# kaist-ina/BWA-MEME

Hardware: AMD Instinct MI355X
Metric: seeding_reads_per_sec (higher is better)
Workload: dtype u64; 1 GPU; learned-index seeding (rounds 1-3 + hit gather), 150 bp SE reads vs 3100 Mbp synthetic genome (fwd+rc suffix array of 6200000000 entries), index and reads resident in HBM; genome_bp=3100000000, sa_entries=6200000000, read_len=150, rmi_leaves_log2=28

## Files before the change

bwa-meme_amd/csrc/meme_common.h:

```cpp
#pragma once
#include <hip/hip_runtime.h>
#include <stdint.h>
#include <stdio.h>
#include <string>
#include <type_traits>
#include <utility>
#include <vector>

#include "meme_hip.h"

typedef uint64_t u64;
typedef int64_t i64;

struct __attribute__((aligned(16))) SaEnt {
    u64 key;
    u64 pos;
};

struct RmiRec {
    double icpt;
    double slope;
    u64 err;
};

struct Rmi32 {
    double icpt;
    double slope;
    u64 err;
    u64 pad;
};

struct DevIndex {
    i64 n = 0;
    const SaEnt* sa = nullptr;
    const u64* pac = nullptr;
    const Rmi32* l2 = nullptr;
    const Rmi32* l1 = nullptr;
    i64 n_l2 = 0, n_l1 = 0;
    int shift = 64;
    const uint8_t* plcp = nullptr;
};

template <bool HOST> struct Buf {
    void* p = nullptr;
    size_t cap = 0;
    Buf() = default;
    Buf(const Buf&) = delete; Buf& operator=(const Buf&) = delete;
    ~Buf() { if (p) (void)(HOST ? hipHostFree(p) : hipFree(p)); }
    template <class T> T* as() const { return (T*)p; }
};
typedef Buf<false> DevBuf;
typedef Buf<true> HostBuf;
static_assert(!std::is_copy_constructible<DevBuf>::value && !std::is_copy_assignable<DevBuf>::value && !std::is_copy_constructible<HostBuf>::value &&
              !std::is_copy_assignable<HostBuf>::value, "a workspace owns its memory: a copy would free it twice");
template <int N> struct Events {
    hipEvent_t e[N] = {};
    Events() = default;
    Events(const Events&) = delete; Events& operator=(const Events&) = delete;
    ~Events() { for (hipEvent_t x : e) if (x) (void)hipEventDestroy(x); }
    hipEvent_t& operator[](int i) { return e[i]; }
    hipError_t ensure() { for (hipEvent_t& x : e) if (!x) { const hipError_t r = hipEventCreate(&x); if (r != hipSuccess) return r; } return hipSuccess; }
};
struct Stream {
    hipStream_t s = nullptr;
    Stream() = default;
    Stream(const Stream&) = delete; Stream& operator=(const Stream&) = delete;
    ~Stream() { if (s) (void)hipStreamDestroy(s); }
    operator hipStream_t() const { return s; }
};

struct Carve {
    unsigned char* base;
    size_t bytes = 0;
    explicit Carve(void* b) : base((unsigned char*)b) {}
    template <class T> T* take(size_t count, size_t align = 1) { bytes = (bytes + align - 1) / align * align; T* q = base ? (T*)(base + bytes) : nullptr; bytes += count * sizeof(T); return q; }
    i64* col(i64 n) { return take<i64>((size_t)n + 1); }
};
struct ContigTab {
    i64* off; int* len; unsigned char* alt; size_t bytes;
    ContigTab(void* base, i64 n, bool with_alt) { Carve c(base); off = c.take<i64>(n); len = c.take<int>(n); alt = c.take<unsigned char>((with_alt ? n : 0) + 64); bytes = c.bytes; }
};
struct ChainCounts {
    i64 *chain_off, *seed_off, *nch, *nsd; int* tree; unsigned char* fb; unsigned long long* route; size_t bytes;
    ChainCounts(void* base, i64 n) { Carve c(base); chain_off = c.col(n); seed_off = c.col(n); nch = c.col(n); nsd = c.col(n); tree = c.take<int>(n); fb = c.take<unsigned char>(n + 64);
                                     route = c.take<unsigned long long>(8, 16); bytes = c.bytes; }
};
struct ChainLists {
    i64 *list[5], *work[5], *woff[5]; unsigned char* cls; size_t bytes;
    ChainLists(void* base, i64 n) { Carve c(base); for (int k = 0; k < 5; ++k) { list[k] = c.col(n); work[k] = c.col(n); woff[k] = c.col(n); } cls = c.take<unsigned char>(n + 64); bytes = c.bytes; }
};
enum { EXT_L = 0, EXT_R = 1, EXT_B = 2 };
struct ExtCounts {
    i64 *cnt[3], *off[3], *cntS, *offS; size_t bytes;
    ExtCounts(void* base, i64 n) { Carve c(base); for (i64*& q : cnt) q = c.col(n); for (i64*& q : off) q = c.col(n); cntS = c.col(n); offS = c.col(n); bytes = c.bytes; }
    bool adjacent(i64 n) const { return off[1] == off[0] + (n + 1) && off[2] == off[1] + (n + 1); }
};
struct CountScan {
    i64 *cnt, *off; size_t bytes;
    CountScan(void* base, i64 n) { Carve c(base); cnt = c.col(n); off = c.col(n); bytes = c.bytes; }
};
struct ExtRetry {
    meme_seqpair* half[2]; size_t bytes;
    ExtRetry(void* base, i64 nmax) { Carve c(base); for (meme_seqpair*& q : half) q = c.take<meme_seqpair>((size_t)nmax + 1); bytes = c.bytes; }
};
struct ExtRounds {
    int4* state; uint8_t* act; uint8_t* sel; size_t bytes;
    ExtRounds(void* base, i64 n, i64 seeds) { Carve c(base); state = c.take<int4>(n + 1); act = c.take<uint8_t>(n + 1); sel = c.take<uint8_t>(seeds + 64); bytes = c.bytes; }
};
struct GcigCols {
    i64 *zsz, *csz, *zoff, *coff, *ncig, *ooff, *msz, *moff, *psz, *poff, *isdp, *dpoff, *dplist, *is16, *o16, *is32, *o32, *is64, *o64, *bad; size_t bytes;
    GcigCols(void* base, i64 n) { Carve c(base); zsz = c.col(n); csz = c.col(n); zoff = c.col(n); coff = c.col(n); ncig = c.col(n); ooff = c.col(n); msz = c.col(n); moff = c.col(n);
        psz = c.col(n); poff = c.col(n); isdp = c.col(n); dpoff = c.col(n); dplist = c.col(n); is16 = c.col(n); o16 = c.col(n); is32 = c.col(n); o32 = c.col(n); is64 = c.col(n);
        o64 = c.col(n); bad = c.take<i64>(8); bytes = c.bytes; }
};
struct BswSort {
    int *hist, *offs, *cursor, *maxq; unsigned int* tickets; size_t bytes;
    BswSort(void* base, int keys) { Carve c(base); hist = c.take<int>(keys); offs = c.take<int>(keys + 1); cursor = c.take<int>(keys); maxq = c.take<int>(1); tickets = c.take<unsigned int>(30); bytes = c.bytes; }
};
struct MateCounts {
    i64 *cntQ, *cntJ, *cntR, *cntY, *offQ, *offJ, *offR, *offY; size_t bytes;
    MateCounts(void* base, i64 n) { Carve c(base); cntQ = c.col(n); cntJ = c.col(n); cntR = c.col(n); cntY = c.col(n); offQ = c.col(n); offJ = c.col(n); offR = c.col(n); offY = c.col(n); bytes = c.bytes; }
};
struct SamCols {
    i64 *bound, *soff, *len, *toff, *bad; size_t bytes;
    SamCols(void* base, i64 n) { Carve c(base); bound = c.col(n); soff = c.col(n); len = c.col(n); toff = c.col(n); bad = c.take<i64>(8); bytes = c.bytes; }
};
struct ResidentBatch {
    DevBuf reads, read_off, packed, smems, hits, smem_off, hit_off;
    i64 last_seed_reads = 0;
    i64 last_seed_max_len = 0;
    bool reads_resident = false;
};
enum { SEED_CTR_SLOT = 0, SEED_CTR_SEARCHES = 1, SEED_CTR_OVERFLOW = 2, SEED_CTR_WINDOWS = 3, SEED_CTR_PROF = 4, SEED_CTR_LANE = 12, SEED_CTR_PEND = 13, SEED_CTR_BLK = 14, SEED_CTR_BLK_OUT = 15,
       SEED_CTRS = 16 };
enum { SEED_EV_PACK0, SEED_EV_PACK1, SEED_EV_SEARCH0, SEED_EV_SEARCH1, SEED_EV_RESEED0, SEED_EV_GATHER0, SEED_EV_GATHER1, SEED_EVS };
struct SeedWs {
    DevBuf slots[3], ovf[2];
    DevBuf slot_cnt, slot_hits, slot_loc, counters, pend, blk;
    HostBuf h_smems, h_hits, h_smem_off, h_hit_off;
    unsigned long long* counter_set(int cset) { return (unsigned long long*)counters.p + SEED_CTRS * cset; }
    Events<SEED_EVS> ev;
    Stream emit; Events<2> emit_ev;
};
struct ChainWs {
    DevBuf ch1, sd1, hdr, frac, contigs, counts, chains, seeds, lists;
    DevBuf wave[5];
    HostBuf h_chain_off, h_chains, h_seed_off, h_seeds, h_tree, h_frac, h_fallback;
    Events<5> ev;
    const i64* chain_off() const { return (const i64*)counts.p; }
    const i64* seed_off(i64 n) const { return ChainCounts(counts.p, n).seed_off; }
};
enum { EXT_CTR_RETRY = 0, EXT_CTR_FLT_JOBS = 2, EXT_CTR_CENSUS = 8, EXT_CTR_HEAVY = 24, EXT_CTR_BYTES = 256 };
struct ExtWs {
    DevBuf rmax, regs, order, counts, pairs_l, pairs_r, retry, seq, counters;
    DevBuf flt_sc, flt_jobs, flt_cnt, flt_seeds, flt_score, flt_hsp;
    DevBuf live_cnt, live_regs, rounds, heavy;
    HostBuf h_reg_off, h_regs; Events<2> ev;
};
struct BswWs { DevBuf pairs, refb, qerb, order, ws, hist; Events<2> ev; };
struct GcigWs {
    DevBuf jobs, cols, z, cig, res, ops, md, nm, md_packed, cjobs, cres; HostBuf h_res, h_ops, h_md; Events<2> ev;
};
struct KswvWs {
    DevBuf jobs, order, ref, qer, res, rowmax, rm_off; HostBuf h_res; Events<2> ev;
};
struct MateWs {
    DevBuf regs, reg_off, contigs, counts, gar, aux, batch_off; HostBuf h_gar, h_batch_off, h_jobs;
};
struct SamWs {
    DevBuf names, name_off, quals, recs, blob, cols, scratch, text, contigs; HostBuf h_text_off, h_text; Events<2> ev;
};

struct SideStreams {
    Stream st[3];
    Events<3> done;
    Events<1> fork;
};

struct meme_ctx {
    int device = 0;
    int n_cus = 256;
    DevIndex idx;
    bool owns_index = false;
    std::vector<std::pair<void*, size_t>> owned;
    void* plcp_aux = nullptr;
    ResidentBatch batch;
    DevBuf scan_tmp;
    ChainWs chain; ExtWs ext; BswWs bsw; GcigWs gcig; KswvWs kswv; MateWs mate; SamWs sam; SeedWs seed;
    Stream stream;
    SideStreams side;
    i64 seed_blocks = 0;
    i64 smem_cap = 128;
    i64 group_lanes = 4;
    i64 seed_blocks_per_cu = 5;
    i64 max_batch = 0;
    i64 ext_slab_jobs = 8 << 20;
    i64 ext_slab_bytes = (i64)3 << 29;
    i64 ext_split = 1;
    i64 bsw_circ = 1;
    i64 sam_max_batch = 0;
    i64 ext_live_only = 0;
    i64 ext_rounds = 1;
    i64 gcig_groups = 1;
    i64 gcig_zcap = -1;
    i64 ext_census = 0;
    i64 seed_defer = 1;
    i64 chain_light_hits = 32;
    i64 chain_lane_hits = 256;
    i64 chain_wave_tiers = 1;
    i64 bsw_blocks = 0;
    i64 bsw_lane_min_pairs = 32768;
    i64 sam_text_reads = 0;
    bool sam_has_quals = false;
    meme_timings tm = {};
};

void meme_set_error(const char* fmt, ...);
int meme_buf_reserve(meme_ctx* ctx, DevBuf& b, size_t bytes);
int meme_side_stream(meme_ctx* ctx, int i);
int meme_hostbuf_reserve(meme_ctx* ctx, HostBuf& b, size_t bytes);
inline unsigned grid_blocks(i64 items, int per, i64 cap = 256 * 64) { i64 b = (items + per - 1) / per; return (unsigned)(b < cap ? (b < 1 ? 1 : b) : cap); }
int meme_stage_contigs(meme_ctx* ctx, DevBuf& buf, std::vector<unsigned char>& host, const meme_contig* contigs, int32_t n_contigs, i64 l_pac, bool with_alt,
                       const char* prefix, ContigTab* out);
int meme_scan_exclusive(meme_ctx* ctx, const i64* d_in, i64* d_out, i64 n);
int meme_scan_total(meme_ctx* ctx, const i64* d_in, i64* d_out, i64 n, i64* h_total);
inline bool meme_fits_free_hbm(size_t need, size_t have, size_t* free_b) { size_t total_b = 0; return need <= have || hipMemGetInfo(free_b, &total_b) != hipSuccess || need <= *free_b / 2 + have; }
int meme_bsw_launch(meme_ctx* ctx, meme_seqpair* d_pairs, const uint8_t* d_ref, const uint8_t* d_qer, int npairs, int w, const meme_bsw_opt* opt,
                    int host_maxq);
hipError_t meme_bsw_last_ms(meme_ctx* ctx, float* ms);
constexpr int MEME_SEEDSW_MAX = 200;
struct meme_seedsw_job { i64 rb; i64 qoff; int seed; short tlen, qlen; };
int meme_seedsw_launch(meme_ctx* ctx, const meme_seedsw_job* d_jobs, const unsigned long long* d_njobs, i64 max_jobs, int* d_sc, const meme_ext_opt* o);
int meme_kswv_run(meme_ctx* ctx, const meme_kswv_job* jobs, int64_t njobs, const uint8_t* ref, int64_t ref_bytes, const uint8_t* qer, int64_t qer_bytes, const meme_bsw_opt* opt,
                  bool staged, meme_kswv_host_result* out);
int meme_chain_reserve(meme_ctx* ctx, i64 n);
int meme_chain_run(meme_ctx* ctx, const meme_contig* contigs, int32_t n_contigs, const meme_chain_opt* opt, i64* totals);

#define HIP_TRY(expr)                                                                          \
    do {                                                                                       \
        hipError_t _e = (expr);                                                                \
        if (_e != hipSuccess) {                                                                \
            meme_set_error("%s failed: %s (%s:%d)", #expr, hipGetErrorString(_e), __FILE__, __LINE__); \
            return MEME_E_HIP;                                                                 \
        }                                                                                      \
    } while (0)

__device__ __forceinline__ u64 load_pos5(const uint8_t* pos5, i64 i) {
    const i64 bo = i * 5;
    const uint32_t* pd = reinterpret_cast<const uint32_t*>(pos5 + (bo & ~3ll));
    const u64 two = (u64)pd[0] | ((u64)pd[1] << 32);
    const u64 v5 = (two >> (8 * (int)(bo & 3))) & 0xffffffffffull;
    return ((v5 & 0xffffffffull) << 8) | (v5 >> 32);
}
__device__ __forceinline__ u64 extract32(const u64* w, i64 s) {
    i64 k = s >> 5;
    int sh = (int)(s & 31) * 2;
    u64 a = w[k], b = w[k + 1];
    return sh ? (a << sh) | (b >> (64 - sh)) : a;
}
```

bwa-meme_amd/csrc/meme_ctx.hip:

```cpp
#include <fcntl.h>
#include <stdarg.h>
#include <stdlib.h>
#include <string.h>
#include <sys/stat.h>
#include <unistd.h>
#include <atomic>
#include <chrono>
#include <functional>
#include <thread>

#include "meme_common.h"

static thread_local char g_err[512] = "";

void meme_set_error(const char* fmt, ...) {
    va_list ap;
    va_start(ap, fmt);
    vsnprintf(g_err, sizeof(g_err), fmt, ap);
    va_end(ap);
}

extern "C" const char* meme_last_error(void) { return g_err; }

int meme_buf_reserve(meme_ctx* ctx, DevBuf& b, size_t bytes) {
    if (bytes <= b.cap) return MEME_OK;
    if (b.p) { HIP_TRY(hipStreamSynchronize(ctx->stream)); HIP_TRY(hipFree(b.p)); b.p = nullptr; b.cap = 0; }
    size_t want = bytes + bytes / 4 + 256;
    HIP_TRY(hipMalloc(&b.p, want));
    b.cap = want;
    return MEME_OK;
}

int meme_side_stream(meme_ctx* ctx, int i) {
    SideStreams& S = ctx->side;
    if (!S.st[i].s) HIP_TRY(hipStreamCreateWithFlags(&S.st[i].s, hipStreamNonBlocking));
    if (!S.done[i]) HIP_TRY(hipEventCreateWithFlags(&S.done[i], hipEventDisableTiming));
    if (!S.fork[0]) HIP_TRY(hipEventCreateWithFlags(&S.fork[0], hipEventDisableTiming));
    return MEME_OK;
}

int meme_hostbuf_reserve(meme_ctx* ctx, HostBuf& b, size_t bytes) {
    if (bytes <= b.cap) return MEME_OK;
    if (b.p) { HIP_TRY(hipStreamSynchronize(ctx->stream)); HIP_TRY(hipHostFree(b.p)); b.p = nullptr; b.cap = 0; }
    size_t want = bytes + bytes / 4 + 4096;
    HIP_TRY(hipHostMalloc(&b.p, want, hipHostMallocDefault));
    b.cap = want;
    return MEME_OK;
}

extern "C" void* meme_host_alloc(int64_t bytes) {
    void* p = nullptr;
    if (bytes <= 0) return nullptr;
    if (hipHostMalloc(&p, (size_t)bytes, hipHostMallocDefault) != hipSuccess) { meme_set_error("hipHostMalloc(%lld) failed", (long long)bytes); return nullptr; }
    return p;
}
extern "C" void meme_host_free(void* p) { if (p) (void)hipHostFree(p); }

extern "C" int meme_device_count(void) {
    int n = 0;
    if (hipGetDeviceCount(&n) != hipSuccess) return 0;
    return n;
}


extern "C" meme_ctx* meme_ctx_create(int device) {
    int n = meme_device_count();
    if (n <= 0) { meme_set_error("no HIP device visible: the MI355X backend has no CPU fallback"); return nullptr; }
    if (device < 0 || device >= n) { meme_set_error("device %d out of range (0..%d)", device, n - 1); return nullptr; }
    if (hipSetDevice(device) != hipSuccess) { meme_set_error("hipSetDevice(%d) failed", device); return nullptr; }
    meme_ctx* ctx = new meme_ctx();
    ctx->device = device;
    { hipDeviceProp_t prop; if (hipGetDeviceProperties(&prop, device) == hipSuccess && prop.multiProcessorCount > 0) ctx->n_cus = prop.multiProcessorCount; }
    if (hipStreamCreateWithFlags(&ctx->stream.s, hipStreamNonBlocking) != hipSuccess) {
        meme_set_error("hipStreamCreate failed");
        delete ctx;
        return nullptr;
    }
    return ctx;
}

extern "C" void meme_ctx_destroy(meme_ctx* ctx) {
    if (!ctx) return;
    (void)hipSetDevice(ctx->device);
    for (hipStream_t st : {ctx->stream.s, ctx->side.st[0].s, ctx->side.st[1].s, ctx->side.st[2].s, ctx->seed.emit.s})
        if (st) (void)hipStreamSynchronize(st);
    if (ctx->owns_index) for (auto& o : ctx->owned) (void)hipFree(o.first);
    if (ctx->plcp_aux) (void)hipFree(ctx->plcp_aux);
    delete ctx;
}

int meme_stage_contigs(meme_ctx* ctx, DevBuf& buf, std::vector<unsigned char>& host, const meme_contig* contigs, int32_t n_contigs, i64 l_pac, bool with_alt,
                       const char* prefix, ContigTab* out) {
    for (int i = 0; i < n_contigs; ++i)
        if (contigs[i].len < 1 || contigs[i].offset < 0 || contigs[i].offset + contigs[i].len > l_pac || (i > 0 && contigs[i].offset < contigs[i - 1].offset + contigs[i - 1].len)) {
            meme_set_error("%scontig %d (offset %lld, length %d) is not a valid reference sequence of a %lld-base genome", prefix, i, (long long)contigs[i].offset, contigs[i].len,
                           (long long)l_pac);
            return MEME_E_ARG;
        }
    const size_t bytes = ContigTab(nullptr, n_contigs, with_alt).bytes;
    int rc = meme_buf_reserve(ctx, buf, bytes);
    if (rc) return rc;
    host.assign(bytes, 0);
    ContigTab t(host.data(), n_contigs, with_alt);
    for (int i = 0; i < n_contigs; ++i) { t.off[i] = contigs[i].offset; t.len[i] = contigs[i].len; if (with_alt) t.alt[i] = contigs[i].is_alt ? 1 : 0; }
    HIP_TRY(hipMemcpyAsync(buf.p, host.data(), bytes, hipMemcpyHostToDevice, ctx->stream));
    *out = ContigTab(buf.p, n_contigs, with_alt);
    return MEME_OK;
}

extern "C" int meme_ctx_sync(meme_ctx* ctx) {
    if (!ctx) return MEME_E_ARG;
    HIP_TRY(hipStreamSynchronize(ctx->stream));
    return MEME_OK;
}

extern "C" void* meme_ctx_stream(meme_ctx* ctx) { return ctx ? (void*)ctx->stream : nullptr; }

extern "C" int meme_get_timings(meme_ctx* ctx, meme_timings* out) {
    if (!ctx || !out) return MEME_E_ARG;
    *out = ctx->tm;
    return MEME_OK;
}

extern "C" int meme_set_tuning(meme_ctx* ctx, const char* key, int64_t value) {
    if (!ctx || !key) return MEME_E_ARG;
    if (!strcmp(key, "gcig_groups") && value != 0 && value != 1) { meme_set_error("gcig_groups must be 0 or 1"); return MEME_E_ARG; }
    if (!strcmp(key, "group_lanes") && value != 1 && value != 2 && value != 4 && value != 8 && value != 16 && value != 32) { meme_set_error("group_lanes must be 1, 2, 4, 8, 16 or 32"); return MEME_E_ARG; }
    const i64 any = INT64_MIN;
    static const struct { const char* key; i64 meme_ctx::*member; i64 at_least; } keys[] = {
        {"seed_blocks", &meme_ctx::seed_blocks, any}, {"smem_cap", &meme_ctx::smem_cap, 8}, {"seed_defer", &meme_ctx::seed_defer, any}, {"max_batch", &meme_ctx::max_batch, any},
        {"sam_max_batch", &meme_ctx::sam_max_batch, any}, {"bsw_circ", &meme_ctx::bsw_circ, any}, {"ext_split", &meme_ctx::ext_split, any}, {"ext_slab_jobs", &meme_ctx::ext_slab_jobs, 1},
        {"ext_census", &meme_ctx::ext_census, any}, {"gcig_zcap", &meme_ctx::gcig_zcap, any}, {"gcig_groups", &meme_ctx::gcig_groups, any}, {"ext_live_only", &meme_ctx::ext_live_only, any},
        {"ext_rounds", &meme_ctx::ext_rounds, 0}, {"bsw_blocks", &meme_ctx::bsw_blocks, any}, {"bsw_lane_min_pairs", &meme_ctx::bsw_lane_min_pairs, any},
        {"chain_wave_tiers", &meme_ctx::chain_wave_tiers, any}, {"chain_lane_hits", &meme_ctx::chain_lane_hits, any}, {"chain_light_hits", &meme_ctx::chain_light_hits, any},
        {"group_lanes", &meme_ctx::group_lanes, any}, {"seed_blocks_per_cu", &meme_ctx::seed_blocks_per_cu, 1}};
    for (const auto& k : keys) if (!strcmp(key, k.key)) { ctx->*k.member = value < k.at_least ? k.at_least : value; return MEME_OK; }
    meme_set_error("unknown tuning key %s", key);
    return MEME_E_ARG;
}

extern "C" int meme_index_share(meme_ctx* ctx, meme_ctx* owner);
extern "C" int64_t meme_index_pac64_words(int64_t sa_num) { return ((sa_num + 31) >> 5) + 8; }
extern "C" int64_t meme_index_pos5_bytes(int64_t sa_num) { return sa_num * 5 + 16; }

__global__ void __launch_bounds__(256) k_pack_text(const uint8_t* __restrict__ text, i64 n, u64* __restrict__ pac, i64 words) {
  for (i64 w = (i64)blockIdx.x * blockDim.x + threadIdx.x; w < words; w += (i64)gridDim.x * blockDim.x) {
    i64 base = w << 5;
    u64 v = 0;
    if (base + 32 <= n) {
        const uint4* p = reinterpret_cast<const uint4*>(text + base);
        uint4 a = p[0], b = p[1];
        uint32_t q[8] = {a.x, a.y, a.z, a.w, b.x, b.y, b.z, b.w};
#pragma unroll
        for (int k = 0; k < 8; ++k) {
            uint32_t x = q[k];
            v = (v << 8) | ((u64)(x & 3) << 6) | ((u64)((x >> 8) & 3) << 4) | ((u64)((x >> 16) & 3) << 2) |
                (u64)((x >> 24) & 3);
        }
    } else {
        for (int r = 0; r < 32; ++r) {
            i64 p = base + r;
            u64 c = p < n ? (u64)(text[p] & 3) : 3ull;
            v = (v << 2) | c;
        }
    }
    pac[w] = v;
  }
}

__global__ void __launch_bounds__(256) k_build_entries(const uint8_t* __restrict__ pos_packed, const u64* __restrict__ sa_u64,
                                                        i64 n, const u64* __restrict__ pac, SaEnt* __restrict__ ent) {
  for (i64 i = (i64)blockIdx.x * blockDim.x + threadIdx.x; i < n; i += (i64)gridDim.x * blockDim.x) {
    const u64 pos = sa_u64 ? sa_u64[i] : load_pos5(pos_packed, i);
    SaEnt e;
    e.key = extract32(pac, (i64)pos);
    e.pos = pos;
    ent[i] = e;
  }
}

__global__ void __launch_bounds__(256) k_pos5_from_sa(const u64* __restrict__ sa, i64 n, uint8_t* __restrict__ pos5) {
  for (i64 i = (i64)blockIdx.x * blockDim.x + threadIdx.x; i < n; i += (i64)gridDim.x * blockDim.x) {
    const u64 pos = sa[i];
    uint8_t* p = pos5 + i * 5;
    const uint32_t hi = (uint32_t)(pos >> 8);
    p[0] = (uint8_t)hi; p[1] = (uint8_t)(hi >> 8); p[2] = (uint8_t)(hi >> 16); p[3] = (uint8_t)(hi >> 24); p[4] = (uint8_t)(pos & 0xff);
  }
}

__global__ void __launch_bounds__(256) k_rmi32(const RmiRec* __restrict__ in, i64 n, Rmi32* __restrict__ out) {
  for (i64 i = (i64)blockIdx.x * blockDim.x + threadIdx.x; i < n; i += (i64)gridDim.x * blockDim.x) {
    const RmiRec r = in[i];
    Rmi32 o;
    o.icpt = r.icpt; o.slope = r.slope; o.err = r.err; o.pad = 0;
    out[i] = o;
  }
}

__device__ __forceinline__ int pair_lcp(const SaEnt a, const SaEnt b, i64 n, const u64* __restrict__ pac) {
    i64 lim = n - (i64)(a.pos > b.pos ? a.pos : b.pos);
    if (lim > 255) lim = 255;
    const u64 x = a.key ^ b.key;
    int l = x ? (__clzll((long long)x) >> 1) : 32;
    if (!x) {
        for (int m = 1; l < lim; ++m) {
            const u64 y = extract32(pac, (i64)a.pos + 32 * m) ^ extract32(pac, (i64)b.pos + 32 * m);
            if (y) { l += __clzll((long long)y) >> 1; break; }
            l += 32;
        }
    }
    return l < (int)lim ? l : (int)lim;
}

__global__ void __launch_bounds__(256) k_build_plcp(const SaEnt* __restrict__ ent, i64 n, const u64* __restrict__ pac, uint8_t* __restrict__ plcp) {
    __shared__ int sl[257];
    for (i64 b0 = (i64)blockIdx.x * 256; b0 < n; b0 += (i64)gridDim.x * 256) {
        const i64 i = b0 + threadIdx.x;
        SaEnt e; e.key = 0; e.pos = 0;
        int ln = 0;
        if (i < n) {
            e = ent[i];
            if (i + 1 < n) ln = pair_lcp(e, ent[i + 1], n, pac);
        }
        sl[threadIdx.x + 1] = ln;
        if (threadIdx.x == 0) sl[0] = b0 > 0 ? pair_lcp(ent[b0 - 1], e, n, pac) : 0;
        __syncthreads();
        if (i < n) {
            const int a = sl[threadIdx.x], b = sl[threadIdx.x + 1];
            plcp[e.pos] = (uint8_t)(a > b ? a : b);
        }
        __syncthreads();
    }
}

extern "C" int meme_stage_build_plcp(meme_ctx* ctx, const void* d_sa_ent, int64_t n, const void* d_pac64, void* d_plcp) {
    if (!ctx || !d_sa_ent || !d_pac64 || !d_plcp || n <= 0) return MEME_E_ARG;
    HIP_TRY(hipSetDevice(ctx->device));
    hipLaunchKernelGGL(k_build_plcp, dim3(grid_blocks(n, 256)), dim3(256), 0, ctx->stream, (const SaEnt*)d_sa_ent, (i64)n, (const u64*)d_pac64,
                       (uint8_t*)d_plcp);
    HIP_TRY(hipGetLastError());
    return MEME_OK;
}

extern "C" int meme_stage_pack_text(meme_ctx* ctx, const uint8_t* d_text, int64_t n, void* d_pac64) {
    if (!ctx || !d_text || !d_pac64 || n <= 0) return MEME_E_ARG;
    HIP_TRY(hipSetDevice(ctx->device));
    i64 words = meme_index_pac64_words(n);
    hipLaunchKernelGGL(k_pack_text, dim3(grid_blocks(words, 256)), dim3(256), 0, ctx->stream, d_text, n,
                       (u64*)d_pac64, words);
    HIP_TRY(hipGetLastError());
    return MEME_OK;
}

extern "C" int meme_stage_build_entries(meme_ctx* ctx, const uint8_t* d_pos_packed, int64_t n, const void* d_pac64,
                                        void* d_sa_ent) {
    if (!ctx || !d_pos_packed || !d_pac64 || !d_sa_ent || n <= 0) return MEME_E_ARG;
    HIP_TRY(hipSetDevice(ctx->device));
    hipLaunchKernelGGL(k_build_entries, dim3(grid_blocks(n, 256)), dim3(256), 0, ctx->stream, d_pos_packed,
                       (const u64*)nullptr, (i64)n, (const u64*)d_pac64, (SaEnt*)d_sa_ent);
    HIP_TRY(hipGetLastError());
    return MEME_OK;
}

extern "C" int meme_stage_entries_from_sa(meme_ctx* ctx, const uint64_t* d_sa, int64_t n, const void* d_pac64,
                                          void* d_sa_ent) {
    if (!ctx || !d_sa || !d_pac64 || !d_sa_ent || n <= 0) return MEME_E_ARG;
    HIP_TRY(hipSetDevice(ctx->device));
    hipLaunchKernelGGL(k_build_entries, dim3(grid_blocks(n, 256)), dim3(256), 0, ctx->stream,
                       (const uint8_t*)nullptr, (const u64*)d_sa, (i64)n, (const u64*)d_pac64, (SaEnt*)d_sa_ent);
    HIP_TRY(hipGetLastError());
    return MEME_OK;
}

extern "C" int meme_stage_pos5_from_sa(meme_ctx* ctx, const uint64_t* d_sa, int64_t n, void* d_pos5) {
    if (!ctx || !d_sa || !d_pos5 || n <= 0) return MEME_E_ARG;
    HIP_TRY(hipSetDevice(ctx->device));
    hipLaunchKernelGGL(k_pos5_from_sa, dim3(grid_blocks(n, 256)), dim3(256), 0, ctx->stream, (const u64*)d_sa, (i64)n, (uint8_t*)d_pos5);
    HIP_TRY(hipGetLastError());
    return MEME_OK;
}

extern "C" int meme_stage_rmi32(meme_ctx* ctx, const void* d_rmi24, int64_t records, void* d_rmi32) {
    if (!ctx || !d_rmi32 || records < 0 || (records > 0 && !d_rmi24)) return MEME_E_ARG;
    HIP_TRY(hipSetDevice(ctx->device));
    if (records == 0) return MEME_OK;
    hipLaunchKernelGGL(k_rmi32, dim3(grid_blocks(records, 256)), dim3(256), 0, ctx->stream, (const RmiRec*)d_rmi24, (i64)records, (Rmi32*)d_rmi32);
    HIP_TRY(hipGetLastError());
    return MEME_OK;
}

static int set_rmi(meme_ctx* ctx, i64 l2_records, i64 l1_records) {
    if (l2_records <= 0 || (l2_records & (l2_records - 1)) != 0) {
        meme_set_error("L2 parameter table must hold a power-of-two number of 24-byte records (got %lld)",
                       (long long)l2_records);
        return MEME_E_IO;
    }
    int bits = 0;
    while (((i64)1 << bits) < l2_records) ++bits;
    ctx->idx.shift = 64 - bits;
    ctx->idx.n_l2 = l2_records;
    ctx->idx.n_l1 = l1_records;
    return MEME_OK;
}

static void drop_index(meme_ctx* ctx) {
    if (ctx->owns_index) for (auto& o : ctx->owned) (void)hipFree(o.first);
    ctx->owned.clear();
    ctx->owns_index = false;
    if (ctx->plcp_aux) { (void)hipFree(ctx->plcp_aux); ctx->plcp_aux = nullptr; }
    ctx->idx = DevIndex();
}

static int own_alloc(meme_ctx* ctx, void** p, size_t bytes) {
    HIP_TRY(hipMalloc(p, bytes));
    ctx->owned.push_back({*p, bytes});
    ctx->owns_index = true;
    return MEME_OK;
}

typedef std::function<int(int, void*, size_t)> index_fetch_fn;
typedef std::function<void(const void*, i64, i64, hipStream_t)> index_piece_fn;
typedef std::function<int(int, int, const index_piece_fn&)> index_stream_fn;
static int index_build_from(meme_ctx* ctx, int64_t n, int64_t l1_bytes, int64_t l2_bytes, const index_fetch_fn& fetch,
                            const index_stream_fn& stream = index_stream_fn()) {
    if (n < 64 || l2_bytes < 24 || l2_bytes % 24 || l1_bytes % 24) {
        meme_set_error("index: bad sizes (sa_num must be >= 64, parameter files multiples of 24 B)");
        return MEME_E_ARG;
    }
    HIP_TRY(hipSetDevice(ctx->device));
    drop_index(ctx);
    int rc = set_rmi(ctx, l2_bytes / 24, l1_bytes / 24);
    if (rc) return rc;
    const bool trace = getenv("MEME_LOAD_TRACE") != nullptr;
    auto t_last = std::chrono::steady_clock::now();
    auto lap = [&](const char* what) {
        if (!trace) return;
        (void)hipStreamSynchronize(ctx->stream);
        const auto now = std::chrono::steady_clock::now();
        fprintf(stderr, "[meme] index build: %s %.3f s\n", what, std::chrono::duration<double>(now - t_last).count());
        t_last = now;
    };
    const i64 words = meme_index_pac64_words(n);
    const i64 n_l2 = l2_bytes / 24, n_l1 = l1_bytes / 24;
    void *d_ent = nullptr, *d_pac = nullptr, *d_l2 = nullptr, *d_l1 = nullptr, *d_tmp = nullptr;
    if ((rc = own_alloc(ctx, &d_ent, (size_t)n * sizeof(SaEnt)))) return rc;
    if ((rc = own_alloc(ctx, &d_pac, (size_t)words * 8))) return rc;
    if ((rc = own_alloc(ctx, &d_l2, (size_t)n_l2 * 32))) return rc;
    if ((rc = own_alloc(ctx, &d_l1, (size_t)(n_l1 > 0 ? n_l1 : 1) * 32))) return rc;
    size_t tmp_bytes = stream ? (size_t)n + 64 : (size_t)meme_index_pos5_bytes(n);
    if (!stream && (size_t)l2_bytes > tmp_bytes) tmp_bytes = (size_t)l2_bytes;
    if (!stream && (size_t)l1_bytes > tmp_bytes) tmp_bytes = (size_t)l1_bytes;
    HIP_TRY(hipMalloc(&d_tmp, tmp_bytes));
    lap("device allocations");
    auto fail = [&](int code) { (void)hipStreamSynchronize(ctx->stream); (void)hipFree(d_tmp); return code; };
    if ((rc = fetch(0, d_tmp, (size_t)n))) return fail(rc);
    if ((rc = meme_stage_pack_text(ctx, (const uint8_t*)d_tmp, n, d_pac))) return fail(rc);
    if (hipStreamSynchronize(ctx->stream) != hipSuccess) return fail(MEME_E_HIP);
    lap("text + pack kernel");
    if (stream) {
        if ((rc = stream(1, 5, [&](const void* d_piece, i64 first, i64 count, hipStream_t st) {
                hipLaunchKernelGGL(k_build_entries, dim3(grid_blocks(count, 256)), dim3(256), 0, st, (const uint8_t*)d_piece, (const u64*)nullptr, count,
                                   (const u64*)d_pac, (SaEnt*)d_ent + first);
            }))) return fail(rc);
        lap("position image -> entries (streamed)");
        if ((rc = stream(2, 24, [&](const void* d_piece, i64 first, i64 count, hipStream_t st) {
                hipLaunchKernelGGL(k_rmi32, dim3(grid_blocks(count, 256)), dim3(256), 0, st, (const RmiRec*)d_piece, count, (Rmi32*)d_l2 + first);
            }))) return fail(rc);
        if (n_l1 > 0 && (rc = stream(3, 24, [&](const void* d_piece, i64 first, i64 count, hipStream_t st) {
                hipLaunchKernelGGL(k_rmi32, dim3(grid_blocks(count, 256)), dim3(256), 0, st, (const RmiRec*)d_piece, count, (Rmi32*)d_l1 + first);
            }))) return fail(rc);
        if (hipGetLastError() != hipSuccess) return fail(MEME_E_HIP);
    } else {
        if ((rc = fetch(1, d_tmp, (size_t)n * 5))) return fail(rc);
        if (hipMemsetAsync((uint8_t*)d_tmp + (size_t)n * 5, 0, 16, ctx->stream) != hipSuccess) return fail(MEME_E_HIP);
        if ((rc = meme_stage_build_entries(ctx, (const uint8_t*)d_tmp, n, d_pac, d_ent))) return fail(rc);
        if (hipStreamSynchronize(ctx->stream) != hipSuccess) return fail(MEME_E_HIP);
        lap("position image + entry kernel");
        if ((rc = fetch(2, d_tmp, (size_t)l2_bytes))) return fail(rc);
        if ((rc = meme_stage_rmi32(ctx, d_tmp, n_l2, d_l2))) return fail(rc);
        if (n_l1 > 0) {
            if (hipStreamSynchronize(ctx->stream) != hipSuccess) return fail(MEME_E_HIP);
            if ((rc = fetch(3, d_tmp, (size_t)l1_bytes))) return fail(rc);
            if ((rc = meme_stage_rmi32(ctx, d_tmp, n_l1, d_l1))) return fail(rc);
        }
    }
    HIP_TRY(hipStreamSynchronize(ctx->stream));
    lap("model records");
    HIP_TRY(hipFree(d_tmp));
    lap("free of the staging buffer");
    void* d_plcp = nullptr;
    if ((rc = own_alloc(ctx, &d_plcp, (size_t)n + 256))) return rc;
    if ((rc = meme_stage_build_plcp(ctx, d_ent, n, d_pac, d_plcp))) return rc;
    HIP_TRY(hipStreamSynchronize(ctx->stream));
    lap("plcp table");
    ctx->idx.plcp = (const uint8_t*)d_plcp;
    ctx->idx.n = n;
    ctx->idx.sa = (const SaEnt*)d_ent;
    ctx->idx.pac = (const u64*)d_pac;
    ctx->idx.l2 = (const Rmi32*)d_l2;
    ctx->idx.l1 = (const Rmi32*)d_l1;
    return MEME_OK;
}

extern "C" int meme_index_load_host(meme_ctx* ctx, const uint8_t* pos_packed, int64_t n, const uint8_t* text,
                                    const void* l1, int64_t l1_bytes, const void* l2, int64_t l2_bytes) {
    if (!ctx || !pos_packed || !text || !l2 || (l1_bytes > 0 && !l1)) { meme_set_error("meme_index_load_host: null argument"); return MEME_E_ARG; }
    const void* src[4] = {text, pos_packed, l2, l1};
    return index_build_from(ctx, n, l1_bytes, l2_bytes, [&](int which, void* d_dst, size_t bytes) {
        if (hipMemcpyAsync(d_dst, src[which], bytes, hipMemcpyHostToDevice, ctx->stream) != hipSuccess) return (int)MEME_E_HIP;
        return hipStreamSynchronize(ctx->stream) == hipSuccess ? (int)MEME_OK : (int)MEME_E_HIP;
    });
}

static long long file_size(const std::string& path) {
    struct stat st;
    return stat(path.c_str(), &st) == 0 ? (long long)st.st_size : -1;
}

struct LoadBuffers {
    static constexpr size_t PIECE = (size_t)16 << 20;
    int T = 0;
    std::vector<uint8_t*> buf;
    std::vector<uint8_t*> dbuf;
    int init(int readers) {
        T = readers;
        buf.assign((size_t)2 * T, nullptr);
        dbuf.assign((size_t)2 * T, nullptr);
        for (auto& b : buf) if (hipHostMalloc((void**)&b, PIECE, hipHostMallocDefault) != hipSuccess) return MEME_E_HIP;
        for (auto& b : dbuf) if (hipMalloc((void**)&b, PIECE + 64) != hipSuccess) return MEME_E_HIP;
        return MEME_OK;
    }
    ~LoadBuffers() { for (auto b : buf) if (b) (void)hipHostFree(b); for (auto b : dbuf) if (b) (void)hipFree(b); }
};

static int file_to_device(meme_ctx* ctx, LoadBuffers& LB, const std::string& path, void* d_dst, size_t bytes, int unit = 1,
                          const index_piece_fn* consume = nullptr) {
    if (bytes == 0) return MEME_OK;
    const int fd = open(path.c_str(), O_RDONLY);
    if (fd < 0) { meme_set_error("cannot open %s", path.c_str()); return MEME_E_IO; }
    const size_t piece = LoadBuffers::PIECE / (size_t)unit * (size_t)unit;
    const size_t n_pieces = (bytes + piece - 1) / piece;
    const int T = (int)(n_pieces < (size_t)LB.T ? n_pieces : (size_t)LB.T);
    std::atomic<int> err{MEME_OK};
    auto reader = [&](int t) {
        if (hipSetDevice(ctx->device) != hipSuccess) { err = MEME_E_HIP; return; }
        hipStream_t st = nullptr;
        uint8_t* buf[2] = {LB.buf[(size_t)2 * t], LB.buf[(size_t)2 * t + 1]};
        hipEvent_t ev[2] = {nullptr, nullptr};
        bool ok = hipStreamCreateWithFlags(&st, hipStreamNonBlocking) == hipSuccess;
        for (int b = 0; b < 2 && ok; ++b) ok = hipEventCreateWithFlags(&ev[b], hipEventDisableTiming) == hipSuccess;
        int turn = 0;
        for (size_t k = (size_t)t; ok && k < n_pieces && err == MEME_OK; k += (size_t)T, turn ^= 1) {
            const size_t off = k * piece, len = bytes - off < piece ? bytes - off : piece;
            if (hipEventSynchronize(ev[turn]) != hipSuccess) { ok = false; break; }
            size_t got = 0;
            while (got < len) {
                const ssize_t r = pread(fd, buf[turn] + got, len - got, (off_t)(off + got));
                if (r <= 0) break;
                got += (size_t)r;
            }
            if (got != len) { err = MEME_E_IO; break; }
            if (consume) {
                uint8_t* slot = LB.dbuf[(size_t)2 * t + turn];
                ok = hipMemcpyAsync(slot, buf[turn], len, hipMemcpyHostToDevice, st) == hipSuccess;
                if (ok) (*consume)(slot, (i64)(off / (size_t)unit), (i64)(len / (size_t)unit), st);
                ok = ok && hipEventRecord(ev[turn], st) == hipSuccess;
            } else
                ok = hipMemcpyAsync((uint8_t*)d_dst + off, buf[turn], len, hipMemcpyHostToDevice, st) == hipSuccess &&
                     hipEventRecord(ev[turn], st) == hipSuccess;
        }
        if (st && hipStreamSynchronize(st) != hipSuccess) ok = false;
        for (int b = 0; b < 2; ++b) if (ev[b]) (void)hipEventDestroy(ev[b]);
        if (st) (void)hipStreamDestroy(st);
        if (!ok && err == MEME_OK) err = MEME_E_HIP;
    };
    std::vector<std::thread> th;
    for (int t = 1; t < T; ++t) th.emplace_back(reader, t);
    reader(0);
    for (auto& x : th) x.join();
    close(fd);
    if (err == MEME_E_IO) meme_set_error("short read from %s", path.c_str());
    else if (err != MEME_OK) meme_set_error("HIP error while loading %s: %s", path.c_str(), hipGetErrorString(hipGetLastError()));
    return err;
}

extern "C" int meme_index_load_files(meme_ctx* ctx, const char* prefix) {
    if (!ctx || !prefix) return MEME_E_ARG;
    const std::string p(prefix);
    const std::string name[4] = {p + ".0123", p + ".pos_packed", p + ".suffixarray_uint64_L2_PARAMETERS", p + ".suffixarray_uint64_L1_PARAMETERS"};
    long long size[4];
    for (int i = 0; i < 4; ++i)
        if ((size[i] = file_size(name[i])) < 0) { meme_set_error("cannot read %s", name[i].c_str()); return MEME_E_IO; }
    if (size[1] % 5 || size[1] / 5 != size[0]) {
        meme_set_error("%s: .pos_packed (%lld B) and .0123 (%lld B) disagree on the suffix count", prefix, size[1], size[0]);
        return MEME_E_IO;
    }
    const bool trace = getenv("MEME_LOAD_TRACE") != nullptr;
    LoadBuffers LB;
    HIP_TRY(hipSetDevice(ctx->device));
    if (LB.init(getenv("MEME_LOAD_THREADS") && atoi(getenv("MEME_LOAD_THREADS")) > 0 ? atoi(getenv("MEME_LOAD_THREADS")) : 8)) { meme_set_error("pinned staging for the index load could not be allocated"); return MEME_E_HIP; }
    return index_build_from(ctx, size[0], size[3], size[2], [&](int which, void* d_dst, size_t bytes) {
        if ((long long)bytes != size[which]) { meme_set_error("%s changed size while loading", name[which].c_str()); return (int)MEME_E_IO; }
        const auto t0 = std::chrono::steady_clock::now();
        const int rc = file_to_device(ctx, LB, name[which], d_dst, bytes);
        if (trace) {
            const double dt = std::chrono::duration<double>(std::chrono::steady_clock::now() - t0).count();
            fprintf(stderr, "[meme] %s: %.2f GB to the device in %.2f s (%.1f GB/s)\n", name[which].c_str(), bytes / 1e9, dt, bytes / 1e9 / dt);
        }
        return rc;
    }, [&](int which, int unit, const index_piece_fn& consume) {
        if (size[which] % unit) { meme_set_error("%s is not a whole number of %d-byte records", name[which].c_str(), unit); return (int)MEME_E_IO; }
        const auto t0 = std::chrono::steady_clock::now();
        const int rc = file_to_device(ctx, LB, name[which], nullptr, (size_t)size[which], unit, &consume);
        if (trace) {
            const double dt = std::chrono::duration<double>(std::chrono::steady_clock::now() - t0).count();
            fprintf(stderr, "[meme] %s: %.2f GB through the device rings in %.2f s (%.1f GB/s)\n", name[which].c_str(), size[which] / 1e9, dt, size[which] / 1e9 / dt);
        }
        return rc;
    });
}

extern "C" int meme_index_attach(meme_ctx* ctx, const meme_index_arrays* a) {
    if (!ctx || !a || !a->d_sa_ent || !a->d_pac64 || !a->d_l2 || a->sa_num < 64) return MEME_E_ARG;
    drop_index(ctx);
    int rc = set_rmi(ctx, a->l2_records, a->l1_records);
    if (rc) return rc;
    ctx->idx.n = a->sa_num;
    ctx->idx.sa = (const SaEnt*)a->d_sa_ent;
    ctx->idx.pac = (const u64*)a->d_pac64;
    ctx->idx.l2 = (const Rmi32*)a->d_l2;
    ctx->idx.l1 = (const Rmi32*)a->d_l1;
    HIP_TRY(hipSetDevice(ctx->device));
    HIP_TRY(hipMalloc(&ctx->plcp_aux, (size_t)a->sa_num + 256));
    if ((rc = meme_stage_build_plcp(ctx, a->d_sa_ent, a->sa_num, a->d_pac64, ctx->plcp_aux))) return rc;
    HIP_TRY(hipStreamSynchronize(ctx->stream));
    ctx->idx.plcp = (const uint8_t*)ctx->plcp_aux;
    return MEME_OK;
}

extern "C" int meme_index_describe(meme_ctx* ctx, meme_index_arrays* out) {
    if (!ctx || !out) return MEME_E_ARG;
    if (!ctx->idx.sa) { meme_set_error("no index loaded"); return MEME_E_STATE; }
    out->sa_num = ctx->idx.n;
    out->d_sa_ent = (void*)ctx->idx.sa;
    out->d_pac64 = (void*)ctx->idx.pac;
    out->d_l2 = (void*)ctx->idx.l2;
    out->l2_records = ctx->idx.n_l2;
    out->d_l1 = (void*)ctx->idx.l1;
    out->l1_records = ctx->idx.n_l1;
    return MEME_OK;
}

extern "C" int meme_index_replicate(meme_ctx* dst, meme_ctx* src) {
    if (!dst || !src || dst == src) return MEME_E_ARG;
    if (!src->idx.sa) { meme_set_error("meme_index_replicate: source has no index"); return MEME_E_STATE; }
    if (dst->device == src->device) return meme_index_share(dst, src);
    if (!src->owns_index) { meme_set_error("meme_index_replicate: the source ctx must own its index (load_host / load_files)"); return MEME_E_STATE; }
    HIP_TRY(hipSetDevice(dst->device));
    drop_index(dst);
    int can = 0;
    (void)hipDeviceCanAccessPeer(&can, dst->device, src->device);
    if (can) { hipError_t e = hipDeviceEnablePeerAccess(src->device, 0); (void)e; (void)hipGetLastError(); }
    DevIndex I = src->idx;
    for (auto& o : src->owned) {
        void* d = nullptr;
        int rc = own_alloc(dst, &d, o.second);
        if (rc) return rc;
        HIP_TRY(hipMemcpyPeerAsync(d, dst->device, o.first, src->device, o.second, dst->stream));
        if ((const void*)I.sa == o.first) I.sa = (const SaEnt*)d;
        if ((const void*)I.pac == o.first) I.pac = (const u64*)d;
        if ((const void*)I.l2 == o.first) I.l2 = (const Rmi32*)d;
        if ((const void*)I.l1 == o.first) I.l1 = (const Rmi32*)d;
        if ((const void*)I.plcp == o.first) I.plcp = (const uint8_t*)d;
    }
    HIP_TRY(hipStreamSynchronize(dst->stream));
    dst->idx = I;
    return MEME_OK;
}

extern "C" int meme_index_share(meme_ctx* ctx, meme_ctx* owner) {
    if (!ctx || !owner || ctx->device != owner->device) return MEME_E_ARG;
    if (!owner->idx.sa) { meme_set_error("owner has no index"); return MEME_E_STATE; }
    drop_index(ctx);
    ctx->idx = owner->idx;
    return MEME_OK;
}
```

bwa-meme_amd/csrc/meme_seed.hip:

```cpp
#include <limits.h>
#include <stdlib.h>
#include <string.h>
#include <utility>

#include "meme_seed_kernel.h"

namespace {

using namespace seedk;

constexpr int SCAN_BLOCK = 256;
constexpr int SCAN_ITEMS = 4;
constexpr int SCAN_TILE = SCAN_BLOCK * SCAN_ITEMS;

__device__ __forceinline__ i64 block_scan_excl(i64 v, i64* total) {
    __shared__ i64 wsum[SCAN_BLOCK / 64];
    const int lane = threadIdx.x & 63, wid = threadIdx.x >> 6;
    i64 x = v;
#pragma unroll
    for (int d = 1; d < 64; d <<= 1) {
        i64 y = __shfl_up(x, d);
        if (lane >= d) x += y;
    }
    if (lane == 63) wsum[wid] = x;
    __syncthreads();
    i64 off = 0, tot = 0;
    for (int w = 0; w < SCAN_BLOCK / 64; ++w) {
        if (w < wid) off += wsum[w];
        tot += wsum[w];
    }
    __syncthreads();
    *total = tot;
    return off + x - v;
}

__global__ void __launch_bounds__(SCAN_BLOCK) k_tile_sums(const int* __restrict__ cnt, const i64* __restrict__ hits, i64 n,
                                                          i64* __restrict__ tile_sums) {
    i64 base = (i64)blockIdx.x * SCAN_TILE + threadIdx.x * SCAN_ITEMS;
    i64 a = 0, b = 0;
    for (int k = 0; k < SCAN_ITEMS; ++k) {
        i64 i = base + k;
        if (i < n) {
            int c = cnt[i];
            a += c < 0 ? 0 : c;
            b += hits[i];
        }
    }
    i64 ta, tb;
    block_scan_excl(a, &ta);
    block_scan_excl(b, &tb);
    if (threadIdx.x == 0) { tile_sums[2 * blockIdx.x] = ta; tile_sums[2 * blockIdx.x + 1] = tb; }
}

__global__ void __launch_bounds__(SCAN_BLOCK) k_scan_tiles(i64* __restrict__ tile_sums, i64 ntiles, i64* __restrict__ totals) {
    i64 ca = 0, cb = 0;
    for (i64 base = 0; base < ntiles; base += SCAN_BLOCK) {
        i64 i = base + threadIdx.x;
        i64 a = i < ntiles ? tile_sums[2 * i] : 0, b = i < ntiles ? tile_sums[2 * i + 1] : 0;
        i64 ta, tb;
        i64 ea = block_scan_excl(a, &ta);
        i64 eb = block_scan_excl(b, &tb);
        if (i < ntiles) { tile_sums[2 * i] = ca + ea; tile_sums[2 * i + 1] = cb + eb; }
        ca += ta;
        cb += tb;
    }
    if (threadIdx.x == 0) { totals[0] = ca; totals[1] = cb; }
}

__global__ void __launch_bounds__(SCAN_BLOCK) k_offsets(const int* __restrict__ cnt, const i64* __restrict__ hits, i64 n,
                                                        const i64* __restrict__ tile_sums, i64* __restrict__ smem_off,
                                                        i64* __restrict__ hit_off) {
    i64 base = (i64)blockIdx.x * SCAN_TILE + threadIdx.x * SCAN_ITEMS;
    i64 va[SCAN_ITEMS], vb[SCAN_ITEMS], a = 0, b = 0;
    for (int k = 0; k < SCAN_ITEMS; ++k) {
        i64 i = base + k;
        va[k] = vb[k] = 0;
        if (i < n) {
            int c = cnt[i];
            va[k] = c < 0 ? 0 : c;
            vb[k] = hits[i];
        }
        a += va[k];
        b += vb[k];
    }
    i64 ta, tb;
    i64 ea = block_scan_excl(a, &ta) + tile_sums[2 * blockIdx.x];
    i64 eb = block_scan_excl(b, &tb) + tile_sums[2 * blockIdx.x + 1];
    for (int k = 0; k < SCAN_ITEMS; ++k) {
        i64 i = base + k;
        if (i < n) { smem_off[i] = ea; hit_off[i] = eb; }
        ea += va[k];
        eb += vb[k];
    }
    if (blockIdx.x == gridDim.x - 1 && threadIdx.x == SCAN_BLOCK - 1) { smem_off[n] = ea; hit_off[n] = eb; }
}

struct TierTable {
    const SlotRec* base[N_TIERS];
    int cap[N_TIERS];
};

__global__ void __launch_bounds__(BLOCK) k_gather(const SaEnt* __restrict__ sa, TierTable tiers, const i64* __restrict__ slot_loc,
                                                   const int* __restrict__ cnt, i64 n, int hits_per_smem,
                                                   const i64* __restrict__ smem_off, const i64* __restrict__ hit_off,
                                                   meme_mem_tl* __restrict__ smems, u64* __restrict__ hits) {
    constexpr int GL = 16;
    const int lane = threadIdx.x & 63;
    const int t = lane & (GL - 1);
    const int gbase = lane - t;
    i64 gid = ((i64)blockIdx.x * BLOCK + threadIdx.x) / GL;
    const i64 ngroups = (i64)gridDim.x * BLOCK / GL;
    for (i64 r = gid; r < n; r += ngroups) {
        const int c = cnt[r];
        if (c <= 0) continue;
        const i64 loc = slot_loc[r];
        const int tier = (int)(loc >> 40);
        const SlotRec* sl = tiers.base[tier] + (loc & ((1ll << 40) - 1)) * tiers.cap[tier];
        meme_mem_tl* out = smems + smem_off[r];
        u64* hout = hits + hit_off[r];
        i64 hb0 = 0;
        for (int k0 = 0; k0 < c; k0 += GL) {
            const int k = k0 + t;
            const bool act = k < c;
            SlotRec s;
            s.start = s.end = 0; s.sa_start = 0; s.count = 0;
            if (act) s = sl[k];
            i64 h = s.count;
            if (hits_per_smem > 0 && h > hits_per_smem) h = hits_per_smem;
            i64 incl = h;
#pragma unroll
            for (int d = 1; d < GL; d <<= 1) {
                i64 y = __shfl_up(incl, d, GL);
                if (t >= d) incl += y;
            }
            const i64 hb = hb0 + incl - h;
            u64 first = 0;
            if (act) {
                first = (s.sa_start & SLOT_POS) ? (u64)(s.sa_start & SLOT_VAL) : sa[s.sa_start].pos;
                meme_mem_tl m;
                m.start = s.start;
                m.end = s.end;
                m.hitbeg = (int32_t)hb;
                m.hitcount = s.count > (i64)INT_MAX ? INT_MAX : (int32_t)s.count;
                m.cache_refpos = first;
                out[k] = m;
                if (h > 0) hout[hb] = first;
                for (i64 i = 1; i < h && i < 4; ++i) hout[hb + i] = sa[s.sa_start + i].pos;
            }
            u64 longmask = (__ballot(act && h > 4) >> gbase) & 0xffffull;
            while (longmask) {
                const int src = __ffsll((long long)longmask) - 1;
                longmask &= longmask - 1;
                const i64 lh = __shfl(h, src, GL), lhb = __shfl(hb, src, GL), lsa = __shfl(s.sa_start, src, GL);
                for (i64 i = 4 + t; i < lh; i += GL) hout[lhb + i] = sa[lsa + i].pos;
            }
            hb0 += __shfl(incl, GL - 1, GL);
        }
    }
}

template <int G>
int launch_k_seed(hipStream_t stream, const SeedArgs& A, size_t lds, i64 blocks) {
    if (lds > 64 * 1024)
        HIP_TRY(hipFuncSetAttribute((const void*)k_seed<G>, hipFuncAttributeMaxDynamicSharedMemorySize, (int)lds));
    hipLaunchKernelGGL(k_seed<G>, dim3((unsigned)blocks), dim3(BLOCK), lds, stream, A);
    HIP_TRY(hipGetLastError());
    return MEME_OK;
}

struct SeedRun {
    meme_ctx* ctx;
    const i64* d_read_off; i64 nreads;
    const meme_seed_opt* opt;
    PackGeom geo;
    TierTable tiers = {};
    bool defer = false;
    i64 n_early = -1;
    i64 n_todo = 0;
    float ms_total = 0.f, ms_reseed = 0.f;
    i64 launches = 0, searches = 0, windows = 0, lane_searches = 0;
};

int seed_pack(SeedRun& R, const uint8_t* d_reads, i64 max_len, i64 total_bytes) {
    meme_ctx* ctx = R.ctx;
    if (max_len > MAX_READ_LEN) {
        meme_set_error("read of %lld bases exceeds the learned-index limit of %d (LEARNED_MAX_READ_LEN)", (long long)max_len, MAX_READ_LEN);
        return MEME_E_ARG;
    }
    if (max_len < 1) max_len = 1;
    PackGeom& geo = R.geo;
    geo.W = (int)((max_len + 31) / 32) + 2;
    geo.MW = (int)((max_len + 63) / 64);
    geo.stride = 2 * geo.W + 2 * geo.MW + 1;
    int rc;
    if ((rc = meme_buf_reserve(ctx, ctx->batch.packed, (size_t)R.nreads * geo.stride * 8))) return rc;
    HIP_TRY(hipEventRecord(ctx->seed.ev[SEED_EV_PACK0], ctx->stream));
    int rb = (int)((48 * 1024) / max_len);
    if (rb > 32) rb = 32;
    if (rb < 1) rb = 1;
    i64 pblocks = (R.nreads + rb - 1) / rb;
    if (pblocks > (i64)ctx->n_cus * 16) pblocks = (i64)ctx->n_cus * 16;
    size_t plds = ((size_t)rb * (size_t)max_len + 16 + 48 + 3) & ~(size_t)3;
    hipLaunchKernelGGL(k_pack_reads, dim3((unsigned)pblocks), dim3(256), plds, ctx->stream, d_reads,
                       R.d_read_off, R.nreads, total_bytes, geo, rb, (u64*)ctx->batch.packed.p);
    HIP_TRY(hipGetLastError());
    HIP_TRY(hipEventRecord(ctx->seed.ev[SEED_EV_PACK1], ctx->stream));
    return MEME_OK;
}

int launch_tier(SeedRun& R, int tier, i64 n_todo, const i64* pending, int cset, hipStream_t stream, bool defer) {
    meme_ctx* ctx = R.ctx;
    int G = tier == 0 ? (int)ctx->group_lanes : 32;
    const int cap = tier == 0 ? (int)ctx->smem_cap : TIER_CAP[tier];
    const int lcap = cap < TIER_LCAP[tier] ? cap : TIER_LCAP[tier];
    DevBuf& sb = ctx->seed.slots[tier];
    DevBuf& ob = ctx->seed.ovf[tier & 1];
    const size_t need = (size_t)n_todo * cap * sizeof(SlotRec);
    if (tier > 0 && need > sb.cap) {
        size_t free_b = 0;
        if (!meme_fits_free_hbm(need, 0, &free_b)) {
            meme_set_error("%lld reads emitted more than %d SMEMs each: re-running them needs %.1f GB of slots, more than half of the "
                           "free HBM (%.1f GB); seed this batch in smaller pieces", (long long)n_todo, R.tiers.cap[tier - 1],
                           need / 1e9, free_b / 1e9);
            return MEME_E_CAPACITY;
        }
    }
    int rc;
    if ((rc = meme_buf_reserve(ctx, sb, need))) return rc;
    if ((rc = meme_buf_reserve(ctx, ob, (size_t)n_todo * sizeof(i64)))) return rc;
    unsigned long long* counters = ctx->seed.counter_set(cset);
    HIP_TRY(hipMemsetAsync(counters, 0, SEED_CTRS * sizeof(unsigned long long), stream));
    SeedArgs A;
    A.I = ctx->idx;
    A.packed = (const u64*)ctx->batch.packed.p;
    A.read_off = R.d_read_off;
    A.nreads = n_todo;
    A.geo = R.geo;
    A.opt = *R.opt;
    A.slots = (SlotRec*)sb.p;
    A.slot_cnt = (int*)ctx->seed.slot_cnt.p;
    A.slot_hits = (i64*)ctx->seed.slot_hits.p;
    A.slot_loc = (i64*)ctx->seed.slot_loc.p;
    A.pending = pending;
    A.ovf_list = (i64*)ob.p;
    A.cap = cap;
    A.lcap = lcap;
    A.tier = tier;
    A.counters = counters;
    A.defer = defer ? 1 : 0;
    R.tiers.base[tier] = (const SlotRec*)sb.p;
    R.tiers.cap[tier] = cap;
    while (G < 32 && seed_lds_bytes(G, R.geo, lcap) > (size_t)160 * 1024) G *= 2;
    const int groups = BLOCK / G;
    size_t lds = seed_lds_bytes(G, R.geo, lcap);
    i64 want = (n_todo + groups - 1) / groups;
    i64 blocks = ctx->seed_blocks > 0 ? ctx->seed_blocks : (i64)ctx->n_cus * ctx->seed_blocks_per_cu;
    if (blocks > want) blocks = want;
    if (blocks < 1) blocks = 1;
    if (tier == 0) HIP_TRY(hipEventRecord(ctx->seed.ev[SEED_EV_SEARCH0], stream));
    switch (G) {
    case 1: return launch_k_seed<1>(stream, A, lds, blocks);
    case 2: return launch_k_seed<2>(stream, A, lds, blocks);
    case 4: return launch_k_seed<4>(stream, A, lds, blocks);
    case 8: return launch_k_seed<8>(stream, A, lds, blocks);
    case 16: return launch_k_seed<16>(stream, A, lds, blocks);
    case 32: return launch_k_seed<32>(stream, A, lds, blocks);
    default: meme_set_error("group_lanes must be 1, 2, 4, 8, 16 or 32"); return MEME_E_ARG;
    }
}

int fetch_counters(SeedRun& R, int cset, unsigned long long* h) {
    HIP_TRY(hipMemcpyAsync(h, R.ctx->seed.counter_set(cset), SEED_CTRS * sizeof(unsigned long long), hipMemcpyDeviceToHost, R.ctx->stream));
    HIP_TRY(hipStreamSynchronize(R.ctx->stream));
    return MEME_OK;
}
void tally(SeedRun& R, const unsigned long long* h) {
    ++R.launches;
    R.searches += (i64)h[SEED_CTR_SEARCHES];
    R.windows += (i64)h[SEED_CTR_WINDOWS];
    R.n_todo = (i64)h[SEED_CTR_OVERFLOW];
#ifdef SEED_PROF
    {
        double tot = 0; for (int k = 0; k < 8; ++k) tot += (double)h[SEED_CTR_PROF + k];
        fprintf(stderr, "[seed prof]:");
        const char* nm[6] = {"control", "request+rmi", "window+compare", "resolve", "level", "apply"};
        for (int k = 0; k < 6; ++k) fprintf(stderr, " %s %.1f%%", nm[k], 100.0 * (double)h[SEED_CTR_PROF + k] / (tot > 0 ? tot : 1));
        fprintf(stderr, "\n");
    }
#endif
}

int launch_reseed(SeedRun& R) {
    meme_ctx* ctx = R.ctx;
    SeedWs& S = ctx->seed;
    const i64 nreads = R.nreads;
    HIP_TRY(hipEventRecord(S.ev[SEED_EV_RESEED0], ctx->stream));
    ReseedArgs A;
    A.I = ctx->idx; A.packed = (const u64*)ctx->batch.packed.p; A.geo = R.geo; A.nreads = nreads; A.opt = *R.opt;
    A.slots = (SlotRec*)S.slots[0].p; A.cap = (int)ctx->smem_cap; A.slot_cnt = (int*)S.slot_cnt.p; A.slot_hits = (i64*)S.slot_hits.p;
    A.ovf_list = (i64*)S.ovf[0].p; A.counters = S.counter_set(0); A.pend_list = (i64*)S.pend.p;
    A.blk = (BlkRec*)S.blk.p; A.blk_out = A.blk + nreads * BLK_PER_READ; A.blk_cap = nreads * BLK_PER_READ;
    A.blk_ctr = SEED_CTR_BLK; A.blk_out_ctr = SEED_CTR_BLK_OUT;
    i64 rblocks = (nreads + 255) / 256;
    if (rblocks > (i64)ctx->n_cus * 32) rblocks = (i64)ctx->n_cus * 32;
    hipLaunchKernelGGL(k_reseed, dim3((unsigned)rblocks), dim3(256), 0, ctx->stream, A);
    HIP_TRY(hipEventRecord(ctx->side.fork[0], ctx->stream));
    const unsigned sblocks = (unsigned)(rblocks < (i64)ctx->n_cus * 4 ? rblocks : (i64)ctx->n_cus * 4);
    if (!S.emit.s) HIP_TRY(hipStreamCreateWithFlags(&S.emit.s, hipStreamNonBlocking));
    for (int i = 0; i < 2; ++i) if (!S.emit_ev[i]) HIP_TRY(hipEventCreateWithFlags(&S.emit_ev[i], hipEventDisableTiming));
    HIP_TRY(hipEventRecord(S.emit_ev[0], ctx->stream));
    HIP_TRY(hipStreamWaitEvent(S.emit, S.emit_ev[0], 0));
    hipLaunchKernelGGL(k_reseed_emit, dim3(sblocks), dim3(256), 0, S.emit, A);
    HIP_TRY(hipEventRecord(S.emit_ev[1], S.emit));
    constexpr int ROUNDS = 4;
    for (int round = 0; round < ROUNDS; ++round) {
        hipLaunchKernelGGL(k_reseed_search, dim3(sblocks), dim3(256), 0, ctx->stream, A);
        if (round < ROUNDS - 1) {
            hipLaunchKernelGGL(k_reseed_resume<false>, dim3(sblocks), dim3(256), 0, ctx->stream, A);
            HIP_TRY(hipMemsetAsync(S.counter_set(0) + A.blk_ctr, 0, sizeof(unsigned long long), ctx->stream));
            std::swap(A.blk, A.blk_out); std::swap(A.blk_ctr, A.blk_out_ctr);
        } else hipLaunchKernelGGL(k_reseed_resume<true>, dim3(sblocks), dim3(256), 0, ctx->stream, A);
    }
    HIP_TRY(hipGetLastError());
    return MEME_OK;
}

int launch_early_overflow(SeedRun& R) {
    meme_ctx* ctx = R.ctx;
    Stream& side = ctx->side.st[0];
    unsigned long long h_ovf = 0;
    HIP_TRY(hipStreamWaitEvent(side, ctx->side.fork[0], 0));
    HIP_TRY(hipMemcpyAsync(&h_ovf, ctx->seed.counter_set(0) + SEED_CTR_OVERFLOW, 8, hipMemcpyDeviceToHost, side));
    HIP_TRY(hipStreamSynchronize(side));
    if (h_ovf == 0) return MEME_OK;
    R.n_early = (i64)h_ovf;
    int rc;
    if ((rc = launch_tier(R, 1, R.n_early, (const i64*)ctx->seed.ovf[0].p, 1, side, false))) return rc;
    HIP_TRY(hipEventRecord(ctx->side.done[0], side));
    HIP_TRY(hipStreamWaitEvent(ctx->stream, ctx->side.done[0], 0));
    return MEME_OK;
}

int seed_tier0(SeedRun& R) {
    meme_ctx* ctx = R.ctx;
    SeedWs& S = ctx->seed;
    int rc;
    R.defer = ctx->seed_defer != 0 && ctx->idx.plcp != nullptr && R.opt->rounds >= 2;
    if (R.defer && (rc = meme_buf_reserve(ctx, S.pend, (size_t)R.nreads * sizeof(i64)))) return rc;
    if (R.defer && (rc = meme_buf_reserve(ctx, S.blk, (size_t)R.nreads * BLK_PER_READ * 2 * sizeof(BlkRec)))) return rc;
    if ((rc = launch_tier(R, 0, R.nreads, nullptr, 0, ctx->stream, R.defer))) return rc;
    if (R.defer) {
        if ((rc = meme_side_stream(ctx, 0)) || (rc = launch_reseed(R)) || (rc = launch_early_overflow(R))) return rc;
        HIP_TRY(hipStreamWaitEvent(ctx->stream, S.emit_ev[1], 0));
    }
    HIP_TRY(hipEventRecord(S.ev[SEED_EV_SEARCH1], ctx->stream));
    unsigned long long h[SEED_CTRS];
    if ((rc = fetch_counters(R, 0, h))) return rc;
    float ms = 0.f;
    HIP_TRY(hipEventElapsedTime(&ms, S.ev[SEED_EV_SEARCH0], S.ev[SEED_EV_SEARCH1]));
    R.ms_total += ms;
    if (R.defer) {
        float a = 0.f;
        HIP_TRY(hipEventElapsedTime(&a, S.ev[SEED_EV_RESEED0], S.ev[SEED_EV_SEARCH1]));
        R.ms_reseed += a;
        R.lane_searches += (i64)h[SEED_CTR_LANE];
        if (getenv("MEME_SEED_TRACE")) fprintf(stderr, "[meme] seed tier 0: search kernel + re-seeding kernels %.2f ms, of which behind k_seed %.2f ms (%lld lane searches; %lld reads of the "
                                               "overflow tier beside them)\n", ms, a, (long long)h[SEED_CTR_LANE], (long long)(R.n_early < 0 ? 0 : R.n_early));
    }
    tally(R, h);
    return MEME_OK;
}

int seed_overflow_tiers(SeedRun& R) {
    meme_ctx* ctx = R.ctx;
    SeedWs& S = ctx->seed;
    int rc;
    unsigned long long h[SEED_CTRS];
    for (int tier = 1; R.n_todo > 0; ++tier) {
        if (tier >= N_TIERS) {
            meme_set_error("a read produced more than %d SMEMs", TIER_CAP[N_TIERS - 1]);
            return MEME_E_CAPACITY;
        }
        const int cset = tier & 1;
        if (tier == 1 && R.n_early == R.n_todo) {
            if ((rc = fetch_counters(R, cset, h))) return rc;
        } else {
            HIP_TRY(hipEventRecord(S.ev[SEED_EV_SEARCH0], ctx->stream));
            if ((rc = launch_tier(R, tier, R.n_todo, (const i64*)S.ovf[(tier - 1) & 1].p, cset, ctx->stream, false))) return rc;
            HIP_TRY(hipEventRecord(S.ev[SEED_EV_SEARCH1], ctx->stream));
            if ((rc = fetch_counters(R, cset, h))) return rc;
            float ms = 0.f;
            HIP_TRY(hipEventElapsedTime(&ms, S.ev[SEED_EV_SEARCH0], S.ev[SEED_EV_SEARCH1]));
            R.ms_total += ms;
        }
        tally(R, h);
    }
    return MEME_OK;
}

int seed_gather(SeedRun& R, meme_seed_result* out) {
    meme_ctx* ctx = R.ctx;
    SeedWs& S = ctx->seed;
    ResidentBatch& B = ctx->batch;
    const i64 nreads = R.nreads;
    int rc;
    i64 ntiles = (nreads + SCAN_TILE - 1) / SCAN_TILE;
    if ((rc = meme_buf_reserve(ctx, ctx->scan_tmp, (size_t)(2 * ntiles + 2) * sizeof(i64)))) return rc;
    if ((rc = meme_buf_reserve(ctx, B.smem_off, (size_t)(nreads + 1) * sizeof(i64)))) return rc;
    if ((rc = meme_buf_reserve(ctx, B.hit_off, (size_t)(nreads + 1) * sizeof(i64)))) return rc;
    i64* tiles = (i64*)ctx->scan_tmp.p;
    i64* totals = tiles + 2 * ntiles;
    HIP_TRY(hipEventRecord(S.ev[SEED_EV_GATHER0], ctx->stream));
    hipLaunchKernelGGL(k_tile_sums, dim3((unsigned)ntiles), dim3(SCAN_BLOCK), 0, ctx->stream, (const int*)S.slot_cnt.p,
                       (const i64*)S.slot_hits.p, nreads, tiles);
    hipLaunchKernelGGL(k_scan_tiles, dim3(1), dim3(SCAN_BLOCK), 0, ctx->stream, tiles, ntiles, totals);
    hipLaunchKernelGGL(k_offsets, dim3((unsigned)ntiles), dim3(SCAN_BLOCK), 0, ctx->stream, (const int*)S.slot_cnt.p,
                       (const i64*)S.slot_hits.p, nreads, (const i64*)tiles, (i64*)B.smem_off.p, (i64*)B.hit_off.p);
    HIP_TRY(hipGetLastError());
    i64 h_tot[2];
    HIP_TRY(hipMemcpyAsync(h_tot, totals, sizeof(h_tot), hipMemcpyDeviceToHost, ctx->stream));
    HIP_TRY(hipStreamSynchronize(ctx->stream));
    if ((rc = meme_buf_reserve(ctx, B.smems, (size_t)(h_tot[0] + 1) * sizeof(meme_mem_tl)))) return rc;
    if ((rc = meme_buf_reserve(ctx, B.hits, (size_t)(h_tot[1] + 1) * sizeof(u64)))) return rc;
    i64 gblocks = (nreads + 15) / 16;
    if (gblocks > (i64)ctx->n_cus * 8) gblocks = (i64)ctx->n_cus * 8;
    if (gblocks < 1) gblocks = 1;
    hipLaunchKernelGGL(k_gather, dim3((unsigned)gblocks), dim3(BLOCK), 0, ctx->stream, ctx->idx.sa, R.tiers,
                       (const i64*)S.slot_loc.p, (const int*)S.slot_cnt.p, nreads, R.opt->hits_per_smem,
                       (const i64*)B.smem_off.p, (const i64*)B.hit_off.p, (meme_mem_tl*)B.smems.p, (u64*)B.hits.p);
    HIP_TRY(hipGetLastError());
    HIP_TRY(hipEventRecord(S.ev[SEED_EV_GATHER1], ctx->stream));
    HIP_TRY(hipStreamSynchronize(ctx->stream));
    HIP_TRY(hipEventElapsedTime(&ctx->tm.seed_gather_ms, S.ev[SEED_EV_GATHER0], S.ev[SEED_EV_GATHER1]));
    out->d_smems = (const meme_mem_tl*)B.smems.p;
    out->d_smem_off = (const i64*)B.smem_off.p;
    out->d_hits = (const u64*)B.hits.p;
    out->d_hit_off = (const i64*)B.hit_off.p;
    out->total_smems = h_tot[0];
    out->total_hits = h_tot[1];
    out->searches = R.searches;
    return MEME_OK;
}

int launch_seed(meme_ctx* ctx, const uint8_t* d_reads, const i64* d_read_off, i64 nreads, i64 max_len, i64 total_bytes,
                const meme_seed_opt* opt, meme_seed_result* out) {
    int rc;
    SeedWs& S = ctx->seed;
    ctx->batch.last_seed_reads = 0;
    ctx->sam_text_reads = 0;
    if ((rc = meme_buf_reserve(ctx, S.slot_cnt, (size_t)nreads * sizeof(int)))) return rc;
    if ((rc = meme_buf_reserve(ctx, S.slot_hits, (size_t)nreads * sizeof(i64)))) return rc;
    if ((rc = meme_buf_reserve(ctx, S.slot_loc, (size_t)nreads * sizeof(i64)))) return rc;
    if ((rc = meme_buf_reserve(ctx, S.counters, 2 * SEED_CTRS * sizeof(unsigned long long)))) return rc;
    HIP_TRY(S.ev.ensure());
    SeedRun R;
    R.ctx = ctx; R.d_read_off = d_read_off; R.nreads = nreads; R.opt = opt;
    if ((rc = seed_pack(R, d_reads, max_len, total_bytes)) || (rc = seed_tier0(R)) || (rc = seed_overflow_tiers(R))) return rc;
    HIP_TRY(hipEventElapsedTime(&ctx->tm.seed_pack_ms, S.ev[SEED_EV_PACK0], S.ev[SEED_EV_PACK1]));
    ctx->tm.seed_kernel_ms = R.ms_total;
    ctx->tm.seed_launches = R.launches;
    ctx->tm.seed_windows = R.windows;
    ctx->tm.seed_reseed_ms = R.ms_reseed;
    ctx->tm.seed_lane_searches = R.lane_searches;
    return seed_gather(R, out);
}

__global__ void __launch_bounds__(256) k_max_len(const i64* __restrict__ off, i64 n, int* out) {
    __shared__ int wmax[4];
    int v = 0;
    for (i64 i = (i64)blockIdx.x * blockDim.x + threadIdx.x; i < n; i += (i64)gridDim.x * blockDim.x) {
        int l = (int)(off[i + 1] - off[i]);
        v = v > l ? v : l;
    }
    for (int d = 32; d >= 1; d >>= 1) { int y = __shfl_xor(v, d); v = v > y ? v : y; }
    if ((threadIdx.x & 63) == 0) wmax[threadIdx.x >> 6] = v;
    __syncthreads();
    if (threadIdx.x == 0) {
        for (int k = 1; k < 4; ++k) v = v > wmax[k] ? v : wmax[k];
        atomicMax(out, v);
    }
}

int device_max_len(meme_ctx* ctx, const i64* d_read_off, i64 nreads, i64* max_len) {
    int rc;
    if ((rc = meme_buf_reserve(ctx, ctx->scan_tmp, 64))) return rc;
    HIP_TRY(hipMemsetAsync(ctx->scan_tmp.p, 0, 4, ctx->stream));
    i64 mblocks = (nreads + 255) / 256;
    if (mblocks > 1024) mblocks = 1024;
    hipLaunchKernelGGL(k_max_len, dim3((unsigned)mblocks), dim3(256), 0, ctx->stream, d_read_off, nreads,
                       (int*)ctx->scan_tmp.p);
    int v = 0;
    HIP_TRY(hipMemcpyAsync(&v, ctx->scan_tmp.p, 4, hipMemcpyDeviceToHost, ctx->stream));
    HIP_TRY(hipStreamSynchronize(ctx->stream));
    *max_len = v;
    return MEME_OK;
}

int check_opt(const meme_seed_opt* opt) {
    if (!opt || opt->min_seed_len < 1 || opt->rounds < 1 || opt->rounds > 3 || opt->hits_per_smem < 0) {
        meme_set_error("bad meme_seed_opt");
        return MEME_E_ARG;
    }
    return MEME_OK;
}

}

extern "C" int meme_seed_batch_device(meme_ctx* ctx, const uint8_t* d_reads, const int64_t* d_read_off, int64_t nreads,
                                      int64_t total_bases, const meme_seed_opt* opt, meme_seed_result* out) {
    if (!ctx || !d_reads || !d_read_off || !out || nreads < 0) return MEME_E_ARG;
    int rc = check_opt(opt);
    if (rc) return rc;
    if (!ctx->idx.sa) { meme_set_error("meme_seed_batch: no index loaded"); return MEME_E_STATE; }
    HIP_TRY(hipSetDevice(ctx->device));
    if (nreads == 0) { memset(out, 0, sizeof(*out)); return MEME_OK; }
    i64 max_len = 0;
    if ((rc = device_max_len(ctx, (const i64*)d_read_off, nreads, &max_len))) return rc;
    return launch_seed(ctx, d_reads, (const i64*)d_read_off, nreads, max_len, total_bases, opt, out);
}

extern "C" int meme_seed_batch(meme_ctx* ctx, const uint8_t* reads, const int64_t* read_off, int64_t nreads,
                               const meme_seed_opt* opt, meme_mem_tl* smems, int64_t smem_capacity, int64_t* smem_off,
                               uint64_t* hits, int64_t hit_capacity, int64_t* hit_off, int64_t* total_smems,
                               int64_t* total_hits) {
    if (!ctx || !reads || !read_off || !smems || !smem_off || !hits || !hit_off || nreads < 0) return MEME_E_ARG;
    int rc = check_opt(opt);
    if (rc) return rc;
    if (!ctx->idx.sa) { meme_set_error("meme_seed_batch: no index loaded"); return MEME_E_STATE; }
    HIP_TRY(hipSetDevice(ctx->device));
    if (nreads == 0) { smem_off[0] = 0; hit_off[0] = 0; if (total_smems) *total_smems = 0; if (total_hits) *total_hits = 0; return MEME_OK; }
    const i64 bases = read_off[nreads] - read_off[0];
    if (read_off[0] != 0) { meme_set_error("read_off[0] must be 0"); return MEME_E_ARG; }
    if ((rc = meme_buf_reserve(ctx, ctx->batch.reads, (size_t)bases + 16))) return rc;
    if ((rc = meme_buf_reserve(ctx, ctx->batch.read_off, (size_t)(nreads + 1) * sizeof(i64)))) return rc;
    HIP_TRY(hipMemcpyAsync(ctx->batch.reads.p, reads, (size_t)bases, hipMemcpyHostToDevice, ctx->stream));
    HIP_TRY(hipMemcpyAsync(ctx->batch.read_off.p, read_off, (size_t)(nreads + 1) * sizeof(i64), hipMemcpyHostToDevice, ctx->stream));
    meme_seed_result res;
    i64 max_len = 0;
    for (i64 i = 0; i < nreads; ++i) max_len = read_off[i + 1] - read_off[i] > max_len ? read_off[i + 1] - read_off[i] : max_len;
    rc = launch_seed(ctx, (const uint8_t*)ctx->batch.reads.p, (const i64*)ctx->batch.read_off.p, nreads, max_len, bases, opt, &res);
    if (rc) return rc;
    if (total_smems) *total_smems = res.total_smems;
    if (total_hits) *total_hits = res.total_hits;
    HIP_TRY(hipMemcpyAsync(smem_off, res.d_smem_off, (size_t)(nreads + 1) * sizeof(i64), hipMemcpyDeviceToHost, ctx->stream));
    HIP_TRY(hipMemcpyAsync(hit_off, res.d_hit_off, (size_t)(nreads + 1) * sizeof(i64), hipMemcpyDeviceToHost, ctx->stream));
    if (res.total_smems > smem_capacity || res.total_hits > hit_capacity) {
        HIP_TRY(hipStreamSynchronize(ctx->stream));
        meme_set_error("output buffers too small: need %lld SMEMs and %lld hits", (long long)res.total_smems,
                       (long long)res.total_hits);
        return MEME_E_CAPACITY;
    }
    HIP_TRY(hipMemcpyAsync(smems, res.d_smems, (size_t)res.total_smems * sizeof(meme_mem_tl), hipMemcpyDeviceToHost, ctx->stream));
    HIP_TRY(hipMemcpyAsync(hits, res.d_hits, (size_t)res.total_hits * sizeof(u64), hipMemcpyDeviceToHost, ctx->stream));
    HIP_TRY(hipStreamSynchronize(ctx->stream));
    return MEME_OK;
}

extern "C" int meme_seed_reserve(meme_ctx* ctx, int64_t nreads, int64_t total_bases) {
    if (!ctx || nreads < 0 || total_bases < 0) return MEME_E_ARG;
    if (nreads == 0) return MEME_OK;
    HIP_TRY(hipSetDevice(ctx->device));
    const size_t n = (size_t)nreads;
    const i64 len = total_bases / nreads + 32;
    const size_t stride = (size_t)(2 * ((len + 31) / 32 + 2) + 2 * ((len + 63) / 64) + 1);
    int rc;
    ResidentBatch& B = ctx->batch; SeedWs& S = ctx->seed;
    ChainWs& C = ctx->chain; ExtWs& E = ctx->ext;
    struct { DevBuf* b; size_t bytes; } dev[] = {
        {&B.reads, (size_t)total_bases + 16}, {&B.read_off, (n + 1) * 8}, {&S.slot_cnt, n * 4}, {&S.slot_hits, n * 8},
        {&S.slot_loc, n * 8}, {&S.counters, 2 * SEED_CTRS * 8}, {&S.pend, n * 8}, {&S.blk, n * BLK_PER_READ * 2 * sizeof(BlkRec)}, {&B.packed, n * stride * 8}, {&S.slots[0], n * (size_t)ctx->smem_cap * sizeof(SlotRec)},
        {&B.smem_off, (n + 1) * 8}, {&B.hit_off, (n + 1) * 8}, {&B.smems, n * 12 * sizeof(meme_mem_tl)}, {&B.hits, n * 24 * 8},
        {&C.chains, n * 3 * sizeof(meme_chain)}, {&C.seeds, n * 6 * sizeof(meme_chain_seed)}};
    for (auto& d : dev) if ((rc = meme_buf_reserve(ctx, *d.b, d.bytes))) return rc;
    if ((rc = meme_chain_reserve(ctx, nreads))) return rc;
    struct { HostBuf* b; size_t bytes; } host[] = {
        {&S.h_smem_off, (n + 1) * 8}, {&S.h_hit_off, (n + 1) * 8}, {&S.h_smems, n * 12 * sizeof(meme_mem_tl)}, {&S.h_hits, n * 24 * 8},
        {&C.h_chain_off, (n + 1) * 8}, {&C.h_chains, n * 3 * sizeof(meme_chain)}, {&C.h_seed_off, (n + 1) * 8},
        {&C.h_seeds, n * 6 * sizeof(meme_chain_seed)}, {&C.h_tree, n * 4}, {&C.h_frac, n * 4}, {&C.h_fallback, n}};
    for (auto& h : host) if ((rc = meme_hostbuf_reserve(ctx, *h.b, h.bytes))) return rc;
    struct { DevBuf* b; size_t bytes; } dev2[] = {
        {&E.rmax, n * 3 * 16}, {&E.regs, n * 4 * sizeof(meme_alnreg)}, {&E.order, n * 4 * 4}, {&E.counts, ExtCounts(nullptr, nreads).bytes},
        {&E.pairs_l, n * 2 * sizeof(meme_seqpair)}, {&E.pairs_r, n * 2 * sizeof(meme_seqpair)}, {&E.retry, n * 4 * sizeof(meme_seqpair)},
        {&E.seq, n * 4 * 250}};
    for (auto& d : dev2) if ((rc = meme_buf_reserve(ctx, *d.b, d.bytes))) return rc;
    if ((rc = meme_hostbuf_reserve(ctx, E.h_reg_off, (n + 1) * 8)) || (rc = meme_hostbuf_reserve(ctx, E.h_regs, n * 4 * sizeof(meme_alnreg))) ||
        (rc = meme_hostbuf_reserve(ctx, ctx->gcig.h_res, n / 2 * sizeof(meme_gres))) || (rc = meme_hostbuf_reserve(ctx, ctx->gcig.h_ops, n * 4))) return rc;
    return MEME_OK;
}

__global__ void __launch_bounds__(256) k_ascii_to_codes(uint4* __restrict__ p, i64 nvec) {
    for (i64 i = (i64)blockIdx.x * blockDim.x + threadIdx.x; i < nvec; i += (i64)gridDim.x * blockDim.x) {
        uint4 v = p[i];
        uint32_t w[4] = {v.x, v.y, v.z, v.w};
#pragma unroll
        for (int k = 0; k < 4; ++k) {
            uint32_t o = 0;
#pragma unroll
            for (int b = 0; b < 4; ++b) {
                const uint32_t c = (w[k] >> (8 * b)) & 0xffu, u = c & 0xdfu;
                const uint32_t code = c < 4 ? c : (u == 'A' ? 0u : u == 'C' ? 1u : u == 'G' ? 2u : u == 'T' ? 3u : 4u);
                o |= code << (8 * b);
            }
            w[k] = o;
        }
        v.x = w[0]; v.y = w[1]; v.z = w[2]; v.w = w[3];
        p[i] = v;
    }
}

static int seed_host_reads(meme_ctx* ctx, const uint8_t* reads, const int64_t* read_off, int64_t nreads, const meme_seed_opt* opt, const char* who,
                           meme_seed_host_result* out, int64_t* totals, bool ascii = false) {
    if (!ctx || !reads || !read_off || nreads < 0) return MEME_E_ARG;
    int rc = check_opt(opt);
    if (rc) return rc;
    if (!ctx->idx.sa) { meme_set_error("%s: no index loaded", who); return MEME_E_STATE; }
    HIP_TRY(hipSetDevice(ctx->device));
    if (out) {
        memset(out, 0, sizeof(*out));
        if ((rc = meme_hostbuf_reserve(ctx, ctx->seed.h_smem_off, (size_t)(nreads + 1) * sizeof(i64)))) return rc;
        if ((rc = meme_hostbuf_reserve(ctx, ctx->seed.h_hit_off, (size_t)(nreads + 1) * sizeof(i64)))) return rc;
        out->smem_off = (const int64_t*)ctx->seed.h_smem_off.p;
        out->hit_off = (const int64_t*)ctx->seed.h_hit_off.p;
    }
    if (totals) totals[0] = totals[1] = 0;
    ctx->batch.last_seed_reads = 0;
    if (nreads == 0) { if (out) { ((i64*)ctx->seed.h_smem_off.p)[0] = 0; ((i64*)ctx->seed.h_hit_off.p)[0] = 0; } return MEME_OK; }
    if (read_off[0] != 0) { meme_set_error("read_off[0] must be 0"); return MEME_E_ARG; }
    const i64 bases = read_off[nreads];
    if ((rc = meme_buf_reserve(ctx, ctx->batch.reads, (size_t)bases + 16))) return rc;
    if ((rc = meme_buf_reserve(ctx, ctx->batch.read_off, (size_t)(nreads + 1) * sizeof(i64)))) return rc;
    HIP_TRY(hipMemcpyAsync(ctx->batch.reads.p, reads, (size_t)bases, hipMemcpyHostToDevice, ctx->stream));
    HIP_TRY(hipMemcpyAsync(ctx->batch.read_off.p, read_off, (size_t)(nreads + 1) * sizeof(i64), hipMemcpyHostToDevice, ctx->stream));
    if (ascii) {
        const i64 nvec = (bases + 15) / 16;
        i64 cb = (nvec + 255) / 256;
        if (cb > (i64)ctx->n_cus * 16) cb = (i64)ctx->n_cus * 16;
        hipLaunchKernelGGL(k_ascii_to_codes, dim3((unsigned)(cb < 1 ? 1 : cb)), dim3(256), 0, ctx->stream, (uint4*)ctx->batch.reads.p, nvec);
        HIP_TRY(hipGetLastError());
    }
    i64 max_len = 0;
    for (i64 i = 0; i < nreads; ++i) max_len = read_off[i + 1] - read_off[i] > max_len ? read_off[i + 1] - read_off[i] : max_len;
    meme_seed_result res;
    rc = launch_seed(ctx, (const uint8_t*)ctx->batch.reads.p, (const i64*)ctx->batch.read_off.p, nreads, max_len, bases, opt, &res);
    if (rc) return rc;
    if (out) {
        if ((rc = meme_hostbuf_reserve(ctx, ctx->seed.h_smems, (size_t)(res.total_smems + 1) * sizeof(meme_mem_tl)))) return rc;
        if ((rc = meme_hostbuf_reserve(ctx, ctx->seed.h_hits, (size_t)(res.total_hits + 1) * sizeof(u64)))) return rc;
        HIP_TRY(hipMemcpyAsync(ctx->seed.h_smem_off.p, res.d_smem_off, (size_t)(nreads + 1) * sizeof(i64), hipMemcpyDeviceToHost, ctx->stream));
        HIP_TRY(hipMemcpyAsync(ctx->seed.h_hit_off.p, res.d_hit_off, (size_t)(nreads + 1) * sizeof(i64), hipMemcpyDeviceToHost, ctx->stream));
        HIP_TRY(hipMemcpyAsync(ctx->seed.h_smems.p, res.d_smems, (size_t)res.total_smems * sizeof(meme_mem_tl), hipMemcpyDeviceToHost, ctx->stream));
        HIP_TRY(hipMemcpyAsync(ctx->seed.h_hits.p, res.d_hits, (size_t)res.total_hits * sizeof(u64), hipMemcpyDeviceToHost, ctx->stream));
        out->smems = (const meme_mem_tl*)ctx->seed.h_smems.p;
        out->hits = (const uint64_t*)ctx->seed.h_hits.p;
        out->total_smems = res.total_smems;
        out->total_hits = res.total_hits;
    }
    HIP_TRY(hipStreamSynchronize(ctx->stream));
    if (totals) { totals[0] = res.total_smems; totals[1] = res.total_hits; }
    ctx->batch.last_seed_reads = nreads;
    ctx->batch.reads_resident = true;
    ctx->batch.last_seed_max_len = max_len;
    return MEME_OK;
}

extern "C" int meme_seed_batch_host(meme_ctx* ctx, const uint8_t* reads, const int64_t* read_off, int64_t nreads,
                                    const meme_seed_opt* opt, meme_seed_host_result* out) {
    if (!out) return MEME_E_ARG;
    return seed_host_reads(ctx, reads, read_off, nreads, opt, "meme_seed_batch_host", out, nullptr);
}

extern "C" int meme_seed_batch_resident(meme_ctx* ctx, const uint8_t* reads, const int64_t* read_off, int64_t nreads,
                                        const meme_seed_opt* opt, int64_t* total_smems, int64_t* total_hits) {
    int64_t tot[2] = {0, 0};
    const int rc = seed_host_reads(ctx, reads, read_off, nreads, opt, "meme_seed_batch_resident", nullptr, tot);
    if (total_smems) *total_smems = tot[0];
    if (total_hits) *total_hits = tot[1];
    return rc;
}

extern "C" int meme_seed_batch_resident_ascii(meme_ctx* ctx, const uint8_t* reads, const int64_t* read_off, int64_t nreads,
                                              const meme_seed_opt* opt, int64_t* total_smems, int64_t* total_hits) {
    int64_t tot[2] = {0, 0};
    const int rc = seed_host_reads(ctx, reads, read_off, nreads, opt, "meme_seed_batch_resident_ascii", nullptr, tot, true);
    if (total_smems) *total_smems = tot[0];
    if (total_hits) *total_hits = tot[1];
    return rc;
}
```

bwa-meme_amd/csrc/meme_seed_kernel.h:

```cpp
#pragma once
#include <limits.h>

#include "meme_common.h"

namespace seedk {

constexpr int BLOCK = 256;
constexpr int MAX_READ_LEN = 500;

struct SlotRec {
    int32_t start, end;
    i64 sa_start;
    i64 count;
};
constexpr i64 SLOT_POS = 1ll << 62;
constexpr i64 SLOT_DEFER = 1ll << 61;
constexpr i64 SLOT_PEND = 1ll << 59;
constexpr i64 SLOT_VAL = (1ll << 48) - 1;
constexpr int DEFER_MAX_K = 64;


constexpr int N_TIERS = 3;
constexpr int TIER_CAP[N_TIERS] = {64, 2048, 65536};
#ifndef LCAP0
#define LCAP0 16
#endif
constexpr int TIER_LCAP[N_TIERS] = {LCAP0, 512, 512};

struct PackGeom {
    int W;
    int MW;
    int stride;
};

struct SeedArgs {
    DevIndex I;
    const u64* packed;
    const i64* read_off;
    i64 nreads;
    PackGeom geo;
    meme_seed_opt opt;
    SlotRec* slots;
    int* slot_cnt;
    i64* slot_hits;
    i64* slot_loc;
    const i64* pending;
    i64* ovf_list;
    int cap, lcap, tier;
    unsigned long long* counters;
    int defer;
};

__global__ void __launch_bounds__(256) k_pack_reads(const uint8_t* __restrict__ reads, const i64* __restrict__ read_off,
                                                     i64 nreads, i64 total_bytes, PackGeom g, int PACK_RB,
                                                     u64* __restrict__ out) {
    extern __shared__ __attribute__((aligned(16))) unsigned char pk_raw[];
    uint32_t* stage = reinterpret_cast<uint32_t*>(pk_raw);
    const uint8_t* sb = pk_raw;
    __shared__ int has_n[64];
    for (i64 r0 = (i64)blockIdx.x * PACK_RB; r0 < nreads; r0 += (i64)gridDim.x * PACK_RB) {
        const int nr = (int)(nreads - r0 < PACK_RB ? nreads - r0 : PACK_RB);
        const i64 b0 = read_off[r0], b1 = read_off[r0 + nr];
        const i64 a0 = b0 & ~3ll;
        const int ndw = (int)((b1 - a0 + 3) >> 2);
        __syncthreads();
        const uint32_t* src = reinterpret_cast<const uint32_t*>(reads + a0);
        for (int k = threadIdx.x; k < ndw; k += blockDim.x) {
            uint32_t v;
            if (a0 + 4 * (i64)k + 4 <= total_bytes) v = src[k];
            else {
                v = 0;
                for (int bb = 0; bb < 4; ++bb)
                    if (a0 + 4 * (i64)k + bb < total_bytes) v |= (uint32_t)reads[a0 + 4 * (i64)k + bb] << (8 * bb);
            }
            stage[k] = v;
        }
        __syncthreads();
        const int shift = (int)(b0 - a0);
        const int nw = g.stride - 1;
        for (int rr = threadIdx.x; rr < nr; rr += blockDim.x) {
            const i64 ro = read_off[r0 + rr];
            const int len = (int)(read_off[r0 + rr + 1] - ro);
            uint32_t acc = 0;
            if (len > 0 && len <= MAX_READ_LEN) {
                const int o = shift + (int)(ro - b0), last = o + len - 1;
                const int d0 = o >> 2, d1 = last >> 2;
                for (int d = d0; d <= d1; ++d) {
                    uint32_t m = 0xFCFCFCFCu;
                    if (d == d0) m &= 0xFFFFFFFFu << (8 * (o & 3));
                    if (d == d1) m &= 0xFFFFFFFFu >> (8 * (3 - (last & 3)));
                    acc |= stage[d] & m;
                }
            }
            has_n[rr] = acc != 0;
        }
        __syncthreads();
        for (int wk = threadIdx.x; wk < nr * nw; wk += blockDim.x) {
            const int rr = wk / nw, k = wk - rr * nw;
            const i64 r = r0 + rr;
            const i64 ro = read_off[r];
            int len = (int)(read_off[r + 1] - ro);
            u64 v = 0;
            if (len > MAX_READ_LEN) len = 0;
            const int po = shift + (int)(ro - b0);
            const uint8_t* p = sb + po;
            if (k < 2 * g.W) {
                const bool rc = k >= g.W;
                const int w = rc ? k - g.W : k;
                const int nvalid = len - 32 * w;
                if (nvalid <= 0) v = 0;
                else if (!has_n[rr]) {
                    const int s0 = rc ? (nvalid >= 32 ? nvalid - 32 : 0) : 32 * w;
                    const int o = po + s0, dwi = o >> 2;
                    const unsigned sh = (unsigned)(o & 3);
                    uint32_t a[9];
#pragma unroll
                    for (int q = 0; q < 9; ++q) a[q] = stage[dwi + q];
                    if (!rc) {
#pragma unroll
                        for (int q = 0; q < 8; ++q) {
                            const uint32_t x = __builtin_amdgcn_alignbyte(a[q + 1], a[q], sh) & 0x03030303u;
                            v = (v << 8) | ((x * 0x40100401u) >> 24);
                        }
                        if (nvalid < 32) v &= ~0ull << (2 * (32 - nvalid));
                    } else {
#pragma unroll
                        for (int q = 7; q >= 0; --q) {
                            const uint32_t x = (__builtin_amdgcn_alignbyte(a[q + 1], a[q], sh) & 0x03030303u) ^ 0x03030303u;
                            v = (v << 8) | ((x * 0x01041040u) >> 24);
                        }
                        if (nvalid < 32) v <<= 2 * (32 - nvalid);
                    }
                } else {
#pragma unroll 16
                    for (int j = 0; j < 32; ++j) {
                        const int i = 32 * w + j;
                        u64 c = 0;
                        if (i < len) {
                            const uint8_t bb = rc ? p[len - 1 - i] : p[i];
                            c = bb < 4 ? (rc ? 3 - bb : bb) : 0;
                        }
                        v = (v << 2) | c;
                    }
                }
            } else if (has_n[rr]) {
                int m = k - 2 * g.W;
                const bool rc = m >= g.MW;
                if (rc) m -= g.MW;
                for (int j = 0; j < 64; ++j) {
                    const int i = 64 * m + j;
                    if (i < len) {
                        const uint8_t bb = rc ? p[len - 1 - i] : p[i];
                        if (bb >= 4) v |= 1ull << j;
                    }
                }
            }
            out[r * g.stride + k] = v;
        }
        __syncthreads();
        for (int rr = threadIdx.x; rr < nr; rr += blockDim.x) {
            const i64 r = r0 + rr;
            const int len = (int)(read_off[r + 1] - read_off[r]);
            out[r * g.stride + nw] = (u64)(unsigned)len | (has_n[rr] ? (1ull << 31) : 0ull);
        }
    }
}

enum Pc : int {
    PC_FETCH, PC_ALLPOS_TOP, PC_ZZ_TOP, PC_ZZ_RIGHT, PC_ZZ_END, PC_AFTER_STEP1, PC_R2_LOOP, PC_R2_AFTER, PC_R3_INIT,
    PC_R3_TOP, PC_DONE, PC_EXIT
};
enum Kind : int { K_S1_RIGHT, K_ZZ_LEFT, K_ZZ_RIGHT, K_OP_MEM, K_OP_SMEM, K_R3 };
enum Phase : int { PH_CTRL, PH_PART, PH_EDGE_DN, PH_EDGE_UP };

#ifndef CMP_WORDS
#define CMP_WORDS 2
#endif
typedef const __attribute__((address_space(3))) u64* lds_u64;
typedef __attribute__((address_space(3))) int* lds_int;
typedef __attribute__((address_space(3))) unsigned short* lds_u16;
typedef const __attribute__((address_space(1))) u64* glb_u64;
typedef const __attribute__((address_space(1))) SaEnt* glb_ent;
typedef const __attribute__((address_space(1))) Rmi32* glb_rmi;

#ifndef SEED_QUERY_LDS
#define SEED_QUERY_LDS 1
#endif
#ifndef SEED_USE_ERR
#define SEED_USE_ERR 1
#endif
#ifndef SEED_ALIGN_WIN
#define SEED_ALIGN_WIN 0
#endif
#if SEED_QUERY_LDS
typedef lds_u64 q_u64;
#else
typedef const __attribute__((address_space(1))) u64* q_u64;
#endif

__device__ __forceinline__ u64 ext_l(q_u64 w, int s) {
    int k = s >> 5, sh = (s & 31) * 2;
    u64 a = w[k], b = w[k + 1];
    return sh ? (a << sh) | (b >> (64 - sh)) : a;
}

constexpr int PLCP_WIN = 64;
typedef const __attribute__((address_space(3))) uint8_t* lds_u8;
__device__ __forceinline__ i64 plcp_win_fwd(i64 T0, int mid) { const i64 a = T0 + mid - 24; return (a < 0 ? 0 : a) & ~15ll; }
__device__ __forceinline__ i64 plcp_win_rev(i64 T0, int mid, i64 n) { const i64 a = n - 1 - (T0 + mid + 24); return (a < 0 ? 0 : a) & ~15ll; }

__device__ __forceinline__ u64 lowmask(int k) { return k >= 64 ? ~0ull : (k <= 0 ? 0ull : ((1ull << k) - 1ull)); }

enum StIdx : int { ST_BEFORE, ST_AFTER, ST_R2_K, ST_R2_NEXT, ST_R2_SAVED, ST_ZZ_NEXT, ST_ZZ_SP, ST_ZZ_GUARD, ST_AP_GUARD,
                   ST_SM_BASE, ST_N_SMEMS, ST_HITS_LO, ST_HITS_HI, ST_SEARCHES, ST_FLAGS, ST_LAST_CNT_LO, ST_LAST_CNT_HI,
                   ST_LAST_S_LO, ST_LAST_S_HI, ST_WINDOWS,
                   ST_L, ST_SE_LO, ST_SE_HI, ST_EE_LO, ST_EE_HI, ST_NB_LO, ST_NB_HI, ST_LF, ST_CB_LO, ST_CB_HI,
                   ST_TICKET_LO, ST_TICKET_HI, ST_WORDS };
enum StFlag : int { F_ZZ_CHECK = 1, F_ZZ_RET_ONEPOS = 2, F_REC = 4, F_LDS_OVF = 8 };
enum LevelFlag : int { LF_NEED_LO = 1, LF_NEED_HI = 2, LF_HAVE_LAST = 4 };

#ifndef WIN_E
#define WIN_E 3
#endif
#ifndef WIN_SLOTS
#define WIN_SLOTS 12
#endif
__host__ __device__ constexpr int win_entries(int G) { return (WIN_E * G > 64) ? 64 / G : (WIN_E * G < WIN_SLOTS ? WIN_SLOTS / G : WIN_E); }

constexpr int TICKET_CHUNK = 32;

__host__ __device__ inline size_t seed_lds_group_bytes(int G, int stride, int lcap) {
    const int groups = BLOCK / G;
    const int W = win_entries(G) * G;
    return (((size_t)groups * (SEED_QUERY_LDS ? stride * 8 : 0) + (size_t)groups * (2 * lcap + ST_WORDS + (W + 1) / 2) * sizeof(int)) + 7) & ~(size_t)7;
}
inline size_t seed_lds_bytes(int G, const PackGeom& geo, int lcap) {
    return seed_lds_group_bytes(G, geo.stride, lcap) + (size_t)(BLOCK / 64) * 16;
}

template <int E>
__device__ __forceinline__ void window_compare(glb_u64 pac, i64 n, q_u64 s, u64 wq, int off, int cap, const u64 (&ek)[E],
                                               const u64 (&ep)[E], int (&lcp)[E], bool (&less)[E]) {
    int l[E], Lc[E];
    bool lt[E];
    unsigned pend = 0;
    const i64 nlimit = n - (i64)cap;
#pragma unroll
    for (int e = 0; e < E; ++e) {
        Lc[e] = cap;
        if ((i64)ep[e] > nlimit) Lc[e] = (int)(n - (i64)ep[e]);
        const u64 x = ek[e] ^ wq;
        lt[e] = ek[e] < wq;
        l[e] = x ? (__clzll((long long)x) >> 1) : 32;
        if (!x && 32 < Lc[e]) pend |= 1u << e;
    }
    while (pend) {
        const int es = __ffs((int)pend) - 1;
        pend &= pend - 1;
        u64 pos = ep[0];
        int Ls = Lc[0];
#pragma unroll
        for (int e = 1; e < E; ++e)
            if (es == e) { pos = ep[e]; Ls = Lc[e]; }
        const i64 p0 = (i64)pos + 32;
        glb_u64 pw = pac + (p0 >> 5);
        const int sh = (int)(p0 & 31) * 2;
        int ll = 32;
        bool llt = false, done = false;
        for (int k = 1; !done; k += CMP_WORDS, pw += CMP_WORDS) {
            u64 w[CMP_WORDS + 1];
#pragma unroll
            for (int j = 0; j < CMP_WORDS + 1; ++j) w[j] = pw[j];
#pragma unroll
            for (int j = 0; j < CMP_WORDS; ++j) {
                if (done) break;
                const u64 wr = sh ? (w[j] << sh) | (w[j + 1] >> (64 - sh)) : w[j];
                const u64 q = ext_l(s, off + 32 * (k + j));
                const u64 y = wr ^ q;
                if (y) { ll += __clzll((long long)y) >> 1; llt = wr < q; done = true; }
                else { ll += 32; if (ll >= Ls) done = true; }
            }
        }
#pragma unroll
        for (int e = 0; e < E; ++e)
            if (es == e) { l[e] = ll; lt[e] = llt; }
    }
#pragma unroll
    for (int e = 0; e < E; ++e) {
        if (l[e] >= Lc[e]) { lcp[e] = Lc[e]; less[e] = (i64)ep[e] < nlimit; }
        else { lcp[e] = l[e]; less[e] = lt[e]; }
    }
}

__device__ __forceinline__ i64 rmi_lookup(glb_rmi l2, glb_rmi l1, i64 n_l1, int shift, i64 n, u64 key, u64& err_out) {
    u64 m = shift >= 64 ? 0ull : key >> shift;
    double icpt = l2[m].icpt, slope = l2[m].slope;
    u64 err = l2[m].err;
    double x = (double)key;
    double f = fma(slope, x, icpt);
    if (err >> 63) {
        u64 ps = (err >> 32) & 0x7fffffffull;
        double pn = (double)(err & 0xffffffffull) - 1.0;
        double c = f < 0.0 ? 0.0 : (f > pn ? pn : f);
        u64 j = ps + (u64)c;
        if (j >= (u64)n_l1) j = n_l1 > 0 ? (u64)n_l1 - 1 : 0;
        f = fma(l1[j].slope, x, l1[j].icpt);
        err = l1[j].err;
    }
    err_out = err;
    double top = (double)n - 1.0;
    if (f < 0.0) return 0;
    if (f > top) return n - 1;
    return (i64)f;
}

template <int G>
__device__ __forceinline__ int group_or(int v) {
    if constexpr (G >= 2) v |= __builtin_amdgcn_update_dpp(0, v, 0xB1, 0xF, 0xF, true);
    if constexpr (G >= 4) v |= __builtin_amdgcn_update_dpp(0, v, 0x4E, 0xF, 0xF, true);
    if constexpr (G >= 8) v |= __builtin_amdgcn_update_dpp(0, v, 0x141, 0xF, 0xF, true);
    if constexpr (G >= 16) v |= __builtin_amdgcn_update_dpp(0, v, 0x140, 0xF, 0xF, true);
    if constexpr (G >= 32) v |= __shfl_xor(v, 16);
    return v;
}

template <int G, int E>
__device__ __forceinline__ int slot_pair(const int (&v)[E], int t, int ia, int ib) {
    int x = 0;
#pragma unroll
    for (int e = 0; e < E; ++e) {
        const int j = e * G + t;
        x |= (j == ia) ? (v[e] << 16) : 0;
        x |= (j == ib) ? v[e] : 0;
    }
    return group_or<G>(x);
}

__device__ __forceinline__ bool is_n(q_u64 mask, int i) { return (mask[i >> 6] >> (i & 63)) & 1ull; }

__device__ __forceinline__ int first_n(q_u64 mask, bool has_n, int from, int l_seq) {
    if (!has_n) return l_seq;
    int w = from >> 6;
    u64 m = mask[w] & (~0ull << (from & 63));
    const int nw = (l_seq + 63) >> 6;
    for (;;) {
        if (m) {
            int p = w * 64 + __ffsll((long long)m) - 1;
            return p < l_seq ? p : l_seq;
        }
        if (++w >= nw) return l_seq;
        m = mask[w];
    }
}

template <int G>
#ifndef SEED_MIN_WAVES
#define SEED_MIN_WAVES 5
#endif
__global__ void __launch_bounds__(BLOCK, (G >= 4 ? SEED_MIN_WAVES : G)) k_seed(SeedArgs A) {
    extern __shared__ __attribute__((aligned(16))) unsigned char smem_raw[];
    constexpr int GROUPS = BLOCK / G;
    constexpr int E = win_entries(G);
    constexpr int W = E * G;
    constexpr u64 GFULL = (G == 64) ? ~0ull : ((1ull << G) - 1ull);
    constexpr u64 WFULL = (W == 64) ? ~0ull : ((1ull << W) - 1ull);
    const int lane = threadIdx.x & 63;
    const int gib = threadIdx.x / G;
    const int t = threadIdx.x & (G - 1);
    const int gbase = lane & ~(G - 1);
    const int stride = A.geo.stride, PW = A.geo.W, MW = A.geo.MW;
    const int cap = A.cap, lcap = A.lcap;
#if SEED_QUERY_LDS
    u64* rd = reinterpret_cast<u64*>(smem_raw) + (size_t)gib * stride;
    const q_u64 fw = (lds_u64)rd;
#else
    q_u64 fw = (q_u64)A.packed;
#endif
#define rcs (fw + PW)
#define nfw (fw + 2 * PW)
#define nrc (fw + 2 * PW + MW)
    const lds_int ring = (lds_int)(reinterpret_cast<int*>(smem_raw + (SEED_QUERY_LDS ? (size_t)GROUPS * stride * 8 : 0)) +
                                   (size_t)gib * (2 * lcap + ST_WORDS + (W + 1) / 2));
    const lds_int sm_se = ring;
    const lds_int sm_cnt = ring + lcap;
    const lds_int st = ring + 2 * lcap;
    const lds_u16 wl = (lds_u16)(st + ST_WORDS);
    const lds_int wv = (lds_int)(reinterpret_cast<int*>(smem_raw + seed_lds_group_bytes(G, stride, lcap)) + (threadIdx.x >> 6) * 4);
    const glb_ent sa = (glb_ent)A.I.sa;
    const glb_u64 pac = (glb_u64)A.I.pac;
    const glb_rmi l2 = (glb_rmi)A.I.l2, l1 = (glb_rmi)A.I.l1;
    const i64 n = A.I.n;
    const int hits_per_smem = A.opt.hits_per_smem;
#define GBALLOT(p_) ((__ballot(p_) >> gbase) & GFULL)
#define LD64(lo_) (((i64)st[(lo_) + 1] << 32) | (u64)(unsigned)st[lo_])
#define ST64(lo_, v_) do { const i64 v__ = (v_); st[lo_] = (int)(unsigned)(v__ & 0xffffffffll); st[(lo_) + 1] = (int)(v__ >> 32); } while (0)
#define FLAG(f_) ((st[ST_FLAGS] & (f_)) != 0)
#define SETFLAG(f_, v_) do { st[ST_FLAGS] = (v_) ? (st[ST_FLAGS] | (f_)) : (st[ST_FLAGS] & ~(f_)); } while (0)
#define LDS_HANDOFF() do { __builtin_amdgcn_fence(__ATOMIC_RELEASE, "wavefront"); __builtin_amdgcn_wave_barrier(); \
                           __builtin_amdgcn_fence(__ATOMIC_ACQUIRE, "wavefront"); } while (0)

    int pc = PC_FETCH, phase = PH_CTRL;
    int pivot = 0, l_seq = 0, msl = A.opt.min_seed_len, min_intv = 1;
    bool has_n = false;
    int q_kind = 0, q_mode = 0, off = 0, vlen = 0, capc = 0;
    bool q_rc = false, q_exact = false;
    i64 base = 0, lo = -1, hi = n;
    int stepk = 0;
    u64 wq = 0;
    unsigned acc_searches = 0, acc_windows = 0;
    if (lane == 0) wv[0] = TICKET_CHUNK;
    LDS_HANDOFF();

#ifdef SEED_PROF
    unsigned prof[8] = {0, 0, 0, 0, 0, 0, 0, 0};
    unsigned long long prof_t = wall_clock64();
#define PROF_MARK(i_) do { asm volatile("s_waitcnt vmcnt(0) lgkmcnt(0)" ::: "memory"); const unsigned long long now__ = wall_clock64(); prof[i_] += (unsigned)(now__ - prof_t); prof_t = now__; } while (0)
#else
#define PROF_MARK(i_) do { } while (0)
#endif
    for (;;) {
        bool newreq = false;
        if (phase == PH_CTRL) {
            bool have = false;
#define AT(pc_) (!have && pc == (pc_))
            do {
                if (AT(PC_ZZ_TOP)) {
                    if (st[ST_ZZ_SP] >= st[ST_ZZ_NEXT] || ++st[ST_ZZ_GUARD] > 4 * l_seq + 16) pc = PC_ZZ_END;
                    else if (FLAG(F_ZZ_CHECK) && has_n && is_n(nfw, st[ST_ZZ_SP])) {
                        if (l_seq - st[ST_ZZ_SP] < msl) { pivot = l_seq; st[ST_ZZ_SP] = l_seq; }
                        else { st[ST_ZZ_SP] += 1; pivot = pivot + 1; }
                    } else { q_kind = K_ZZ_LEFT; have = true; }
                }
                if (AT(PC_ZZ_RIGHT)) { q_kind = K_ZZ_RIGHT; have = true; }
                if (AT(PC_ZZ_END)) {
                    pivot = st[ST_ZZ_NEXT];
                    pc = FLAG(F_ZZ_RET_ONEPOS) ? PC_R2_AFTER : PC_AFTER_STEP1;
                }
                if (AT(PC_AFTER_STEP1)) {
                    SETFLAG(F_REC, false);
                    st[ST_AFTER] = st[ST_N_SMEMS];
                    if (A.opt.rounds < 2) pc = PC_ALLPOS_TOP;
                    else if (FLAG(F_LDS_OVF)) pc = PC_DONE;
                    else { st[ST_R2_K] = st[ST_BEFORE]; pc = PC_R2_LOOP; }
                }
                if (AT(PC_R2_AFTER)) {
                    min_intv = st[ST_R2_SAVED];
                    pivot = st[ST_R2_NEXT];
                    pc = PC_R2_LOOP;
                }
                if (AT(PC_R2_LOOP)) {
                    int k = st[ST_R2_K];
                    const int kb = st[ST_BEFORE], ke = st[ST_AFTER];
                    int qbeg = 0, qend = 0, cnt = 0;
                    bool take = false;
                    while (k < ke) {
                        const int se = sm_se[k - kb];
                        cnt = sm_cnt[k - kb];
                        qbeg = se & 0xffff; qend = (int)((unsigned)se >> 16);
                        ++k;
                        if (!(qend - qbeg < A.opt.split_len || cnt > A.opt.split_width)) { take = true; break; }
                    }
                    st[ST_R2_K] = k;
                    if (!take) pc = PC_ALLPOS_TOP;
                    else {
                        st[ST_R2_NEXT] = pivot; st[ST_R2_SAVED] = min_intv;
                        pivot = (qbeg + qend) >> 1;
                        min_intv = cnt + 1;
                        if (has_n && is_n(nfw, pivot)) {
                            pivot = (l_seq - pivot < msl) ? l_seq : pivot + 1;
                            pc = PC_R2_AFTER;
                        } else if (pivot != 0 && !(has_n && is_n(nfw, pivot - 1))) { q_kind = K_OP_MEM; have = true; }
                        else { q_kind = K_OP_SMEM; have = true; }
                    }
                }
                if (AT(PC_ALLPOS_TOP)) {
                    if (pivot >= l_seq || ++st[ST_AP_GUARD] > 4 * l_seq + 16) pc = PC_R3_INIT;
                    else {
                        st[ST_BEFORE] = st[ST_N_SMEMS]; st[ST_SM_BASE] = st[ST_BEFORE]; SETFLAG(F_REC, true);
                        if (has_n && is_n(nfw, pivot)) {
                            pivot = (l_seq - pivot < msl) ? l_seq : pivot + 1;
                            pc = PC_AFTER_STEP1;
                        } else if (pivot != 0 && !(has_n && is_n(nfw, pivot - 1))) {
                            st[ST_ZZ_NEXT] = l_seq; SETFLAG(F_ZZ_CHECK, true); SETFLAG(F_ZZ_RET_ONEPOS, false); st[ST_ZZ_SP] = pivot; st[ST_ZZ_GUARD] = 1;
                            q_kind = K_ZZ_LEFT; have = true;
                        } else { q_kind = K_S1_RIGHT; have = true; }
                    }
                }
                if (AT(PC_R3_INIT)) {
                    if (A.opt.rounds >= 3 && A.opt.max_mem_intv > 0 && !FLAG(F_LDS_OVF)) {
                        min_intv = A.opt.max_mem_intv;
                        msl = A.opt.min_seed_len + 1;
                        pivot = 0;
                        pc = PC_R3_TOP;
                    } else pc = PC_DONE;
                }
                if (AT(PC_R3_TOP)) {
                    for (;;) {
                        if (!(pivot < l_seq - msl + 1)) { pc = PC_DONE; break; }
                        if (has_n && is_n(nfw, pivot)) { pivot = pivot + 1; continue; }
                        const int valid = first_n(nfw, has_n, pivot, l_seq) - pivot;
                        if (valid < msl) { pivot = pivot + valid; continue; }
                        q_kind = K_R3; have = true;
                        break;
                    }
                }
                if (AT(PC_DONE)) {
                    const unsigned long long ticket = ((unsigned long long)(unsigned)st[ST_TICKET_HI] << 32) | (unsigned)st[ST_TICKET_LO];
                    const bool ovf = st[ST_N_SMEMS] > cap || FLAG(F_LDS_OVF);
                    if (t == 0) {
                        const i64 rid = A.pending ? A.pending[ticket] : (i64)ticket;
                        A.slot_cnt[rid] = ovf ? 0 : st[ST_N_SMEMS];
                        A.slot_hits[rid] = ovf ? 0 : LD64(ST_HITS_LO);
                        A.slot_loc[rid] = ((i64)A.tier << 40) | (i64)ticket;
                        if (ovf) A.ovf_list[atomicAdd(&A.counters[SEED_CTR_OVERFLOW], 1ull)] = rid;
                    }
                    if (!ovf) { acc_searches += (unsigned)st[ST_SEARCHES]; acc_windows += (unsigned)st[ST_WINDOWS]; }
                    pc = PC_FETCH;
                }
                if (AT(PC_FETCH)) {
                    int idx = TICKET_CHUNK;
                    if (t == 0) idx = __hip_atomic_fetch_add(wv, 1, __ATOMIC_RELAXED, __HIP_MEMORY_SCOPE_WAVEFRONT);
                    const u64 old_base = ((u64)(unsigned)wv[3] << 32) | (unsigned)wv[2];
                    const bool over = t == 0 && idx >= TICKET_CHUNK;
                    const unsigned long long mo = __ballot(over);
                    unsigned long long ticket = old_base + (unsigned)idx;
                    if (mo) {
                        const int first = __ffsll((long long)mo) - 1;
                        const int kreq = __popcll(mo), alloc = kreq > TICKET_CHUNK ? kreq : TICKET_CHUNK;
                        unsigned long long nb = 0;
                        if (lane == first) {
                            nb = atomicAdd(&A.counters[SEED_CTR_SLOT], (unsigned long long)alloc);
                            const unsigned long long wb = nb + (unsigned)(alloc - TICKET_CHUNK);
                            wv[0] = kreq - (alloc - TICKET_CHUNK); wv[2] = (int)(unsigned)(wb & 0xffffffffull); wv[3] = (int)(wb >> 32);
                        }
                        nb = __shfl(nb, first);
                        if (over) ticket = nb + (unsigned)__popcll(mo & ((1ull << lane) - 1ull));
                    }
                    ticket = __shfl(ticket, gbase);
                    if (ticket >= (unsigned long long)A.nreads) pc = PC_EXIT;
                    else {
                        const i64 rid = A.pending ? A.pending[ticket] : (i64)ticket;
                        const u64* src = A.packed + rid * stride;
#if SEED_QUERY_LDS
                        const int lw = (stride - 1) % G;
                        u64 lenw = 0;
                        for (int k = t; k < stride; k += G) {
                            u64 v = src[k];
                            rd[k] = v;
                            if (k == stride - 1) lenw = v;
                        }
                        lenw = (u64)(unsigned)__shfl((int)lenw, gbase + lw);
#else
                        fw = (q_u64)src;
                        const u64 lenw = fw[stride - 1];
#endif
                        l_seq = (int)(lenw & 0x7fffffffull);
                        has_n = ((lenw >> 31) & 1ull) != 0;
                        for (int k = t; k < ST_WORDS; k += G) st[k] = 0;
                        LDS_HANDOFF();
                        if (l_seq <= 0 || l_seq > MAX_READ_LEN) {
                            if (t == 0) { A.slot_cnt[rid] = l_seq > MAX_READ_LEN ? -1 : 0; A.slot_hits[rid] = 0; A.slot_loc[rid] = 0; }
                        } else {
                            st[ST_TICKET_LO] = (int)(unsigned)(ticket & 0xffffffffull);
                            st[ST_TICKET_HI] = (int)(ticket >> 32);
                            pivot = 0; msl = A.opt.min_seed_len; min_intv = 1;
                            pc = PC_ALLPOS_TOP;
                            if (!(has_n && is_n(nfw, 0))) {
                                st[ST_AP_GUARD] = 1; SETFLAG(F_REC, true);
                                q_kind = K_S1_RIGHT; have = true;
                            }
                        }
                    }
                }
            } while (!have && pc != PC_EXIT);
#undef AT
            if (pc == PC_EXIT) {
                if (t == 0) {
                    atomicAdd(&A.counters[SEED_CTR_SEARCHES], (unsigned long long)acc_searches); atomicAdd(&A.counters[SEED_CTR_WINDOWS], (unsigned long long)acc_windows);
#ifdef SEED_PROF
                    for (int k = 0; k < 8; ++k) atomicAdd(&A.counters[SEED_CTR_PROF + k], (unsigned long long)prof[k]);
#endif
                }
                break;
            }
            newreq = true;
        }
        PROF_MARK(0);
        if (newreq) {
            q_rc = q_kind == K_ZZ_LEFT;
            off = q_rc ? l_seq - 1 - pivot : pivot;
            vlen = first_n(q_rc ? nrc : nfw, has_n, off, l_seq) - off;
            q_exact = q_kind == K_S1_RIGHT || q_kind == K_ZZ_RIGHT || q_kind == K_OP_SMEM;
            q_mode = q_kind == K_R3 ? 2 : ((q_exact || min_intv != 1) ? 1 : 0);
            st[ST_SEARCHES] = st[ST_SEARCHES] + 1;
            wq = ext_l(q_rc ? rcs : fw, off);
            u64 key = wq;
            if (vlen < 32) key |= (~0ull) >> (2 * vlen);
            u64 err;
            const i64 pos = rmi_lookup(l2, l1, A.I.n_l1, A.I.shift, n, key, err);
#if SEED_USE_ERR
            const i64 below = (i64)((err >> 32) & 0x3fffffffull) + 1, above = (i64)(err & 0x7fffffffull);
            const i64 span = below + above + 1;
            base = span <= W ? pos - below - (W - span) / 2 : pos - (below * W) / span;
#else
            base = pos - W / 2;
#endif
#if SEED_ALIGN_WIN
            if constexpr (W % 4 == 0) base = (base + 2) & ~3ll;
#endif
            if (base < 0) base = 0;
            if (base > n - W) base = n - W;
            lo = -1; hi = n; stepk = 0; capc = vlen;
            phase = PH_PART;
        }
        PROF_MARK(1);

        const q_u64 s = q_rc ? rcs : fw;
        int lcp[E];
        bool less[E];
        u64 ep[E];
        {
            u64 ek[E];
#pragma unroll
            for (int e = 0; e < E; ++e) { ek[e] = sa[base + e * G + t].key; ep[e] = sa[base + e * G + t].pos; }
            st[ST_WINDOWS] = st[ST_WINDOWS] + 1;
            window_compare<E>(pac, n, s, wq, off, capc, ek, ep, lcp, less);
        }
        PROF_MARK(2);
        u64 m = 0;
#pragma unroll
        for (int e = 0; e < E; ++e) {
            const bool p = phase == PH_PART ? less[e] : ((lcp[e] >= capc) == (phase == PH_EDGE_UP));
            m |= GBALLOT(p) << (e * G);
        }
        if (stepk != 0)
            m = (m | lowmask((int)((lo - base + 1 > W) ? W : (lo - base + 1 < 0 ? 0 : lo - base + 1)))) &
                lowmask((int)((hi - base > W) ? W : (hi - base < 0 ? 0 : hi - base)));
        const int P = __popcll(m);
        const bool at_lo = base == 0 || (phase == PH_EDGE_UP && base == lo + 1);
        const bool at_hi = base + W == n || (phase == PH_EDGE_DN && base + W == hi);
        const bool found = (P > 0 && P < W) || (P == 0 && at_lo) || (P == W && at_hi);

        bool go_level = false, finished = false;
        int L = 0, nb_lo = 0, nb_hi = 0, lf = 0;
        i64 s_edge = 0, e_edge = 0, cb = base;
        int r_L = 0;
        i64 r_start = 0, r_count = 1, r_T = -1;
        bool r_emit = false;
        int cl[E];
        bool cache_in_lds = phase != PH_PART;
        if (found) {
            const int v2 = slot_pair<G, E>(lcp, t, P - 1, P);
            const int lm = P > 0 ? (v2 >> 16) : -1;
            const int lp = P < W ? (v2 & 0xffff) : -1;
            if (phase == PH_PART) {
                const int c = (lm >= lp) ? P - 1 : P;
                L = lm >= lp ? lm : lp;
                r_L = L; r_start = base + c; r_count = 1;
                if (q_exact || q_kind == K_R3) {
                    u64 tc = 0;
#pragma unroll
                    for (int e = 0; e < E; ++e) tc = (e * G + t == c) ? ep[e] : tc;
                    r_T = (i64)(((u64)(unsigned)group_or<G>((int)(tc >> 32)) << 32) | (u64)(unsigned)group_or<G>((int)(unsigned)tc));
                }
                if (q_mode == 0 || (q_mode == 2 && L < msl)) finished = true;
                else {
                    s_edge = e_edge = base + c;
                    lf = LF_NEED_LO | LF_NEED_HI;
                    go_level = true;
                }
            } else {
                L = st[ST_L]; nb_lo = st[ST_NB_LO]; nb_hi = st[ST_NB_HI]; lf = st[ST_LF];
                s_edge = LD64(ST_SE_LO); e_edge = LD64(ST_EE_LO); cb = LD64(ST_CB_LO);
                if (phase == PH_EDGE_DN) { s_edge = base + P; nb_lo = P > 0 ? lm : 0; lf &= ~LF_NEED_LO; }
                else { e_edge = base + P - 1; nb_hi = P < W ? lp : 0; lf &= ~LF_NEED_HI; }
                go_level = true;
            }
        } else {
            if (P == W) lo = base + W - 1; else hi = base;
            bool stop = false;
            if (phase != PH_PART && !q_exact) {
                s_edge = LD64(ST_SE_LO); e_edge = LD64(ST_EE_LO);
                if (phase == PH_EDGE_DN ? (e_edge - hi + 1 >= (i64)min_intv) : (lo - s_edge + 1 >= (i64)min_intv)) {
                    L = st[ST_L]; nb_lo = st[ST_NB_LO]; nb_hi = st[ST_NB_HI]; lf = st[ST_LF]; cb = LD64(ST_CB_LO);
                    if (phase == PH_EDGE_DN) { s_edge = hi; nb_lo = L; lf &= ~LF_NEED_LO; }
                    else { e_edge = lo; nb_hi = L; lf &= ~LF_NEED_HI; }
                    stop = go_level = true;
                }
            }
            if (!stop) {
                if (lo < 0) { base = hi - ((i64)W << stepk); ++stepk; if (base < 0) base = 0; }
                else if (hi >= n) { base = lo + 1 + (((i64)W << stepk) - W); ++stepk; if (base > n - W) base = n - W; }
                else if (hi - lo <= W - 1) { base = lo; if (base > n - W) base = n - W; }
                else base = lo + (hi - lo) / 2 - W / 2;
            }
        }
        PROF_MARK(3);
        if (go_level) {
#pragma unroll
            for (int e = 0; e < E; ++e) cl[e] = cache_in_lds ? (int)wl[e * G + t] : lcp[e];
            for (;;) {
                if (lf & (LF_NEED_LO | LF_NEED_HI)) {
                    u64 ge = 0;
#pragma unroll
                    for (int e = 0; e < E; ++e) ge |= GBALLOT(cl[e] >= L) << (e * G);
                    const u64 nz = ~ge & WFULL;
                    const i64 klo = s_edge - cb;
                    const i64 khi = e_edge - cb;
                    const bool in_lo = (lf & LF_NEED_LO) && klo > 0 && klo <= W;
                    const bool in_hi = (lf & LF_NEED_HI) && khi >= -1 && khi < W - 1;
                    const u64 zlo = in_lo ? (nz & lowmask((int)klo)) : 0ull;
                    const u64 zhi = in_hi ? (nz & ~lowmask((int)khi + 1)) : 0ull;
                    const int hz = zlo ? 63 - __clzll((long long)zlo) : -1;
                    const int lz = zhi ? __ffsll((long long)zhi) - 1 : -1;
                    const int nb2 = slot_pair<G, E>(cl, t, hz, lz);
                    if (lf & LF_NEED_LO) {
                        if (in_lo) {
                            if (zlo) { s_edge = cb + hz + 1; nb_lo = nb2 >> 16; lf &= ~LF_NEED_LO; }
                            else { s_edge = cb; if (cb == 0) { nb_lo = 0; lf &= ~LF_NEED_LO; } }
                        } else if (s_edge == 0) { nb_lo = 0; lf &= ~LF_NEED_LO; }
                    }
                    if (lf & LF_NEED_HI) {
                        if (in_hi) {
                            if (zhi) { e_edge = cb + lz - 1; nb_hi = nb2 & 0xffff; lf &= ~LF_NEED_HI; }
                            else { e_edge = cb + W - 1; if (cb + W >= n) { nb_hi = 0; lf &= ~LF_NEED_HI; } }
                        } else if (e_edge == n - 1) { nb_hi = 0; lf &= ~LF_NEED_HI; }
                    }
                    if (lf & LF_NEED_LO) {
                        phase = PH_EDGE_DN; lo = -1; hi = s_edge; stepk = 1;
                        base = s_edge - W; if (base < 0) base = 0;
                        break;
                    }
                    if (lf & LF_NEED_HI) {
                        phase = PH_EDGE_UP; lo = e_edge; hi = n; stepk = 1;
                        base = e_edge + 1; if (base > n - W) base = n - W;
                        break;
                    }
                }
                const i64 cnt = e_edge - s_edge + 1;
                const int nxt = nb_lo > nb_hi ? nb_lo : nb_hi;
                if (q_mode == 1) {
                    if (cnt >= (i64)min_intv) { r_L = L; r_start = s_edge; r_count = cnt; finished = true; break; }
                } else {
                    if (cnt >= (i64)min_intv) {
                        if (lf & LF_HAVE_LAST) { r_count = LD64(ST_LAST_CNT_LO); r_start = LD64(ST_LAST_S_LO); }
                        else { r_count = cnt; r_start = s_edge; }
                        r_L = L + 1;
                        finished = true;
                        break;
                    }
                    if (nxt < msl) { r_L = msl; r_start = s_edge; r_count = cnt; finished = true; break; }
                    lf |= LF_HAVE_LAST;
                    ST64(ST_LAST_CNT_LO, cnt);
                    ST64(ST_LAST_S_LO, s_edge);
                }
                L = nxt;
                lf = (lf & LF_HAVE_LAST) | ((nb_lo >= L && s_edge > 0) ? LF_NEED_LO : 0) | ((nb_hi >= L && e_edge < n - 1) ? LF_NEED_HI : 0);
            }
            if (finished) {
                if (q_mode == 2) {
                    r_emit = r_count < (i64)min_intv;
                    if (r_L < msl) r_L = msl;
                }
            } else {
                capc = L;
                st[ST_L] = L; st[ST_NB_LO] = nb_lo; st[ST_NB_HI] = nb_hi; st[ST_LF] = lf;
                ST64(ST_SE_LO, s_edge); ST64(ST_EE_LO, e_edge); ST64(ST_CB_LO, cb);
                if (!cache_in_lds) {
#pragma unroll
                    for (int e = 0; e < E; ++e) wl[e * G + t] = (unsigned short)cl[e];
                }
            }
        }
        PROF_MARK(4);
        if (finished) {
            bool emit = false;
            const int e_start = pivot;
            int e_end = pivot;
            switch (q_kind) {
            case K_S1_RIGHT:
            case K_ZZ_RIGHT:
            case K_OP_SMEM:
                emit = r_L >= msl; e_end = pivot + r_L;
                break;
            case K_ZZ_LEFT:
                pivot = pivot - r_L + 1;
                pc = (st[ST_ZZ_NEXT] - pivot < msl) ? PC_ZZ_END : PC_ZZ_RIGHT;
                break;
            case K_OP_MEM:
                st[ST_ZZ_NEXT] = pivot + r_L; SETFLAG(F_ZZ_CHECK, false); SETFLAG(F_ZZ_RET_ONEPOS, true); st[ST_ZZ_SP] = pivot; st[ST_ZZ_GUARD] = 0;
                pc = PC_ZZ_TOP;
                break;
            default:
                emit = r_emit; e_end = pivot + r_L;
                break;
            }
            if (emit) {
                const int ns = st[ST_N_SMEMS];
                const bool have_pos = r_count == 1 && r_T >= 0 && !cache_in_lds;
                const bool defer = have_pos && A.defer != 0 && FLAG(F_REC) && ns < DEFER_MAX_K && ns < cap && A.opt.rounds >= 2 &&
                                   e_end - e_start >= A.opt.split_len && A.opt.split_width >= 1 && nb_lo < msl && nb_hi < msl;
                if (ns < cap && t == 0) {
                    const unsigned long long ticket = ((unsigned long long)(unsigned)st[ST_TICKET_HI] << 32) | (unsigned)st[ST_TICKET_LO];
                    SlotRec sr;
                    sr.start = e_start; sr.end = e_end; sr.count = r_count;
                    sr.sa_start = have_pos ? (SLOT_POS | (defer ? SLOT_DEFER : 0ll) | r_T) : r_start;
                    A.slots[(i64)ticket * cap + ns] = sr;
                }
                if (FLAG(F_REC)) {
                    const int k = ns - st[ST_SM_BASE];
                    if (k < lcap) {
                        sm_se[k] = e_start | (e_end << 16);
                        sm_cnt[k] = (defer || r_count > (i64)INT_MAX) ? INT_MAX : (int)r_count;
                    } else SETFLAG(F_LDS_OVF, true);
                }
                st[ST_N_SMEMS] = ns + 1;
                i64 h = r_count;
                if (hits_per_smem > 0 && h > hits_per_smem) h = hits_per_smem;
                h += LD64(ST_HITS_LO);
                ST64(ST_HITS_LO, h);
            }
            switch (q_kind) {
            case K_S1_RIGHT: pivot = pivot + r_L; pc = PC_AFTER_STEP1; break;
            case K_ZZ_RIGHT: pivot = pivot + r_L; st[ST_ZZ_SP] = pivot; pc = PC_ZZ_TOP; break;
            case K_OP_SMEM: pivot = pivot + r_L; pc = PC_R2_AFTER; break;
            case K_R3: pivot = pivot + (r_L < msl ? msl : r_L); pc = PC_R3_TOP; break;
            default: break;
            }
            phase = PH_CTRL;
        }
        PROF_MARK(5);
    }
#undef PROF_MARK
#undef rcs
#undef nfw
#undef nrc
#undef GBALLOT
#undef LD64
#undef ST64
#undef FLAG
#undef SETFLAG
#undef LDS_HANDOFF
}


__device__ __forceinline__ u64 ext_g(const u64* __restrict__ w, int s) {
    const int k = s >> 5, sh = (s & 31) * 2;
    const u64 a = w[k], b = w[k + 1];
    return sh ? (a << sh) | (b >> (64 - sh)) : a;
}

struct LaneQuery {
    const u64* s;
    int off, vlen;
    u64 wq;
};

__device__ __forceinline__ void lane_compare_ent(const DevIndex& I, const LaneQuery& q, int cap, const SaEnt e, int& lcp, bool& less) {
    const i64 nlimit = I.n - (i64)cap;
    int Lc = cap;
    if ((i64)e.pos > nlimit) Lc = (int)(I.n - (i64)e.pos);
    const u64 x = e.key ^ q.wq;
    bool lt = e.key < q.wq;
    int l = x ? (__clzll((long long)x) >> 1) : 32;
    if (!x && 32 < Lc) {
        const i64 p0 = (i64)e.pos + 32;
        for (int k = 1;; ++k) {
            const u64 wr = extract32(I.pac, p0 + 32 * (k - 1));
            const u64 qq = ext_g(q.s, q.off + 32 * k);
            const u64 y = wr ^ qq;
            if (y) { l += __clzll((long long)y) >> 1; lt = wr < qq; break; }
            l += 32;
            if (l >= Lc) break;
        }
    }
    if (l >= Lc) { lcp = Lc; less = (i64)e.pos < nlimit; }
    else { lcp = l; less = lt; }
}
__device__ __forceinline__ void lane_compare(const DevIndex& I, const LaneQuery& q, int cap, i64 slot, int& lcp, bool& less) {
    lane_compare_ent(I, q, cap, I.sa[slot], lcp, less);
}

constexpr int LANE_W = 16;
struct LaneWin {
    uint32_t* lw;
    i64 base;
    __device__ __forceinline__ bool has(i64 slot) const { return base >= 0 && slot >= base && slot < base + LANE_W; }
    __device__ __forceinline__ int get(i64 slot) const { const int i = (int)(slot - base); return (int)((lw[(i >> 1) * 256] >> (16 * (i & 1))) & 0xffffu); }
};
__device__ __forceinline__ int lane_lcp(const DevIndex& I, const LaneQuery& q, const LaneWin& C, int cap, i64 slot) {
    if (C.has(slot)) return C.get(slot);
    int lc; bool ls;
    lane_compare(I, q, cap, slot, lc, ls);
    return lc;
}

__device__ __forceinline__ void lane_search(const DevIndex& I, const LaneQuery& q, int min_intv, uint32_t* lw, int& r_L, i64& r_start, i64& r_count) {
    const i64 n = I.n;
    u64 key = q.wq;
    if (q.vlen < 32) key |= (~0ull) >> (2 * q.vlen);
    u64 err;
    const i64 p = rmi_lookup((glb_rmi)I.l2, (glb_rmi)I.l1, I.n_l1, I.shift, n, key, err);
    LaneWin C; C.lw = lw; C.base = -1;
    int L = 0;
    i64 s = 0, e = 0;
    bool located = false;
    int lc; bool ls;
    {
        const i64 below = (i64)((err >> 32) & 0x3fffffffull) + 1, above = (i64)(err & 0x7fffffffull);
        const i64 span = below + above + 1;
        i64 base = span <= LANE_W ? p - below - (LANE_W - span) / 2 : p - (below * LANE_W) / span;
        if (base < 0) base = 0;
        if (base > n - LANE_W) base = n - LANE_W;
        SaEnt ent[LANE_W];
#pragma unroll
        for (int k = 0; k < LANE_W; ++k) ent[k] = I.sa[base + k];
        unsigned lessm = 0;
        int prev = 0;
#pragma unroll
        for (int k = 0; k < LANE_W; ++k) {
            lane_compare_ent(I, q, q.vlen, ent[k], lc, ls);
            lessm |= (ls ? 1u : 0u) << k;
            if (k & 1) lw[(k >> 1) * 256] = (uint32_t)prev | ((uint32_t)lc << 16); else prev = lc;
        }
        C.base = base;
        const int P = __popc(lessm);
        if (lessm == ((1u << P) - 1u) && ((P > 0 && P < LANE_W) || (P == 0 && base == 0) || (P == LANE_W && base + LANE_W == n))) {
            const int lm = P > 0 ? C.get(base + P - 1) : -1, lp = P < LANE_W ? C.get(base + P) : -1;
            L = lm >= lp ? lm : lp;
            s = e = base + (lm >= lp ? P - 1 : P);
            located = true;
        }
    }
    if (!located) {
        i64 lo = -1, hi = n;
        lane_compare(I, q, q.vlen, p, lc, ls);
        if (ls) {
            lo = p;
            for (i64 st = 1; hi == n && lo < n - 1; st <<= 1) {
                i64 pr = lo + st; if (pr > n - 1) pr = n - 1;
                lane_compare(I, q, q.vlen, pr, lc, ls);
                if (ls) lo = pr; else hi = pr;
            }
        } else {
            hi = p;
            for (i64 st = 1; lo == -1 && hi > 0; st <<= 1) {
                i64 pr = hi - st; if (pr < 0) pr = 0;
                lane_compare(I, q, q.vlen, pr, lc, ls);
                if (ls) lo = pr; else hi = pr;
            }
        }
        while (hi - lo > 1) {
            const i64 mid = lo + (hi - lo) / 2;
            lane_compare(I, q, q.vlen, mid, lc, ls);
            if (ls) lo = mid; else hi = mid;
        }
        const i64 P = hi;
        const int lm = P > 0 ? lane_lcp(I, q, C, q.vlen, P - 1) : -1, lp = P < n ? lane_lcp(I, q, C, q.vlen, P) : -1;
        L = lm >= lp ? lm : lp;
        s = e = lm >= lp ? P - 1 : P;
    }
    for (;;) {
        while (s > 0 && C.has(s - 1) && C.get(s - 1) >= L) --s;
        if (s > 0 && !C.has(s - 1)) {
            i64 good = s, bad = -1;
            for (i64 st = 1; good > 0; st <<= 1) {
                i64 pr = good - st; if (pr < 0) pr = 0;
                if (lane_lcp(I, q, C, L, pr) >= L) good = pr; else { bad = pr; break; }
            }
            while (bad >= 0 && good - bad > 1) {
                const i64 mid = bad + (good - bad) / 2;
                if (lane_lcp(I, q, C, L, mid) >= L) good = mid; else bad = mid;
            }
            s = good;
        }
        while (e < n - 1 && C.has(e + 1) && C.get(e + 1) >= L) ++e;
        if (e < n - 1 && !C.has(e + 1)) {
            i64 good = e, bad = n;
            for (i64 st = 1; good < n - 1; st <<= 1) {
                i64 pr = good + st; if (pr > n - 1) pr = n - 1;
                if (lane_lcp(I, q, C, L, pr) >= L) good = pr; else { bad = pr; break; }
            }
            while (bad < n && bad - good > 1) {
                const i64 mid = good + (bad - good) / 2;
                if (lane_lcp(I, q, C, L, mid) >= L) good = mid; else bad = mid;
            }
            e = good;
        }
        if (e - s + 1 >= (i64)min_intv) break;
        const int nlo = s > 0 ? lane_lcp(I, q, C, L, s - 1) : 0, nhi = e < n - 1 ? lane_lcp(I, q, C, L, e + 1) : 0;
        L = nlo > nhi ? nlo : nhi;
    }
    r_L = L; r_start = s; r_count = e - s + 1;
}

__device__ __forceinline__ int first_n_g(const u64* __restrict__ mask, bool has_n, int from, int l_seq) {
    if (!has_n) return l_seq;
    int w = from >> 6;
    u64 m = mask[w] & (~0ull << (from & 63));
    const int nw = (l_seq + 63) >> 6;
    for (;;) {
        if (m) { const int p = w * 64 + __ffsll((long long)m) - 1; return p < l_seq ? p : l_seq; }
        if (++w >= nw) return l_seq;
        m = mask[w];
    }
}

struct PlcpView {
    const uint8_t* __restrict__ plcp;
    const uint32_t* win;
    i64 F0, R0;
    __device__ __forceinline__ int at(i64 pos, i64 w0, int dw0) const {
        const i64 d = pos - w0;
        if (d >= 0 && d < PLCP_WIN) return (int)((win[(dw0 + (int)(d >> 2)) * 256] >> (8 * (int)(d & 3))) & 0xffu);
        return (int)plcp[pos];
    }
    __device__ __forceinline__ int fwd(i64 pos) const { return at(pos, F0, 0); }
    __device__ __forceinline__ int rev(i64 pos) const { return at(pos, R0, PLCP_WIN / 4); }
};

struct BlkRec {
    i64 rid;
    int k;
    int pivot, next, guard;
    int stage;
    int r_L;
    i64 r_start, r_count;
};

struct ReseedArgs {
    DevIndex I;
    const u64* packed;
    PackGeom geo;
    i64 nreads;
    meme_seed_opt opt;
    SlotRec* slots;
    int cap;
    int* slot_cnt;
    i64* slot_hits;
    i64* ovf_list;
    unsigned long long* counters;
    i64* pend_list;
    BlkRec* blk;
    BlkRec* blk_out;
    i64 blk_cap;
    int blk_ctr, blk_out_ctr;
};

template <bool OWNED>
struct SmemAppender {
    SlotRec* sl; int cap; int* cnt; i64* hits; i64* ovf_list; unsigned long long* counters; i64 rid; int hps;
    int ns; i64 hits_add;
    __device__ __forceinline__ void push(int start, int end, i64 sa_start, i64 count) {
        const i64 h = (hps > 0 && count > hps) ? (i64)hps : count;
        if (OWNED) {
            if (ns < cap) { SlotRec sr; sr.start = start; sr.end = end; sr.sa_start = sa_start; sr.count = count; sl[ns] = sr; }
            ++ns; hits_add += h;
        } else {
            const int at = atomicAdd(cnt, 1);
            if (at < cap) { SlotRec sr; sr.start = start; sr.end = end; sr.sa_start = sa_start; sr.count = count; sl[at] = sr; }
            else if (at == cap) ovf_list[atomicAdd(&counters[SEED_CTR_OVERFLOW], 1ull)] = rid;
            atomicAdd(reinterpret_cast<unsigned long long*>(hits), (unsigned long long)h);
        }
    }
};

struct RegionState { int pivot, next, guard, stage; };

template <bool OWNED>
__device__ __forceinline__ bool region_walk(const PlcpView& V, i64 n, i64 T0, int qbeg, int qend, int l_seq, int msl, RegionState& S, unsigned& hops,
                                            SmemAppender<OWNED>& ap, int& n_pend) {
    for (;;) {
        if (S.stage == 0) {
            const int plc = V.fwd(T0 + S.pivot);
            if (plc == 0 || plc == 255 || plc >= qend - S.pivot) return true;
            ++hops; S.next = S.pivot + plc; S.stage = 1;
        }
        if (S.stage == 1) {
            if (S.pivot >= S.next || ++S.guard > 4 * l_seq + 16) { S.stage = 3; return false; }
            const int plc = (S.pivot >= qbeg && S.pivot < qend) ? V.rev(n - 1 - (T0 + S.pivot)) : 0;
            if (plc == 0 || plc == 255 || plc >= S.pivot - qbeg + 1) return true;
            ++hops; S.pivot = S.pivot - plc + 1;
            if (S.next - S.pivot < msl) { S.stage = 3; return false; }
            S.stage = 2;
        }
        const int plc = (S.pivot >= qbeg && S.pivot < qend) ? V.fwd(T0 + S.pivot) : 0;
        if (plc == 0 || plc == 255 || plc >= qend - S.pivot) return true;
        if (plc >= msl) {
            if (!OWNED) return true;
            ap.push(S.pivot, S.pivot + plc, SLOT_PEND, 0);
            ++n_pend;
        }
        ++hops; S.pivot = S.pivot + plc; S.stage = 1;
    }
}

__device__ __forceinline__ LaneQuery region_query(const u64* __restrict__ rec, const PackGeom& geo, int l_seq, bool has_n, const RegionState& S) {
    LaneQuery q;
    const bool left = S.stage == 1;
    q.s = rec + (left ? geo.W : 0);
    q.off = left ? l_seq - 1 - S.pivot : S.pivot;
    q.vlen = first_n_g(rec + 2 * geo.W + (left ? geo.MW : 0), has_n, q.off, l_seq) - q.off;
    q.wq = ext_g(q.s, q.off);
    return q;
}

template <bool OWNED>
__device__ __forceinline__ void region_apply(RegionState& S, int msl, int r_L, i64 r_start, i64 r_count, SmemAppender<OWNED>& ap) {
    if (S.stage == 0) { S.next = S.pivot + r_L; S.stage = 1; }
    else if (S.stage == 1) { S.pivot = S.pivot - r_L + 1; S.stage = (S.next - S.pivot < msl) ? 3 : 2; }
    else {
        if (r_L >= msl) ap.push(S.pivot, S.pivot + r_L, r_start, r_count);
        S.pivot = S.pivot + r_L; S.stage = 1;
    }
}

__device__ __forceinline__ void stage_plcp_windows(const uint8_t* __restrict__ plcp, const PlcpView& V, uint32_t* win) {
    uint4 v[2 * (PLCP_WIN / 16)];
#pragma unroll
    for (int q = 0; q < PLCP_WIN / 16; ++q) {
        v[q] = *reinterpret_cast<const uint4*>(plcp + V.F0 + 16 * q);
        v[PLCP_WIN / 16 + q] = *reinterpret_cast<const uint4*>(plcp + V.R0 + 16 * q);
    }
#pragma unroll
    for (int q = 0; q < 2 * (PLCP_WIN / 16); ++q) {
        win[(4 * q + 0) * 256] = v[q].x; win[(4 * q + 1) * 256] = v[q].y; win[(4 * q + 2) * 256] = v[q].z; win[(4 * q + 3) * 256] = v[q].w;
    }
}

constexpr int BLK_PER_READ = 1;
constexpr int BLK_MORE = 16;

__global__ void __launch_bounds__(256) k_reseed(ReseedArgs A) {
    __shared__ uint32_t win[2 * (PLCP_WIN / 4) * 256];
    __shared__ unsigned long long blk_hops, blk_lane;
    __shared__ unsigned blk_pend, blk_pend_base, blk_blk;
    __shared__ unsigned long long blk_blk_base;
    const uint8_t* __restrict__ plcp = A.I.plcp;
    const i64 n = A.I.n;
    const int msl = A.opt.min_seed_len, cap = A.cap;
    for (i64 r0 = (i64)blockIdx.x * blockDim.x; r0 < A.nreads; r0 += (i64)gridDim.x * blockDim.x) {
        if (threadIdx.x == 0) { blk_hops = 0; blk_lane = 0; blk_pend = 0; blk_blk = 0; }
        __syncthreads();
        const i64 r = r0 + threadIdx.x;
        unsigned hops = 0, lsearches = 0;
        int n_pend = 0, n_blk = 0, pend_ns = 0;
        BlkRec held[BLK_PER_READ];
        if (r < A.nreads) {
            const int c0 = A.slot_cnt[r];
            const int c = c0 > DEFER_MAX_K ? DEFER_MAX_K : c0;
            SlotRec* sl = A.slots + r * cap;
            const u64* rec = A.packed + r * A.geo.stride;
            SmemAppender<true> ap;
            ap.sl = sl; ap.cap = cap; ap.hps = A.opt.hits_per_smem; ap.ns = c0; ap.hits_add = 0; ap.rid = r;
            int l_seq = 0;
            int k = -1;
            for (;;) {
                i64 f = 0;
                for (++k; k < c; ++k) { f = sl[k].sa_start; if (f & SLOT_DEFER) break; }
                if (k >= c) break;
                if (l_seq == 0) { const u64 lw = rec[A.geo.stride - 1]; l_seq = (int)(lw & 0x7fffffffull); }
                const int qbeg = sl[k].start, qend = sl[k].end;
                const i64 T0 = (f & SLOT_VAL) - qbeg;
                PlcpView V;
                V.plcp = plcp; V.win = win + threadIdx.x;
                RegionState S;
                S.pivot = (qbeg + qend) >> 1; S.next = 0; S.guard = 0; S.stage = 0;
                V.F0 = plcp_win_fwd(T0, S.pivot); V.R0 = plcp_win_rev(T0, S.pivot, n);
                stage_plcp_windows(plcp, V, win + threadIdx.x);
                if (region_walk<true>(V, n, T0, qbeg, qend, l_seq, msl, S, hops, ap, n_pend)) {
                    BlkRec b;
                    b.rid = r; b.k = k; b.pivot = S.pivot; b.next = S.next; b.guard = S.guard; b.r_L = 0; b.r_start = 0; b.r_count = 0;
                    b.stage = S.stage | (n_blk == BLK_PER_READ - 1 ? BLK_MORE : 0);
#pragma unroll
                    for (int i = 0; i < BLK_PER_READ; ++i) if (i == n_blk) held[i] = b;
                    if (++n_blk == BLK_PER_READ) break;
                }
            }
            if (ap.ns != c0) {
                if (ap.ns > cap) {
                    A.slot_cnt[r] = 0; A.slot_hits[r] = 0;
                    A.ovf_list[atomicAdd(&A.counters[SEED_CTR_OVERFLOW], 1ull)] = r;
                    n_pend = 0; n_blk = 0;
                } else { A.slot_cnt[r] = ap.ns; A.slot_hits[r] = A.slot_hits[r] + ap.hits_add; pend_ns = ap.ns; }
            }
        }
        unsigned my_pend = 0, my_blk = 0;
        if (n_pend) my_pend = atomicAdd(&blk_pend, 1u);
        if (n_blk) my_blk = atomicAdd(&blk_blk, (unsigned)n_blk);
        if (hops | lsearches) { atomicAdd(&blk_hops, (unsigned long long)(hops + lsearches)); if (lsearches) atomicAdd(&blk_lane, (unsigned long long)lsearches); }
        __syncthreads();
        if (threadIdx.x == 0) {
            if (blk_hops) atomicAdd(&A.counters[SEED_CTR_SEARCHES], blk_hops);
            if (blk_lane) atomicAdd(&A.counters[SEED_CTR_LANE], blk_lane);
            if (blk_pend) blk_pend_base = (unsigned)atomicAdd(&A.counters[SEED_CTR_PEND], (unsigned long long)blk_pend);
            if (blk_blk) blk_blk_base = atomicAdd(&A.counters[A.blk_ctr], (unsigned long long)blk_blk);
        }
        __syncthreads();
        if (n_pend) A.pend_list[blk_pend_base + my_pend] = r | ((i64)pend_ns << 40);
#pragma unroll
        for (int i = 0; i < BLK_PER_READ; ++i)
            if (i < n_blk) {
                const unsigned long long at = blk_blk_base + my_blk + i;
                if ((i64)at < A.blk_cap) A.blk[at] = held[i];
            }
        __syncthreads();
    }
}

__global__ void __launch_bounds__(256) k_reseed_emit(ReseedArgs A) {
    __shared__ uint32_t lwin[(LANE_W / 2) * 256];
    const i64 n_list = (i64)A.counters[SEED_CTR_PEND];
    for (i64 i = (i64)blockIdx.x * blockDim.x + threadIdx.x; i < n_list; i += (i64)gridDim.x * blockDim.x) {
        const i64 ent = A.pend_list[i];
        const i64 r = ent & ((1ll << 40) - 1);
        const int c = (int)(ent >> 40);
        SlotRec* sl = A.slots + r * A.cap;
        const u64* rec = A.packed + r * A.geo.stride;
        i64 hits_add = 0;
        int k = -1;
        for (;;) {
            for (++k; k < c; ++k) if (sl[k].sa_start & SLOT_PEND) break;
            if (k >= c) break;
            LaneQuery q;
            q.s = rec; q.off = sl[k].start; q.vlen = sl[k].end - sl[k].start;
            q.wq = ext_g(q.s, q.off);
            int r_L; i64 r_start, r_count;
            lane_search(A.I, q, 1, lwin + threadIdx.x, r_L, r_start, r_count);
            sl[k].sa_start = r_start; sl[k].count = r_count;
            hits_add += (A.opt.hits_per_smem > 0 && r_count > A.opt.hits_per_smem) ? (i64)A.opt.hits_per_smem : r_count;
        }
        atomicAdd(reinterpret_cast<unsigned long long*>(A.slot_hits + r), (unsigned long long)hits_add);
    }
}

__global__ void __launch_bounds__(256) k_reseed_search(ReseedArgs A) {
    __shared__ uint32_t lwin[(LANE_W / 2) * 256];
    i64 n_blk = (i64)A.counters[A.blk_ctr];
    if (n_blk > A.blk_cap) n_blk = A.blk_cap;
    for (i64 i = (i64)blockIdx.x * blockDim.x + threadIdx.x; i < n_blk; i += (i64)gridDim.x * blockDim.x) {
        BlkRec b = A.blk[i];
        const u64* rec = A.packed + b.rid * A.geo.stride;
        const u64 lw = rec[A.geo.stride - 1];
        RegionState S;
        S.pivot = b.pivot; S.next = b.next; S.guard = b.guard; S.stage = b.stage & ~BLK_MORE;
        const LaneQuery q = region_query(rec, A.geo, (int)(lw & 0x7fffffffull), ((lw >> 31) & 1ull) != 0, S);
        lane_search(A.I, q, 2, lwin + threadIdx.x, b.r_L, b.r_start, b.r_count);
        A.blk[i].r_L = b.r_L; A.blk[i].r_start = b.r_start; A.blk[i].r_count = b.r_count;
    }
}

template <bool LAST>
__global__ void __launch_bounds__(256) k_reseed_resume(ReseedArgs A) {
    __shared__ uint32_t win[2 * (PLCP_WIN / 4) * 256];
    __shared__ uint32_t lwin[(LANE_W / 2) * 256];
    __shared__ unsigned long long acc_total, acc_lane, out_base;
    __shared__ unsigned out_n;
    const uint8_t* __restrict__ plcp = A.I.plcp;
    const i64 n = A.I.n;
    const int msl = A.opt.min_seed_len;
    if (threadIdx.x == 0) { acc_total = 0; acc_lane = 0; }
    i64 n_blk = (i64)A.counters[A.blk_ctr];
    if (n_blk > A.blk_cap) n_blk = A.blk_cap;
    unsigned total = 0, lsearches = 0;
    for (i64 i0 = (i64)blockIdx.x * blockDim.x; i0 < n_blk; i0 += (i64)gridDim.x * blockDim.x) {
        if (threadIdx.x == 0) out_n = 0;
        __syncthreads();
        const i64 i = i0 + threadIdx.x;
        bool blocked = false;
        BlkRec nb;
        if (i < n_blk) {
            const BlkRec b = A.blk[i];
            const i64 r = b.rid;
            SlotRec* sl = A.slots + r * A.cap;
            const u64* rec = A.packed + r * A.geo.stride;
            const u64 lw = rec[A.geo.stride - 1];
            const int l_seq = (int)(lw & 0x7fffffffull);
            const bool has_n = ((lw >> 31) & 1ull) != 0;
            SmemAppender<false> ap;
            ap.sl = sl; ap.cap = A.cap; ap.cnt = A.slot_cnt + r; ap.hits = A.slot_hits + r; ap.ovf_list = A.ovf_list; ap.counters = A.counters; ap.rid = r;
            ap.hps = A.opt.hits_per_smem; ap.ns = 0; ap.hits_add = 0;
            unsigned hops = 1;
            int k = b.k;
            const int c = (b.stage & BLK_MORE) ? (A.slot_cnt[r] > DEFER_MAX_K ? DEFER_MAX_K : A.slot_cnt[r]) : 0;
            bool first = true;
            for (;;) {
                const int qbeg = sl[k].start, qend = sl[k].end;
                const i64 T0 = (sl[k].sa_start & SLOT_VAL) - qbeg;
                PlcpView V;
                V.plcp = plcp; V.win = win + threadIdx.x;
                V.F0 = plcp_win_fwd(T0, (qbeg + qend) >> 1); V.R0 = plcp_win_rev(T0, (qbeg + qend) >> 1, n);
                stage_plcp_windows(plcp, V, win + threadIdx.x);
                RegionState S;
                if (first) {
                    S.pivot = b.pivot; S.next = b.next; S.guard = b.guard; S.stage = b.stage & ~BLK_MORE;
                    region_apply<false>(S, msl, b.r_L, b.r_start, b.r_count, ap);
                    first = false;
                } else { S.pivot = (qbeg + qend) >> 1; S.next = 0; S.guard = 0; S.stage = 0; }
                while (S.stage != 3) {
                    int n_pend = 0;
                    if (!region_walk<false>(V, n, T0, qbeg, qend, l_seq, msl, S, hops, ap, n_pend)) break;
                    if (!LAST) {
                        nb.rid = r; nb.k = k; nb.pivot = S.pivot; nb.next = S.next; nb.guard = S.guard; nb.stage = S.stage | (b.stage & BLK_MORE);
                        nb.r_L = 0; nb.r_start = 0; nb.r_count = 0;
                        blocked = true;
                        break;
                    }
                    const LaneQuery q = region_query(rec, A.geo, l_seq, has_n, S);
                    int r_L; i64 r_start, r_count;
                    lane_search(A.I, q, 2, lwin + threadIdx.x, r_L, r_start, r_count);
                    ++lsearches; ++hops;
                    region_apply<false>(S, msl, r_L, r_start, r_count, ap);
                }
                if (blocked) break;
                for (++k; k < c; ++k) if ((sl[k].sa_start & (SLOT_DEFER | SLOT_POS)) == (SLOT_DEFER | SLOT_POS)) break;
                if (k >= c) break;
            }
            total += hops;
        }
        unsigned my = 0;
        if (blocked) my = atomicAdd(&out_n, 1u);
        __syncthreads();
        if (threadIdx.x == 0 && out_n) out_base = atomicAdd(&A.counters[A.blk_out_ctr], (unsigned long long)out_n);
        __syncthreads();
        if (blocked) A.blk_out[out_base + my] = nb;
        __syncthreads();
    }
    if (total) atomicAdd(&acc_total, (unsigned long long)total);
    if (lsearches) atomicAdd(&acc_lane, (unsigned long long)lsearches);
    __syncthreads();
    if (threadIdx.x == 0) {
        if (acc_total) atomicAdd(&A.counters[SEED_CTR_SEARCHES], acc_total);
        if (acc_lane) atomicAdd(&A.counters[SEED_CTR_LANE], acc_lane);
    }
}

}
```

Baseline: 150.4 million reads/s.

## Replace multi-round reseed pipeline with persistent work-stealing kernel and per-wave read packing

```diff
diff --git a/bwa-meme_amd/csrc/meme_common.h b/bwa-meme_amd/csrc/meme_common.h
--- a/bwa-meme_amd/csrc/meme_common.h
+++ b/bwa-meme_amd/csrc/meme_common.h
@@ -140,7 +140,6 @@
     HostBuf h_smems, h_hits, h_smem_off, h_hit_off;
     unsigned long long* counter_set(int cset) { return (unsigned long long*)counters.p + SEED_CTRS * cset; }
     Events<SEED_EVS> ev;
-    Stream emit; Events<2> emit_ev;
 };
 struct ChainWs {
     DevBuf ch1, sd1, hdr, frac, contigs, counts, chains, seeds, lists;
@@ -189,7 +188,10 @@
     ChainWs chain; ExtWs ext; BswWs bsw; GcigWs gcig; KswvWs kswv; MateWs mate; SamWs sam; SeedWs seed;
     Stream stream;
     SideStreams side;
+    int pack_per_cu = 0; size_t pack_per_cu_lds = 0;
+    int reseed_per_cu = 0;
     i64 seed_blocks = 0;
+    i64 reseed_blocks = 0;
     i64 smem_cap = 128;
     i64 group_lanes = 4;
     i64 seed_blocks_per_cu = 5;
diff --git a/bwa-meme_amd/csrc/meme_ctx.hip b/bwa-meme_amd/csrc/meme_ctx.hip
--- a/bwa-meme_amd/csrc/meme_ctx.hip
+++ b/bwa-meme_amd/csrc/meme_ctx.hip
@@ -82,7 +82,7 @@
 extern "C" void meme_ctx_destroy(meme_ctx* ctx) {
     if (!ctx) return;
     (void)hipSetDevice(ctx->device);
-    for (hipStream_t st : {ctx->stream.s, ctx->side.st[0].s, ctx->side.st[1].s, ctx->side.st[2].s, ctx->seed.emit.s})
+    for (hipStream_t st : {ctx->stream.s, ctx->side.st[0].s, ctx->side.st[1].s, ctx->side.st[2].s})
         if (st) (void)hipStreamSynchronize(st);
     if (ctx->owns_index) for (auto& o : ctx->owned) (void)hipFree(o.first);
     if (ctx->plcp_aux) (void)hipFree(ctx->plcp_aux);
@@ -126,9 +126,10 @@
     if (!ctx || !key) return MEME_E_ARG;
     if (!strcmp(key, "gcig_groups") && value != 0 && value != 1) { meme_set_error("gcig_groups must be 0 or 1"); return MEME_E_ARG; }
     if (!strcmp(key, "group_lanes") && value != 1 && value != 2 && value != 4 && value != 8 && value != 16 && value != 32) { meme_set_error("group_lanes must be 1, 2, 4, 8, 16 or 32"); return MEME_E_ARG; }
+    if (!strcmp(key, "reseed_blocks") && (value < 0 || value > 65536)) { meme_set_error("reseed_blocks must be 0 (as many workgroups as are resident) or 1 .. 65536"); return MEME_E_ARG; }
     const i64 any = INT64_MIN;
     static const struct { const char* key; i64 meme_ctx::*member; i64 at_least; } keys[] = {
-        {"seed_blocks", &meme_ctx::seed_blocks, any}, {"smem_cap", &meme_ctx::smem_cap, 8}, {"seed_defer", &meme_ctx::seed_defer, any}, {"max_batch", &meme_ctx::max_batch, any},
+        {"seed_blocks", &meme_ctx::seed_blocks, any}, {"reseed_blocks", &meme_ctx::reseed_blocks, 0}, {"smem_cap", &meme_ctx::smem_cap, 8}, {"seed_defer", &meme_ctx::seed_defer, any}, {"max_batch", &meme_ctx::max_batch, any},
         {"sam_max_batch", &meme_ctx::sam_max_batch, any}, {"bsw_circ", &meme_ctx::bsw_circ, any}, {"ext_split", &meme_ctx::ext_split, any}, {"ext_slab_jobs", &meme_ctx::ext_slab_jobs, 1},
         {"ext_census", &meme_ctx::ext_census, any}, {"gcig_zcap", &meme_ctx::gcig_zcap, any}, {"gcig_groups", &meme_ctx::gcig_groups, any}, {"ext_live_only", &meme_ctx::ext_live_only, any},
         {"ext_rounds", &meme_ctx::ext_rounds, 0}, {"bsw_blocks", &meme_ctx::bsw_blocks, any}, {"bsw_lane_min_pairs", &meme_ctx::bsw_lane_min_pairs, any},
diff --git a/bwa-meme_amd/csrc/meme_seed.hip b/bwa-meme_amd/csrc/meme_seed.hip
--- a/bwa-meme_amd/csrc/meme_seed.hip
+++ b/bwa-meme_amd/csrc/meme_seed.hip
@@ -195,14 +195,21 @@
     int rc;
     if ((rc = meme_buf_reserve(ctx, ctx->batch.packed, (size_t)R.nreads * geo.stride * 8))) return rc;
     HIP_TRY(hipEventRecord(ctx->seed.ev[SEED_EV_PACK0], ctx->stream));
-    int rb = (int)((48 * 1024) / max_len);
-    if (rb > 32) rb = 32;
-    if (rb < 1) rb = 1;
-    i64 pblocks = (R.nreads + rb - 1) / rb;
-    if (pblocks > (i64)ctx->n_cus * 16) pblocks = (i64)ctx->n_cus * 16;
-    size_t plds = ((size_t)rb * (size_t)max_len + 16 + 48 + 3) & ~(size_t)3;
+    int rt = (int)((12 * 1024) / max_len);
+    if (rt > 32) rt = 32;
+    if (rt < 1) rt = 1;
+    const i64 ntiles = (R.nreads + rt - 1) / rt;
+    const size_t plds = (size_t)4 * pack_wave_lds(rt, (int)max_len);
+    if (ctx->pack_per_cu == 0 || ctx->pack_per_cu_lds != plds) {
+        int nb = 0;
+        HIP_TRY(hipOccupancyMaxActiveBlocksPerMultiprocessor(&nb, (const void*)k_pack_reads, 256, plds));
+        ctx->pack_per_cu = nb > 0 ? nb : 1; ctx->pack_per_cu_lds = plds;
+    }
+    i64 pblocks = (ntiles + 3) / 4;
+    if (pblocks > (i64)ctx->n_cus * ctx->pack_per_cu) pblocks = (i64)ctx->n_cus * ctx->pack_per_cu;
+    if (pblocks < 1) pblocks = 1;
     hipLaunchKernelGGL(k_pack_reads, dim3((unsigned)pblocks), dim3(256), plds, ctx->stream, d_reads,
-                       R.d_read_off, R.nreads, total_bytes, geo, rb, (u64*)ctx->batch.packed.p);
+                       R.d_read_off, R.nreads, total_bytes, geo, rt, (int)max_len, (u64*)ctx->batch.packed.p);
     HIP_TRY(hipGetLastError());
     HIP_TRY(hipEventRecord(ctx->seed.ev[SEED_EV_PACK1], ctx->stream));
     return MEME_OK;
@@ -299,28 +306,21 @@
     A.I = ctx->idx; A.packed = (const u64*)ctx->batch.packed.p; A.geo = R.geo; A.nreads = nreads; A.opt = *R.opt;
     A.slots = (SlotRec*)S.slots[0].p; A.cap = (int)ctx->smem_cap; A.slot_cnt = (int*)S.slot_cnt.p; A.slot_hits = (i64*)S.slot_hits.p;
     A.ovf_list = (i64*)S.ovf[0].p; A.counters = S.counter_set(0); A.pend_list = (i64*)S.pend.p;
-    A.blk = (BlkRec*)S.blk.p; A.blk_out = A.blk + nreads * BLK_PER_READ; A.blk_cap = nreads * BLK_PER_READ;
-    A.blk_ctr = SEED_CTR_BLK; A.blk_out_ctr = SEED_CTR_BLK_OUT;
+    A.blk = (BlkRec*)S.blk.p; A.blk_cap = nreads * BLK_PER_READ;
     i64 rblocks = (nreads + 255) / 256;
     if (rblocks > (i64)ctx->n_cus * 32) rblocks = (i64)ctx->n_cus * 32;
     hipLaunchKernelGGL(k_reseed, dim3((unsigned)rblocks), dim3(256), 0, ctx->stream, A);
     HIP_TRY(hipEventRecord(ctx->side.fork[0], ctx->stream));
-    const unsigned sblocks = (unsigned)(rblocks < (i64)ctx->n_cus * 4 ? rblocks : (i64)ctx->n_cus * 4);
-    if (!S.emit.s) HIP_TRY(hipStreamCreateWithFlags(&S.emit.s, hipStreamNonBlocking));
-    for (int i = 0; i < 2; ++i) if (!S.emit_ev[i]) HIP_TRY(hipEventCreateWithFlags(&S.emit_ev[i], hipEventDisableTiming));
-    HIP_TRY(hipEventRecord(S.emit_ev[0], ctx->stream));
-    HIP_TRY(hipStreamWaitEvent(S.emit, S.emit_ev[0], 0));
-    hipLaunchKernelGGL(k_reseed_emit, dim3(sblocks), dim3(256), 0, S.emit, A);
-    HIP_TRY(hipEventRecord(S.emit_ev[1], S.emit));
-    constexpr int ROUNDS = 4;
-    for (int round = 0; round < ROUNDS; ++round) {
-        hipLaunchKernelGGL(k_reseed_search, dim3(sblocks), dim3(256), 0, ctx->stream, A);
-        if (round < ROUNDS - 1) {
-            hipLaunchKernelGGL(k_reseed_resume<false>, dim3(sblocks), dim3(256), 0, ctx->stream, A);
-            HIP_TRY(hipMemsetAsync(S.counter_set(0) + A.blk_ctr, 0, sizeof(unsigned long long), ctx->stream));
-            std::swap(A.blk, A.blk_out); std::swap(A.blk_ctr, A.blk_out_ctr);
-        } else hipLaunchKernelGGL(k_reseed_resume<true>, dim3(sblocks), dim3(256), 0, ctx->stream, A);
-    }
+    if (ctx->reseed_per_cu == 0) {
+        int nb = 0;
+        HIP_TRY(hipOccupancyMaxActiveBlocksPerMultiprocessor(&nb, (const void*)k_reseed_jobs, 256, 0));
+        ctx->reseed_per_cu = nb > 0 ? nb : 1;
+    }
+    i64 jblocks = (i64)ctx->n_cus * ctx->reseed_per_cu;
+    const i64 jmax = (nreads * (BLK_PER_READ + 1) + 255) / 256;
+    if (jblocks > jmax) jblocks = jmax;
+    if (ctx->reseed_blocks > 0) jblocks = ctx->reseed_blocks;
+    hipLaunchKernelGGL(k_reseed_jobs, dim3((unsigned)jblocks), dim3(256), 0, ctx->stream, A);
     HIP_TRY(hipGetLastError());
     return MEME_OK;
 }
@@ -347,11 +347,10 @@
     int rc;
     R.defer = ctx->seed_defer != 0 && ctx->idx.plcp != nullptr && R.opt->rounds >= 2;
     if (R.defer && (rc = meme_buf_reserve(ctx, S.pend, (size_t)R.nreads * sizeof(i64)))) return rc;
-    if (R.defer && (rc = meme_buf_reserve(ctx, S.blk, (size_t)R.nreads * BLK_PER_READ * 2 * sizeof(BlkRec)))) return rc;
+    if (R.defer && (rc = meme_buf_reserve(ctx, S.blk, (size_t)R.nreads * BLK_PER_READ * sizeof(BlkRec)))) return rc;
     if ((rc = launch_tier(R, 0, R.nreads, nullptr, 0, ctx->stream, R.defer))) return rc;
     if (R.defer) {
         if ((rc = meme_side_stream(ctx, 0)) || (rc = launch_reseed(R)) || (rc = launch_early_overflow(R))) return rc;
-        HIP_TRY(hipStreamWaitEvent(ctx->stream, S.emit_ev[1], 0));
     }
     HIP_TRY(hipEventRecord(S.ev[SEED_EV_SEARCH1], ctx->stream));
     unsigned long long h[SEED_CTRS];
@@ -568,7 +567,7 @@
     ChainWs& C = ctx->chain; ExtWs& E = ctx->ext;
     struct { DevBuf* b; size_t bytes; } dev[] = {
         {&B.reads, (size_t)total_bases + 16}, {&B.read_off, (n + 1) * 8}, {&S.slot_cnt, n * 4}, {&S.slot_hits, n * 8},
-        {&S.slot_loc, n * 8}, {&S.counters, 2 * SEED_CTRS * 8}, {&S.pend, n * 8}, {&S.blk, n * BLK_PER_READ * 2 * sizeof(BlkRec)}, {&B.packed, n * stride * 8}, {&S.slots[0], n * (size_t)ctx->smem_cap * sizeof(SlotRec)},
+        {&S.slot_loc, n * 8}, {&S.counters, 2 * SEED_CTRS * 8}, {&S.pend, n * 8}, {&S.blk, n * BLK_PER_READ * sizeof(BlkRec)}, {&B.packed, n * stride * 8}, {&S.slots[0], n * (size_t)ctx->smem_cap * sizeof(SlotRec)},
         {&B.smem_off, (n + 1) * 8}, {&B.hit_off, (n + 1) * 8}, {&B.smems, n * 12 * sizeof(meme_mem_tl)}, {&B.hits, n * 24 * 8},
         {&C.chains, n * 3 * sizeof(meme_chain)}, {&C.seeds, n * 6 * sizeof(meme_chain_seed)}};
     for (auto& d : dev) if ((rc = meme_buf_reserve(ctx, *d.b, d.bytes))) return rc;
diff --git a/bwa-meme_amd/csrc/meme_seed_kernel.h b/bwa-meme_amd/csrc/meme_seed_kernel.h
--- a/bwa-meme_amd/csrc/meme_seed_kernel.h
+++ b/bwa-meme_amd/csrc/meme_seed_kernel.h
@@ -51,65 +51,101 @@
     int defer;
 };
 
+constexpr int PACK_LD = 6;
+__device__ __forceinline__ void pack_wave_sync() {
+    __builtin_amdgcn_fence(__ATOMIC_RELEASE, "wavefront"); __builtin_amdgcn_wave_barrier(); __builtin_amdgcn_fence(__ATOMIC_ACQUIRE, "wavefront");
+}
+__host__ __device__ inline int pack_stage_bytes(int rt, int max_len) { return (rt * max_len + 15 + 48 + 15) & ~15; }
+__host__ __device__ inline int pack_wave_lds(int rt, int max_len) { return ((rt * 8 + 15) & ~15) + pack_stage_bytes(rt, max_len); }
+
 __global__ void __launch_bounds__(256) k_pack_reads(const uint8_t* __restrict__ reads, const i64* __restrict__ read_off,
-                                                     i64 nreads, i64 total_bytes, PackGeom g, int PACK_RB,
+                                                     i64 nreads, i64 total_bytes, PackGeom g, int PACK_RT, int max_len,
                                                      u64* __restrict__ out) {
     extern __shared__ __attribute__((aligned(16))) unsigned char pk_raw[];
-    uint32_t* stage = reinterpret_cast<uint32_t*>(pk_raw);
-    const uint8_t* sb = pk_raw;
-    __shared__ int has_n[64];
-    for (i64 r0 = (i64)blockIdx.x * PACK_RB; r0 < nreads; r0 += (i64)gridDim.x * PACK_RB) {
-        const int nr = (int)(nreads - r0 < PACK_RB ? nreads - r0 : PACK_RB);
-        const i64 b0 = read_off[r0], b1 = read_off[r0 + nr];
-        const i64 a0 = b0 & ~3ll;
-        const int ndw = (int)((b1 - a0 + 3) >> 2);
-        __syncthreads();
-        const uint32_t* src = reinterpret_cast<const uint32_t*>(reads + a0);
-        for (int k = threadIdx.x; k < ndw; k += blockDim.x) {
-            uint32_t v;
-            if (a0 + 4 * (i64)k + 4 <= total_bytes) v = src[k];
-            else {
-                v = 0;
-                for (int bb = 0; bb < 4; ++bb)
-                    if (a0 + 4 * (i64)k + bb < total_bytes) v |= (uint32_t)reads[a0 + 4 * (i64)k + bb] << (8 * bb);
-            }
-            stage[k] = v;
-        }
-        __syncthreads();
-        const int shift = (int)(b0 - a0);
-        const int nw = g.stride - 1;
-        for (int rr = threadIdx.x; rr < nr; rr += blockDim.x) {
-            const i64 ro = read_off[r0 + rr];
-            const int len = (int)(read_off[r0 + rr + 1] - ro);
-            uint32_t acc = 0;
-            if (len > 0 && len <= MAX_READ_LEN) {
-                const int o = shift + (int)(ro - b0), last = o + len - 1;
-                const int d0 = o >> 2, d1 = last >> 2;
-                for (int d = d0; d <= d1; ++d) {
-                    uint32_t m = 0xFCFCFCFCu;
-                    if (d == d0) m &= 0xFFFFFFFFu << (8 * (o & 3));
-                    if (d == d1) m &= 0xFFFFFFFFu >> (8 * (3 - (last & 3)));
-                    acc |= stage[d] & m;
-                }
-            }
-            has_n[rr] = acc != 0;
-        }
-        __syncthreads();
-        for (int wk = threadIdx.x; wk < nr * nw; wk += blockDim.x) {
-            const int rr = wk / nw, k = wk - rr * nw;
-            const i64 r = r0 + rr;
-            const i64 ro = read_off[r];
-            int len = (int)(read_off[r + 1] - ro);
+    const int lane = threadIdx.x & 63, wave = threadIdx.x >> 6;
+    unsigned char* const wbase = pk_raw + (size_t)wave * pack_wave_lds(PACK_RT, max_len);
+    int2* const meta = reinterpret_cast<int2*>(wbase);
+    unsigned char* const sb = wbase + ((PACK_RT * 8 + 15) & ~15);
+    uint32_t* const stage = reinterpret_cast<uint32_t*>(sb);
+    const int cap16 = pack_stage_bytes(PACK_RT, max_len) >> 4;
+    const int stride = g.stride, nw = stride - 1;
+    const int rr0 = lane / stride, k0 = lane - rr0 * stride, drr = 64 / stride, dk = 64 - drr * stride;
+    const i64 ntiles = (nreads + PACK_RT - 1) / PACK_RT;
+    const unsigned align0 = (unsigned)(reinterpret_cast<uintptr_t>(reads) & 15);
+    for (i64 tile = (i64)blockIdx.x * 4 + wave; tile < ntiles; tile += (i64)gridDim.x * 4) {
+        const i64 r0 = tile * PACK_RT;
+        const int nr = (int)(nreads - r0 < PACK_RT ? nreads - r0 : PACK_RT);
+        const i64 my_off = lane <= nr ? read_off[r0 + lane] : 0;
+        const i64 nx_off = __shfl_down(my_off, 1);
+        const i64 b0 = __shfl(my_off, 0), b1 = __shfl(my_off, nr);
+        const i64 a0 = b0 - (i64)((align0 + (unsigned)(b0 & 15)) & 15);
+        int n16 = (int)((b1 - a0 + 15) >> 4);
+        if (n16 > cap16) n16 = cap16;
+        pack_wave_sync();
+        if (lane < nr) { int2 mt; mt.x = (int)(my_off - a0); mt.y = (int)(nx_off - my_off); meta[lane] = mt; }
+        uint32_t nacc = 0;
+        for (int c0 = 0; c0 < n16; c0 += 64 * PACK_LD) {
+            uint4 v[PACK_LD];
+#pragma unroll
+            for (int u = 0; u < PACK_LD; ++u) {
+                const int c = c0 + 64 * u + lane;
+                const i64 o = a0 + 16 * (i64)c;
+                v[u] = make_uint4(0, 0, 0, 0);
+                if (c < n16) {
+                    if (o >= 0 && o + 16 <= total_bytes) v[u] = *reinterpret_cast<const uint4*>(reads + o);
+                    else {
+                        uint32_t d[4] = {0, 0, 0, 0};
+                        for (int bb = 0; bb < 16; ++bb)
+                            if (o + bb >= 0 && o + bb < total_bytes) d[bb >> 2] |= (uint32_t)reads[o + bb] << (8 * (bb & 3));
+                        v[u] = make_uint4(d[0], d[1], d[2], d[3]);
+                    }
+                }
+            }
+#pragma unroll
+            for (int u = 0; u < PACK_LD; ++u) {
+                const int c = c0 + 64 * u + lane;
+                if (c < n16) *reinterpret_cast<uint4*>(sb + 16 * c) = v[u];
+                nacc |= (v[u].x | v[u].y | v[u].z | v[u].w) & 0xFCFCFCFCu;
+            }
+        }
+        pack_wave_sync();
+        if (__ballot(nacc != 0)) {
+            if (lane < nr) {
+                const int2 mt = meta[lane];
+                const int len = mt.y;
+                uint32_t acc = 0;
+                if (len > 0 && len <= MAX_READ_LEN) {
+                    const int o = mt.x, last = o + len - 1;
+                    const int d0 = o >> 2, d1 = last >> 2;
+                    for (int d = d0; d <= d1; ++d) {
+                        uint32_t m = 0xFCFCFCFCu;
+                        if (d == d0) m &= 0xFFFFFFFFu << (8 * (o & 3));
+                        if (d == d1) m &= 0xFFFFFFFFu >> (8 * (3 - (last & 3)));
+                        acc |= stage[d] & m;
+                    }
+                }
+                if (acc) meta[lane].y = len | (int)0x80000000u;
+            }
+            pack_wave_sync();
+        }
+        u64* const otile = out + r0 * stride;
+        const int nout = nr * stride;
+        int rr = rr0, k = k0;
+        for (int wk = lane; wk < nout; wk += 64) {
+            const int2 mt = meta[rr];
+            const int po = mt.x;
+            const bool hasn = mt.y < 0;
+            const int rlen = mt.y & 0x7fffffff;
+            int len = rlen;
+            if (len > MAX_READ_LEN) len = 0;
+            const uint8_t* p = sb + po;
             u64 v = 0;
-            if (len > MAX_READ_LEN) len = 0;
-            const int po = shift + (int)(ro - b0);
-            const uint8_t* p = sb + po;
             if (k < 2 * g.W) {
                 const bool rc = k >= g.W;
                 const int w = rc ? k - g.W : k;
                 const int nvalid = len - 32 * w;
                 if (nvalid <= 0) v = 0;
-                else if (!has_n[rr]) {
+                else if (!hasn) {
                     const int s0 = rc ? (nvalid >= 32 ? nvalid - 32 : 0) : 32 * w;
                     const int o = po + s0, dwi = o >> 2;
                     const unsigned sh = (unsigned)(o & 3);
@@ -143,7 +179,8 @@
                         v = (v << 2) | c;
                     }
                 }
-            } else if (has_n[rr]) {
+            } else if (k == nw) v = (u64)(unsigned)rlen | (hasn ? (1ull << 31) : 0ull);
+            else if (hasn) {
                 int m = k - 2 * g.W;
                 const bool rc = m >= g.MW;
                 if (rc) m -= g.MW;
@@ -155,13 +192,9 @@
                     }
                 }
             }
-            out[r * g.stride + k] = v;
-        }
-        __syncthreads();
-        for (int rr = threadIdx.x; rr < nr; rr += blockDim.x) {
-            const i64 r = r0 + rr;
-            const int len = (int)(read_off[r + 1] - read_off[r]);
-            out[r * g.stride + nw] = (u64)(unsigned)len | (has_n[rr] ? (1ull << 31) : 0ull);
+            otile[wk] = v;
+            rr += drr; k += dk;
+            if (k >= stride) { k -= stride; ++rr; }
         }
     }
 }
@@ -1024,8 +1057,6 @@
     int k;
     int pivot, next, guard;
     int stage;
-    int r_L;
-    i64 r_start, r_count;
 };
 
 struct ReseedArgs {
@@ -1042,9 +1073,7 @@
     unsigned long long* counters;
     i64* pend_list;
     BlkRec* blk;
-    BlkRec* blk_out;
     i64 blk_cap;
-    int blk_ctr, blk_out_ctr;
 };
 
 template <bool OWNED>
@@ -1170,7 +1199,7 @@
                 stage_plcp_windows(plcp, V, win + threadIdx.x);
                 if (region_walk<true>(V, n, T0, qbeg, qend, l_seq, msl, S, hops, ap, n_pend)) {
                     BlkRec b;
-                    b.rid = r; b.k = k; b.pivot = S.pivot; b.next = S.next; b.guard = S.guard; b.r_L = 0; b.r_start = 0; b.r_count = 0;
+                    b.rid = r; b.k = k; b.pivot = S.pivot; b.next = S.next; b.guard = S.guard;
                     b.stage = S.stage | (n_blk == BLK_PER_READ - 1 ? BLK_MORE : 0);
 #pragma unroll
                     for (int i = 0; i < BLK_PER_READ; ++i) if (i == n_blk) held[i] = b;
@@ -1194,7 +1223,7 @@
             if (blk_hops) atomicAdd(&A.counters[SEED_CTR_SEARCHES], blk_hops);
             if (blk_lane) atomicAdd(&A.counters[SEED_CTR_LANE], blk_lane);
             if (blk_pend) blk_pend_base = (unsigned)atomicAdd(&A.counters[SEED_CTR_PEND], (unsigned long long)blk_pend);
-            if (blk_blk) blk_blk_base = atomicAdd(&A.counters[A.blk_ctr], (unsigned long long)blk_blk);
+            if (blk_blk) blk_blk_base = atomicAdd(&A.counters[SEED_CTR_BLK], (unsigned long long)blk_blk);
         }
         __syncthreads();
         if (n_pend) A.pend_list[blk_pend_base + my_pend] = r | ((i64)pend_ns << 40);
@@ -1208,131 +1237,119 @@
     }
 }
 
-__global__ void __launch_bounds__(256) k_reseed_emit(ReseedArgs A) {
-    __shared__ uint32_t lwin[(LANE_W / 2) * 256];
-    const i64 n_list = (i64)A.counters[SEED_CTR_PEND];
-    for (i64 i = (i64)blockIdx.x * blockDim.x + threadIdx.x; i < n_list; i += (i64)gridDim.x * blockDim.x) {
-        const i64 ent = A.pend_list[i];
-        const i64 r = ent & ((1ll << 40) - 1);
-        const int c = (int)(ent >> 40);
-        SlotRec* sl = A.slots + r * A.cap;
-        const u64* rec = A.packed + r * A.geo.stride;
-        i64 hits_add = 0;
-        int k = -1;
-        for (;;) {
-            for (++k; k < c; ++k) if (sl[k].sa_start & SLOT_PEND) break;
-            if (k >= c) break;
-            LaneQuery q;
-            q.s = rec; q.off = sl[k].start; q.vlen = sl[k].end - sl[k].start;
-            q.wq = ext_g(q.s, q.off);
-            int r_L; i64 r_start, r_count;
-            lane_search(A.I, q, 1, lwin + threadIdx.x, r_L, r_start, r_count);
-            sl[k].sa_start = r_start; sl[k].count = r_count;
-            hits_add += (A.opt.hits_per_smem > 0 && r_count > A.opt.hits_per_smem) ? (i64)A.opt.hits_per_smem : r_count;
-        }
-        atomicAdd(reinterpret_cast<unsigned long long*>(A.slot_hits + r), (unsigned long long)hits_add);
-    }
-}
-
-__global__ void __launch_bounds__(256) k_reseed_search(ReseedArgs A) {
-    __shared__ uint32_t lwin[(LANE_W / 2) * 256];
-    i64 n_blk = (i64)A.counters[A.blk_ctr];
-    if (n_blk > A.blk_cap) n_blk = A.blk_cap;
-    for (i64 i = (i64)blockIdx.x * blockDim.x + threadIdx.x; i < n_blk; i += (i64)gridDim.x * blockDim.x) {
-        BlkRec b = A.blk[i];
-        const u64* rec = A.packed + b.rid * A.geo.stride;
-        const u64 lw = rec[A.geo.stride - 1];
-        RegionState S;
-        S.pivot = b.pivot; S.next = b.next; S.guard = b.guard; S.stage = b.stage & ~BLK_MORE;
-        const LaneQuery q = region_query(rec, A.geo, (int)(lw & 0x7fffffffull), ((lw >> 31) & 1ull) != 0, S);
-        lane_search(A.I, q, 2, lwin + threadIdx.x, b.r_L, b.r_start, b.r_count);
-        A.blk[i].r_L = b.r_L; A.blk[i].r_start = b.r_start; A.blk[i].r_count = b.r_count;
-    }
-}
-
-template <bool LAST>
-__global__ void __launch_bounds__(256) k_reseed_resume(ReseedArgs A) {
+enum : int { JOB_NONE = -1, JOB_PEND = 4 };
+__global__ void __launch_bounds__(256, 4) k_reseed_jobs(ReseedArgs A) {
     __shared__ uint32_t win[2 * (PLCP_WIN / 4) * 256];
     __shared__ uint32_t lwin[(LANE_W / 2) * 256];
-    __shared__ unsigned long long acc_total, acc_lane, out_base;
-    __shared__ unsigned out_n;
     const uint8_t* __restrict__ plcp = A.I.plcp;
     const i64 n = A.I.n;
     const int msl = A.opt.min_seed_len;
-    if (threadIdx.x == 0) { acc_total = 0; acc_lane = 0; }
-    i64 n_blk = (i64)A.counters[A.blk_ctr];
+    const int lane = threadIdx.x & 63;
+    i64 n_blk = (i64)A.counters[SEED_CTR_BLK], n_pend = (i64)A.counters[SEED_CTR_PEND];
     if (n_blk > A.blk_cap) n_blk = A.blk_cap;
+    if (n_pend > A.nreads) n_pend = A.nreads;
+    const i64 n_jobs = n_blk + n_pend;
+    i64 rid = 0;
+    int k = 0, c = 0;
+    RegionState S;
+    S.pivot = 0; S.next = 0; S.guard = 0; S.stage = JOB_NONE;
     unsigned total = 0, lsearches = 0;
-    for (i64 i0 = (i64)blockIdx.x * blockDim.x; i0 < n_blk; i0 += (i64)gridDim.x * blockDim.x) {
-        if (threadIdx.x == 0) out_n = 0;
-        __syncthreads();
-        const i64 i = i0 + threadIdx.x;
-        bool blocked = false;
-        BlkRec nb;
-        if (i < n_blk) {
-            const BlkRec b = A.blk[i];
-            const i64 r = b.rid;
-            SlotRec* sl = A.slots + r * A.cap;
-            const u64* rec = A.packed + r * A.geo.stride;
-            const u64 lw = rec[A.geo.stride - 1];
-            const int l_seq = (int)(lw & 0x7fffffffull);
-            const bool has_n = ((lw >> 31) & 1ull) != 0;
-            SmemAppender<false> ap;
-            ap.sl = sl; ap.cap = A.cap; ap.cnt = A.slot_cnt + r; ap.hits = A.slot_hits + r; ap.ovf_list = A.ovf_list; ap.counters = A.counters; ap.rid = r;
-            ap.hps = A.opt.hits_per_smem; ap.ns = 0; ap.hits_add = 0;
-            unsigned hops = 1;
-            int k = b.k;
-            const int c = (b.stage & BLK_MORE) ? (A.slot_cnt[r] > DEFER_MAX_K ? DEFER_MAX_K : A.slot_cnt[r]) : 0;
-            bool first = true;
-            for (;;) {
-                const int qbeg = sl[k].start, qend = sl[k].end;
-                const i64 T0 = (sl[k].sa_start & SLOT_VAL) - qbeg;
+    bool dry = false;
+    for (;;) {
+        for (;;) {
+            const unsigned long long need = dry ? 0ull : __ballot(S.stage == JOB_NONE);
+            if (!need) break;
+            const int first = __ffsll((long long)need) - 1;
+            unsigned long long tb = 0;
+            if (lane == first) tb = atomicAdd(&A.counters[SEED_CTR_BLK_OUT], (unsigned long long)__popcll(need));
+            tb = __shfl(tb, first);
+            bool over = false;
+            if (S.stage == JOB_NONE) {
+                const i64 t = (i64)tb + __popcll(need & ((1ull << lane) - 1ull));
+                if (t >= n_jobs) over = true;
+                else if (t < n_blk) {
+                    const BlkRec b = A.blk[t];
+                    rid = b.rid; k = b.k;
+                    S.pivot = b.pivot; S.next = b.next; S.guard = b.guard; S.stage = b.stage & ~BLK_MORE;
+                    c = 0;
+                    if (b.stage & BLK_MORE) {
+                        c = A.slot_cnt[rid];
+                        if (c > DEFER_MAX_K) c = DEFER_MAX_K;
+                        if (c > A.cap) c = A.cap;
+                    }
+                    const SlotRec* sl = A.slots + rid * A.cap;
+                    const int qbeg = sl[k].start, qend = sl[k].end;
+                    const i64 T0 = (sl[k].sa_start & SLOT_VAL) - qbeg;
+                    PlcpView V;
+                    V.plcp = plcp; V.win = win + threadIdx.x;
+                    V.F0 = plcp_win_fwd(T0, (qbeg + qend) >> 1); V.R0 = plcp_win_rev(T0, (qbeg + qend) >> 1, n);
+                    stage_plcp_windows(plcp, V, win + threadIdx.x);
+                } else {
+                    const i64 ent = A.pend_list[t - n_blk];
+                    rid = ent & ((1ll << 40) - 1);
+                    c = (int)(ent >> 40);
+                    if (c > A.cap) c = A.cap;
+                    const SlotRec* sl = A.slots + rid * A.cap;
+                    for (k = 0; k < c; ++k) if (sl[k].sa_start & SLOT_PEND) break;
+                    if (k < c) S.stage = JOB_PEND;
+                }
+            }
+            if (__ballot(over)) dry = true;
+        }
+        if (!__ballot(S.stage != JOB_NONE)) break;
+        if (S.stage != JOB_NONE) {
+            SlotRec* sl = A.slots + rid * A.cap;
+            const u64* rec = A.packed + rid * A.geo.stride;
+            const bool pend = S.stage == JOB_PEND;
+            const int qbeg = sl[k].start, qend = sl[k].end;
+            int l_seq = 0;
+            LaneQuery q;
+            if (pend) { q.s = rec; q.off = qbeg; q.vlen = qend - qbeg; q.wq = ext_g(q.s, q.off); }
+            else {
+                const u64 lw = rec[A.geo.stride - 1];
+                l_seq = (int)(lw & 0x7fffffffull);
+                q = region_query(rec, A.geo, l_seq, ((lw >> 31) & 1ull) != 0, S);
+            }
+            int r_L; i64 r_start, r_count;
+            lane_search(A.I, q, pend ? 1 : 2, lwin + threadIdx.x, r_L, r_start, r_count);
+            ++lsearches;
+            if (pend) {
+                sl[k].sa_start = r_start; sl[k].count = r_count;
+                const i64 h = (A.opt.hits_per_smem > 0 && r_count > A.opt.hits_per_smem) ? (i64)A.opt.hits_per_smem : r_count;
+                atomicAdd(reinterpret_cast<unsigned long long*>(A.slot_hits + rid), (unsigned long long)h);
+                for (++k; k < c; ++k) if (sl[k].sa_start & SLOT_PEND) break;
+                if (k >= c) S.stage = JOB_NONE;
+            } else {
+                SmemAppender<false> ap;
+                ap.sl = sl; ap.cap = A.cap; ap.cnt = A.slot_cnt + rid; ap.hits = A.slot_hits + rid; ap.ovf_list = A.ovf_list; ap.counters = A.counters; ap.rid = rid;
+                ap.hps = A.opt.hits_per_smem; ap.ns = 0; ap.hits_add = 0;
+                unsigned hops = 1;
+                int n_dummy = 0;
+                i64 T0 = (sl[k].sa_start & SLOT_VAL) - qbeg;
+                int rb = qbeg, re = qend;
                 PlcpView V;
                 V.plcp = plcp; V.win = win + threadIdx.x;
-                V.F0 = plcp_win_fwd(T0, (qbeg + qend) >> 1); V.R0 = plcp_win_rev(T0, (qbeg + qend) >> 1, n);
-                stage_plcp_windows(plcp, V, win + threadIdx.x);
-                RegionState S;
-                if (first) {
-                    S.pivot = b.pivot; S.next = b.next; S.guard = b.guard; S.stage = b.stage & ~BLK_MORE;
-                    region_apply<false>(S, msl, b.r_L, b.r_start, b.r_count, ap);
-                    first = false;
-                } else { S.pivot = (qbeg + qend) >> 1; S.next = 0; S.guard = 0; S.stage = 0; }
-                while (S.stage != 3) {
-                    int n_pend = 0;
-                    if (!region_walk<false>(V, n, T0, qbeg, qend, l_seq, msl, S, hops, ap, n_pend)) break;
-                    if (!LAST) {
-                        nb.rid = r; nb.k = k; nb.pivot = S.pivot; nb.next = S.next; nb.guard = S.guard; nb.stage = S.stage | (b.stage & BLK_MORE);
-                        nb.r_L = 0; nb.r_start = 0; nb.r_count = 0;
-                        blocked = true;
-                        break;
-                    }
-                    const LaneQuery q = region_query(rec, A.geo, l_seq, has_n, S);
-                    int r_L; i64 r_start, r_count;
-                    lane_search(A.I, q, 2, lwin + threadIdx.x, r_L, r_start, r_count);
-                    ++lsearches; ++hops;
-                    region_apply<false>(S, msl, r_L, r_start, r_count, ap);
-                }
-                if (blocked) break;
-                for (++k; k < c; ++k) if ((sl[k].sa_start & (SLOT_DEFER | SLOT_POS)) == (SLOT_DEFER | SLOT_POS)) break;
-                if (k >= c) break;
-            }
-            total += hops;
-        }
-        unsigned my = 0;
-        if (blocked) my = atomicAdd(&out_n, 1u);
-        __syncthreads();
-        if (threadIdx.x == 0 && out_n) out_base = atomicAdd(&A.counters[A.blk_out_ctr], (unsigned long long)out_n);
-        __syncthreads();
-        if (blocked) A.blk_out[out_base + my] = nb;
-        __syncthreads();
-    }
-    if (total) atomicAdd(&acc_total, (unsigned long long)total);
-    if (lsearches) atomicAdd(&acc_lane, (unsigned long long)lsearches);
-    __syncthreads();
-    if (threadIdx.x == 0) {
-        if (acc_total) atomicAdd(&A.counters[SEED_CTR_SEARCHES], acc_total);
-        if (acc_lane) atomicAdd(&A.counters[SEED_CTR_LANE], acc_lane);
-    }
-}
-
-}
+                V.F0 = plcp_win_fwd(T0, (rb + re) >> 1); V.R0 = plcp_win_rev(T0, (rb + re) >> 1, n);
+                region_apply<false>(S, msl, r_L, r_start, r_count, ap);
+                for (;;) {
+                    if (S.stage != 3 && region_walk<false>(V, n, T0, rb, re, l_seq, msl, S, hops, ap, n_dummy)) break;
+                    for (++k; k < c; ++k) if ((sl[k].sa_start & (SLOT_DEFER | SLOT_POS)) == (SLOT_DEFER | SLOT_POS)) break;
+                    if (k >= c) { S.stage = JOB_NONE; break; }
+                    rb = sl[k].start; re = sl[k].end;
+                    T0 = (sl[k].sa_start & SLOT_VAL) - rb;
+                    V.F0 = plcp_win_fwd(T0, (rb + re) >> 1); V.R0 = plcp_win_rev(T0, (rb + re) >> 1, n);
+                    stage_plcp_windows(plcp, V, win + threadIdx.x);
+                    S.pivot = (rb + re) >> 1; S.next = 0; S.guard = 0; S.stage = 0;
+                }
+                total += hops;
+            }
+        }
+    }
+    for (int d = 32; d > 0; d >>= 1) { total += __shfl_xor(total, d); lsearches += __shfl_xor(lsearches, d); }
+    if (lane == 0) {
+        if (total) atomicAdd(&A.counters[SEED_CTR_SEARCHES], (unsigned long long)total);
+        if (lsearches) atomicAdd(&A.counters[SEED_CTR_LANE], (unsigned long long)lsearches);
+    }
+}
+
+}
```

Result: faster. 156.7 million reads/s (median of 6 runs) (+4.2%).
